# Jabruson/FDN-TIP2025

Hardware: AMD Instinct MI355X
Metric: images/sec, FDN (LPNet->FDN forward) 1280x720 bs=8 fp32 (higher is better)
Workload: dtype f32; 1 GPU; BASELINE.json configs[1]: FDN 1280x720 (padded 1280x736) batch=8 per GPU fp32; global_batch=8, parallelism=batch-shard x1, weights=synthetic (tamed 0.03) FDN + real LPNet, hip_streams=1, rccl_ranks=1, hip_graph=True, fdsa_full=False, fdsa_pair=False, no_tail_pin=False, tail_pin_l2=False, narrow_pipe=False, unfused_mlps=False, stats_launches=False, resample_upsample=False, aff_resized=False

## Files before the change

### fdn-tip2025_amd/basicsr/models/archs/FDN_arch.py

```python
import numbers

import numpy as np
import torch
import torch.nn as nn
import torch.nn.functional as F
from einops import rearrange

import fdn_hip
from fdn_hip import ACT_LEAKY, ACT_NONE, ACT_SIGMOID, ops


_Cache = ops.WeightCache


def _w(p):
    return p.detach()


class WithBias_LayerNorm(nn.Module):

    def __init__(self, dim):
        super().__init__()
        self.weight = nn.Parameter(torch.ones(dim))
        self.bias = nn.Parameter(torch.zeros(dim))
# ... 128 lines not shown
        self.dwconv = nn.Conv2d(hidden, hidden * 2, kernel_size=3, padding=1, groups=hidden, bias=bias)
        self._c = _Cache()

    def fused(self, xn, x_high, xp2, x_img, res=None, ln=None):
        _, _, h, w = xn.shape
        wp = ops.spec_pitch(w // 2 + 1)
        z = ops.rfft_rows_ln(xn, *ln, pitch=wp) if ln is not None else ops.rfft_rows(xn, pitch=wp)
        ops.fft_cols_fcaffn(z, x_high, xp2, _w(self.conv1_xa.weight), _w(self.conv1_xp.weight))
        xi = ops.irfft_rows(z, h, w, 2.0 / (h * w))
        gam, bet = self.norm.params()
        if xi.shape[1] in ops.FCAFFN_IN_C and w % 2 == 0:
            t = ops.fcaffn_in(xi, xn, x_img, _w(self.project_in.weight), gam, bet, _w(self.conv1_mul.weight),
                              _w(self.conv3_mul.weight), _w(self.conv1_add.weight), _w(self.conv3_add.weight), x1_ln=ln)
        elif xi.shape[1] >= ops.FCAFFN_PACKED_MIN_C and fdn_hip.matrix_pipe() == "bf16":
            srcs = [self.project_in.weight, self.conv1_mul.weight, self.conv3_mul.weight, self.conv1_add.weight, self.conv3_add.weight]
            wpk = self._c.get("fcpk", srcs, lambda: ops.fcaffn_in_pack(*[_w(p) for p in srcs]))
            t = ops.fcaffn_in_packed(xi, None if ops.GEMM_OWN_STATS else ops.chan_stats(xi), xn, x_img, wpk, gam, bet, x1_ln=ln)
        else:
            stats = ops.chan_stats(xi)
            mul, add = ops.img_mod_maps(x_img, _w(self.conv1_mul.weight), _w(self.conv3_mul.weight),
                                        _w(self.conv1_add.weight), _w(self.conv3_add.weight))
            t = ops.conv1x1(xi, _w(self.project_in.weight), ln_muladd=(stats, gam, bet, xn), muladd=(mul, add), cache=(self._c, "pi"))
        return ops.ffn_tail(t, _w(self.dwconv.weight), _w(self.project_out.weight), res=res, want_stats=res is not None,
                            cache=(self._c, "po"))

    def forward(self, x, x_high, xp2, x_img=None):
        return self.fused(x, x_high, xp2, x_img)


class TransformerBlock(nn.Module):

    def __init__(self, dim, ffn_expansion_factor=2.66, mode=1, bias=False, LayerNorm_type="WithBias", att=False,
                 use_light=True, use_img=True):
        super().__init__()
        self.use_light = use_light
        self.att = att
        if att:
            self.norm1 = LayerNorm(dim)
            self.attn = FDSA(dim, bias)
        self.norm2 = LayerNorm(dim)
        self.ffn = FDFFN(dim, bias, use_light=use_light, use_img=use_img)
        if use_light:
            self.norm3 = LayerNorm(dim)
            self.ffn2 = FCAFFN(dim, bias, use_light=use_light, use_img=use_img)

    def forward(self, xt):
        x, x_high, x_p, x_img = xt
        if self.att:
            x = self.attn.fused(x, ln=(ops.stats_of(x),) + self.norm1.params(), res=x, pin=(self.ffn, self.norm2.params()))
        x = self.ffn.fused(x, ln=(ops.stats_of(x),) + self.norm2.params(), res=x)
        if self.use_light:
            if (x.shape[1] in ops.FCAFFN_IN_C or (x.shape[1] >= ops.FCAFFN_PACKED_MIN_C and fdn_hip.matrix_pipe() == "bf16")) and ops.rows_ln_ok(x):
                x = self.ffn2.fused(x, x_high, x_p, x_img, res=x, ln=(ops.stats_of(x),) + self.norm3.params())
            else:
                x = self.ffn2.fused(self.norm3(x), x_high, x_p, x_img, res=x)
        return x, x_high, x_p, x_img


class Fuse(nn.Module):

    def __init__(self, n_feat):
        super().__init__()
        self.n_feat = n_feat
        self.att_channel = TransformerBlock(dim=n_feat * 2, use_light=False, use_img=False)
        self.conv = nn.Conv2d(n_feat * 2, n_feat * 2, 1, 1, 0)
        self.conv2 = nn.Conv2d(n_feat * 2, n_feat * 2, 1, 1, 0)
        self._c = _Cache()

    def forward(self, enc, dnc, x_high=None, x_high_p=None, x_img=None):
        n = self.n_feat
        x = ops.conv1x1([enc, dnc], _w(self.conv.weight), _w(self.conv.bias), want_stats=True, cache=(self._c, "c1"))
        x = self.att_channel((x, x_high, x_high_p, x_img))[0]
        wf = self._c.get("w", [self.conv2.weight], lambda: self.conv2.weight.detach()[:n] + self.conv2.weight.detach()[n:])
        bf = self._c.get("b", [self.conv2.bias], lambda: self.conv2.bias.detach()[:n] + self.conv2.bias.detach()[n:])
        return ops.conv1x1(x, wf, bf, cache=(self._c, "c2"), want_stats=True)


class OverlapPatchEmbed(nn.Module):
    def __init__(self, in_c=3, embed_dim=48, bias=False):
        super().__init__()
        self.proj = nn.Conv2d(in_c, embed_dim, kernel_size=3, stride=1, padding=1, bias=bias)

    def forward(self, x):
        return ops.conv2d(x, _w(self.proj.weight), pad=1)


class Downsample(nn.Module):

    def __init__(self, n_feat):
        super().__init__()
        self.body = nn.Sequential(nn.Identity(), nn.Conv2d(n_feat, n_feat * 2, 3, stride=1, padding=1, bias=False))

    def forward(self, x):
        return ops.conv2d(ops.resample(x, ops.RS_BILINEAR_HALF), _w(self.body[1].weight), pad=1)


class Upsample(nn.Module):

    def __init__(self, n_feat):
        super().__init__()
        self.body = nn.Sequential(nn.Identity(), nn.Conv2d(n_feat, n_feat // 2, 3, stride=1, padding=1, bias=False))
        self._c = _Cache()

    def forward(self, x):
        if ops.UPCONV_GATHER:
            return ops.upsample_conv3x3(x, _w(self.body[1].weight), cache=(self._c, "up"))
        return ops.conv2d(ops.resample(x, ops.RS_BILINEAR_X2), _w(self.body[1].weight), pad=1)


class FDformer(nn.Module):

    def __init__(self, inp_channels=3, out_channels=3, dim=48, num_blocks=[6, 6, 12, 8], num_refinement_blocks=4,
                 ffn_expansion_factor=3, bias=False):
        super().__init__()

        def stage(d, n, enc):
            return nn.Sequential(*[TransformerBlock(dim=d, ffn_expansion_factor=ffn_expansion_factor, bias=bias, att=True,
                                                    mode=1 if enc else 2, use_light=enc, use_img=enc) for _ in range(n)])

        self.patch_embed = OverlapPatchEmbed(inp_channels, dim)
        self.encoder_level1 = stage(dim, num_blocks[0], True)
        self.down1_2 = Downsample(dim)
        self.encoder_level2 = stage(dim * 2, num_blocks[1], True)
        self.down2_3 = Downsample(dim * 2)
        self.encoder_level3 = stage(dim * 4, num_blocks[2], True)
        self.decoder_level3 = stage(dim * 4, num_blocks[2], False)
        self.up3_2 = Upsample(dim * 4)
        self.reduce_chan_level2 = nn.Conv2d(dim * 4, dim * 2, kernel_size=1, bias=bias)
        self.decoder_level2 = stage(dim * 2, num_blocks[1], False)
        self.up2_1 = Upsample(dim * 2)
        self.decoder_level1 = stage(dim, num_blocks[0], False)
        self.refinement = stage(dim, num_refinement_blocks, False)
        self.fuse2 = Fuse(dim * 2)
        self.fuse1 = Fuse(dim)
        self.output = nn.Conv2d(dim, out_channels, kernel_size=3, stride=1, padding=1, bias=bias)
        self.norm = LayerNorm(3)

    def forward(self, inp_img, ori_img=None, x_high1=None, x_high2=None, x_high3=None, x_high12=None, x_high22=None,
                x_high32=None, x1=None, x2=None, x3=None):
        e1 = self.encoder_level1((self.patch_embed(inp_img), x_high1, x_high12, x1))[0]
        e2 = self.encoder_level2((self.down1_2(e1), x_high2, x_high22, x2))[0]
        e3 = self.encoder_level3((self.down2_3(e2), x_high3, x_high32, x3))[0]
        d3 = self.decoder_level3((e3, x_high3, x_high32, x3))[0]
        d2 = self.fuse2(self.up3_2(d3), e2, x_high2, x_high22, x2)
        d2 = self.decoder_level2((d2, x_high2, x_high22, x2))[0]
        d1 = self.fuse1(self.up2_1(d2), e1, x_high1, x_high12, x1)
        d1 = self.decoder_level1((d1, x_high1, x_high12, x1))[0]
        d1 = self.refinement((d1, x_high1, x_high12, x1))[0]
        res = inp_img if ori_img is None else ori_img
        return ops.conv2d(d1, _w(self.output.weight), pad=1, res=res)


class BasicConv(nn.Module):
    def __init__(self, in_channel, out_channel, kernel_size, stride, bias=True, relu=True, transpose=False):
        super().__init__()
        self.k, self.stride, self.relu, self.transpose = kernel_size, stride, relu, transpose
        if transpose:
            conv = nn.ConvTranspose2d(in_channel, out_channel, kernel_size, padding=kernel_size // 2 - 1, stride=stride, bias=bias)
        else:
            conv = nn.Conv2d(in_channel, out_channel, kernel_size, padding=kernel_size // 2, stride=stride, bias=bias)
        self.main = nn.Sequential(conv)

    def forward(self, x, res=None, res_before_act=False, act=None, post_add=0.0):
        c = self.main[0]
        a = (ACT_LEAKY if self.relu else ACT_NONE) if act is None else act
        if self.transpose:
            return ops.conv_transpose4x4s2(x, _w(c.weight), _w(c.bias), a)
        if self.k == 1 and self.stride == 1:
            return ops.conv1x1(x, _w(c.weight), _w(c.bias), act=a)
        return ops.conv2d(x, _w(c.weight), _w(c.bias), stride=self.stride, pad=self.k // 2, act=a, res=res,
                          res_before_act=res_before_act, post_add=post_add)


class FAM(nn.Module):
    def __init__(self, channel):
        super().__init__()
        self.merge1 = nn.Conv2d(channel * 2, channel, kernel_size=1)
        self.merge2 = nn.Conv2d(channel, channel, kernel_size=3, stride=1, padding=1)

    def forward(self, x1, x2):
        t = ops.conv1x1([x1, x2], _w(self.merge1.weight), _w(self.merge1.bias))
        return ops.conv2d(t, _w(self.merge2.weight), _w(self.merge2.bias), pad=1)


def _mlp2(seq, x):
    t = ops.conv1x1(x, _w(seq[0].weight), _w(seq[0].bias), act=ACT_LEAKY)
    return ops.conv1x1(t, _w(seq[2].weight), _w(seq[2].bias))


def _spectral_mlps(y, process1, process2, H, W):
    z = ops.rfft_rows(y)
    mag, pha = ops.fft_cols_fwd(z, True, True, rd_before=False, fix_real=True)
    if ops.SPECTRAL_MLP_FUSED and mag.shape[1] in ops.SPECTRAL_MLP_C:
        ops.spectral_mlp2(mag, pha, _w(process1[0].weight), _w(process1[0].bias), _w(process1[2].weight), _w(process1[2].bias),
                          _w(process2[0].weight), _w(process2[0].bias), _w(process2[2].weight), _w(process2[2].bias), slope=0.1)
    else:
        mag = _mlp2(process1, mag)
        pha = _mlp2(process2, pha)
    return ops.fft_cols_inv_polar(mag, pha, H, W // 2 + 1)


class FreBlock(nn.Module):
    def __init__(self, nc):
        super().__init__()
        self.fpre = nn.Conv2d(nc, nc, 1, 1, 0)
        self.process1 = nn.Sequential(nn.Conv2d(nc, nc, 1, 1, 0), nn.LeakyReLU(0.1), nn.Conv2d(nc, nc, 1, 1, 0))
        self.process2 = nn.Sequential(nn.Conv2d(nc, nc, 1, 1, 0), nn.LeakyReLU(0.1), nn.Conv2d(nc, nc, 1, 1, 0))

    def forward(self, x, skip_gain=1.0):
        _, _, H, W = x.shape
        y = ops.conv1x1(x, _w(self.fpre.weight), _w(self.fpre.bias))
        zz = _spectral_mlps(y, self.process1, self.process2, H, W)
        return ops.irfft_rows(zz, H, W, 2.0 / (H * W), res=x, alpha=skip_gain)


class ProcessBlock(nn.Module):
    def __init__(self, in_nc, spatial=False):
        super().__init__()
        self.frequency_process = FreBlock(in_nc)
        self.cat = nn.Conv2d(in_nc, in_nc, 1, 1, 0)

    def forward(self, x):
        return self.frequency_process(x, skip_gain=2.0)


class fourier_fuse(nn.Module):
    def __init__(self, in_nc, out_nc):
        super().__init__()
        self.fpre = nn.Sequential(nn.Conv2d(in_nc, out_nc, 1, 1), nn.Conv2d(out_nc, out_nc, 1, 1, 1, groups=out_nc))
        self.process1 = nn.Sequential(nn.Conv2d(out_nc, out_nc, 1, 1, 0), nn.LeakyReLU(0.1), nn.Conv2d(out_nc, out_nc, 1, 1, 0))
        self.process2 = nn.Sequential(nn.Conv2d(out_nc, out_nc, 1, 1, 0), nn.LeakyReLU(0.1), nn.Conv2d(out_nc, out_nc, 1, 1, 0))
        self.fourier_out = nn.Conv2d(out_nc, out_nc, 3, 1, 1)
        self._c = _Cache()

    def forward(self, x1, x2, x4):
        return self._rest(ops.conv1x1([x1, x2, x4], _w(self.fpre[0].weight), _w(self.fpre[0].bias)))

    def forward_multires(self, same, up1, up2):
        wfull, bias = _w(self.fpre[0].weight), _w(self.fpre[0].bias)
        n = wfull.shape[0]
        ks = sum(t.shape[1] for t in same)
        k1 = 0 if up1 is None else up1.shape[1]
        w2 = wfull.reshape(n, -1)
        parts = self._c.get("split", [self.fpre[0].weight], lambda: (w2[:, :ks].contiguous(), w2[:, ks:ks + k1].contiguous(), w2[:, ks + k1:].contiguous()))
        acc = ops.conv1x1(up2, parts[2])
        if up1 is not None:
            acc = ops.conv1x1(up1, parts[1], res=ops.resample(acc, ops.RS_NEAREST_X2))
        return self._rest(ops.conv1x1(same, parts[0], bias, res=ops.resample(acc, ops.RS_NEAREST_X2)))

    def _rest(self, y):
        H, W = y.shape[-2:]
        y = ops.dw1x1_pad1(y, _w(self.fpre[1].weight), _w(self.fpre[1].bias))
        zz = _spectral_mlps(y, self.process1, self.process2, H, W)
        xo = ops.irfft_rows(zz, H, W, 2.0 / (H * W))
        return ops.conv2d(xo, _w(self.fourier_out.weight), _w(self.fourier_out.bias), pad=1)


class MAR_archa(nn.Module):
    def __init__(self, use_ratio=True, block=None, apply_ratio=True):
        super().__init__()
        ProcessBlock_ = ProcessBlock if block is None else block
        self.use_ratio = use_ratio
        self.apply_ratio = apply_ratio
        c = 12
        self.Encoder = nn.ModuleList([ProcessBlock_(c), ProcessBlock_(c * 2), ProcessBlock_(c * 4)])
        self.Decoder = nn.ModuleList([ProcessBlock_(c * 4), ProcessBlock_(c * 2), ProcessBlock_(c)])
        self.Convs = nn.ModuleList([BasicConv(c * 4, c * 2, 1, 1, relu=True), BasicConv(c * 2, c, 1, 1, relu=True)])
        self.ConvsOut = nn.ModuleList([BasicConv(c * 4, 3, 3, 1, relu=False), BasicConv(c * 2, 3, 3, 1, relu=False)])
        self.AFFs = nn.ModuleList([fourier_fuse(c * 7, c), fourier_fuse(c * 7, c * 2)])
        self.FAM1 = FAM(c * 4)
        self.f1 = nn.Sequential(nn.Conv2d(3 * 16, c * 4, 1, 1, 0), ProcessBlock_(c * 4))
        self.f2 = nn.Sequential(nn.Conv2d(3 * 4, c * 2, 1, 1, 0), ProcessBlock_(c * 2))
        self.f3 = nn.Sequential(nn.Conv2d(3, c, 1, 1, 0), ProcessBlock_(c))
        self.f3_down = BasicConv(c, c * 2, 3, 2, relu=True)
        self.f2_down = BasicConv(c * 2, c * 4, 3, 2, relu=True)
        self.f2_up = BasicConv(c * 4, c * 2, 4, 2, relu=True, transpose=True)
        self.f3_up = BasicConv(c * 2, c, 4, 2, relu=True, transpose=True)
        self.out = BasicConv(c, 3, 3, 1, relu=False)
        self.FAM2 = FAM(c * 2)

    def _stem(self, seq, x, ratio):
        t = seq[1](ops.conv1x1(x, _w(seq[0].weight), _w(seq[0].bias)))
        return ops.scale_batch_(t, ratio) if self.apply_ratio else t

    def forward(self, x, ratio):
        x_2 = ops.resample(x, ops.RS_NEAREST_HALF)
        x_4 = ops.resample(x_2, ops.RS_NEAREST_HALF)
        z2 = self._stem(self.f2, ops.resample(x, ops.RS_PIXEL_UNSHUFFLE, 2), ratio)
        z4 = self._stem(self.f1, ops.resample(x, ops.RS_PIXEL_UNSHUFFLE, 4), ratio)
        x_ = self._stem(self.f3, x, ratio)
        res1 = self.Encoder[0](x_)
        res2 = self.Encoder[1](self.FAM2(self.f3_down(res1), z2))
        z = self.Encoder[2](self.FAM1(self.f2_down(res2), z4))
        z12 = ops.resample(res1, ops.RS_NEAREST_HALF)
        if ops.AFF_MULTIRES:
            res2n = self.AFFs[1].forward_multires([z12, res2], None, z)
            res1 = self.AFFs[0].forward_multires([res1], res2, z)
            res2 = res2n
        else:
            z21 = ops.resample(res2, ops.RS_NEAREST_X2)
            z42 = ops.resample(z, ops.RS_NEAREST_X2)
            z41 = ops.resample(z42, ops.RS_NEAREST_X2)
            res2 = self.AFFs[1](z12, res2, z42)
            res1 = self.AFFs[0](res1, z21, z41)
        z = self.Decoder[0](z)
        o4 = self.ConvsOut[0](z, res=x_4, res_before_act=True, act=ACT_SIGMOID, post_add=1e-8)
        z = self.f2_up(z)
        c0 = self.Convs[0].main[0]
        z = self.Decoder[1](ops.conv1x1([z, res2], _w(c0.weight), _w(c0.bias), act=ACT_LEAKY))
        o2 = self.ConvsOut[1](z, res=x_2, res_before_act=True, act=ACT_SIGMOID, post_add=1e-8)
        z = self.f3_up(z)
        c1 = self.Convs[1].main[0]
        z = self.Decoder[2](ops.conv1x1([z, res1], _w(c1.weight), _w(c1.bias), act=ACT_LEAKY))
        o1 = self.out(z, res=x, res_before_act=True, act=ACT_SIGMOID, post_add=1e-8)
        return [o4, o2, o1]


class MAR(nn.Module):
    def __init__(self, use_ratio=True):
        super().__init__()
        self.net = MAR_archa(use_ratio=True)
        self.scale = 40.0
        self.use_ratio = use_ratio

    def forward(self, x, ratio=None):
        ratio = ratio.reshape(-1).contiguous()
        x1 = x
        x2 = ops.resample(x1, ops.RS_BILINEAR_HALF)
        x3 = ops.resample(x2, ops.RS_BILINEAR_HALF)
        i3, i2, i1 = self.net(x, ratio)
        return ops.gamma_curve(x3, i3, self.scale), ops.gamma_curve(x2, i2, self.scale), ops.gamma_curve(x1, i1, self.scale)


class FDN(nn.Module):

    def __init__(self):
        super().__init__()
        self.net_a = MAR(use_ratio=True)
        self.net_p = FDformer(inp_channels=3, out_channels=3, dim=32, num_blocks=[6, 6, 10], num_refinement_blocks=4,
                              ffn_expansion_factor=3, bias=False)
        for p in self.net_a.parameters():
            p.requires_grad = False
        self.norm1 = LayerNorm(3)
        self.norm2 = LayerNorm(3)
        self.norm3 = LayerNorm(3)

    @staticmethod
    def _spectrum(x, want_abs, want_ang, rd):
        return ops.fft_cols_fwd(ops.rfft_rows(x), want_abs, want_ang, rd_before=rd, fix_real=True)

    def forward(self, inp_img, ori=None, device=None, ratio_i=None, mode=1):
        if ratio_i is None:
            raise ValueError("FDN.forward needs ratio_i of shape (B, 1) (reference FDN_arch.py:872)")
        inp_img = inp_img.contiguous()
        ratio = ratio_i.reshape(-1).to(torch.float32).contiguous()
        norms = (self.norm1, self.norm2, self.norm3)
        p1 = inp_img
        p2 = ops.resample(p1, ops.RS_BILINEAR_HALF)
        p3 = ops.resample(p2, ops.RS_BILINEAR_HALF)
        phas = [self._spectrum(n(p), False, True, True)[1] for n, p in zip(norms, (p1, p2, p3))]
        q3, q2, q1 = self.net_a(inp_img, ratio)
        amps = [self._spectrum(n(q), True, False, False)[0] for n, q in zip(norms, (q1, q2, q3))]
        out = self.net_p(inp_img, ori_img=inp_img, x_high1=amps[0], x_high2=amps[1], x_high3=amps[2],
                         x_high12=phas[0], x_high22=phas[1], x_high32=phas[2], x1=q1, x2=q2, x3=q3)
        return out, q1, q2, q3
```

### fdn-tip2025_amd/basicsr/models/archs/fdnlol24_arch.py

```python
import numbers

import numpy as np
import torch
import torch.nn as nn
import torch.nn.functional as F
from einops import rearrange

from fdn_hip import ops
from basicsr.models.archs.FDN_arch import (FDN, FDformer, FreBlock, LayerNorm, MAR_archa, _w)
from basicsr.models.archs import FDN_arch as _blur


class ProcessBlock(nn.Module):

    def __init__(self, in_nc, spatial=False):
        super().__init__()
        if spatial:
            raise NotImplementedError("spatial=True is never instantiated by FDN_lolv1 (fdnlol24_arch.py:104-137)")
        self.frequency_process = FreBlock(in_nc)
        self.cat = nn.Conv2d(in_nc, in_nc, 1, 1, 0)

    def forward(self, x):
        y = self.frequency_process(x, skip_gain=1.0)
        return ops.conv1x1(y, _w(self.cat.weight), _w(self.cat.bias), res=x)


class fourier_multi_scale_gamma2(MAR_archa):

    def __init__(self, use_ratio):
        super().__init__(use_ratio=use_ratio, block=ProcessBlock, apply_ratio=bool(use_ratio))


class MAR(_blur.MAR):

    def __init__(self, use_ratio=True):
        super().__init__(use_ratio=use_ratio)
        self.net = fourier_multi_scale_gamma2(use_ratio=use_ratio)


class FDN_lolv1(FDN):

    def __init__(self):
        nn.Module.__init__(self)
        self.net_a = MAR(use_ratio=True)
        self.net_p = FDformer(inp_channels=3, out_channels=3, dim=24, num_blocks=[6, 6, 10], num_refinement_blocks=4,
                              ffn_expansion_factor=3, bias=False)
        for p in self.net_a.parameters():
            p.requires_grad = False
        self.norm1 = LayerNorm(3)
        self.norm2 = LayerNorm(3)
        self.norm3 = LayerNorm(3)

    def forward(self, inp_img, ori=None, device=None, ratio_i=None, mode=1):
        out = super().forward(inp_img, ori=ori, device=device, ratio_i=ratio_i, mode=mode)[0]
        return out, out, out, out
```

### fdn-tip2025_amd/csrc/capi.hip

```cpp
#include "common.hpp"

#include <atomic>
extern "C" int fdn_abi_version(void) { return 20; }

static std::atomic<int> g_matrix_pipe_mode{0};
extern "C" int fdn_set_matrix_pipe(int mode) {
    if (mode < 0 || mode > 2) return FDN_ERR_ARG;
    g_matrix_pipe_mode.store(mode);
    return FDN_OK;
}
bool fdn_matrix_pipe_f32() { return g_matrix_pipe_mode.load() == 1; }
bool fdn_matrix_pipe_wide() { return g_matrix_pipe_mode.load() == 0; }

static std::atomic<long long> g_bf16_launches{0};
void fdn_note_bf16_launch() { g_bf16_launches.fetch_add(1, std::memory_order_relaxed); }
extern "C" long fdn_bf16_mfma_launches(void) { return g_bf16_launches.load(); }

extern "C" const char* fdn_error_string(int code) {
    switch (code) {
        case FDN_OK: return "ok";
        case FDN_ERR_ARG: return "invalid argument (null pointer, bad shape or unsupported size)";
        case FDN_ERR_LAUNCH: return "HIP kernel launch failed";
        case FDN_ERR_WORKSPACE: return "workspace too small";
        case FDN_ERR_UNSUPPORTED: return "configuration not supported by this build";
        default: return "unknown error";
    }
}

#include <mutex>
#include <map>
#include <utility>

namespace {
std::mutex g_mu;
int g_cus_by_dev[64];
int g_cu_budget_by_dev[64];
std::map<std::pair<const void*, int>, size_t> g_lds_limit;
struct OccKey {
    const void* k; int dev, threads; size_t lds;
    bool operator<(const OccKey& o) const {
        if (k != o.k) return k < o.k;
        if (dev != o.dev) return dev < o.dev;
        if (threads != o.threads) return threads < o.threads;
        return lds < o.lds;
    }
};
std::map<OccKey, int> g_occ;
}

bool fdn_occupancy(int* blocks_per_cu, const void* kernel, int threads, size_t lds) {
    int dev = 0;
    if (hipGetDevice(&dev) != hipSuccess) return false;
    std::lock_guard<std::mutex> lk(g_mu);
    const OccKey key{kernel, dev, threads, lds};
    auto it = g_occ.find(key);
    if (it == g_occ.end()) {
        int n = 0;
        if (hipOccupancyMaxActiveBlocksPerMultiprocessor(&n, kernel, threads, lds) != hipSuccess) return false;
        it = g_occ.emplace(key, n).first;
    }
    *blocks_per_cu = it->second;
    return true;
}

int fdn_persistent_grid(const void* kernel, int threads, size_t lds, int total_tiles, fdn_grid_cap cap) {
    const int cus = fdn_device_cus();
    if (cus <= 0) return -1;
    if (lds > 48 * 1024 && !fdn_allow_dynamic_lds(kernel, lds)) return -1;
    int per_cu = 1 << 20;
    if (cap.by_occupancy && !fdn_occupancy(&per_cu, kernel, threads, lds)) per_cu = 1;
    if (cap.max_wg > 0 && per_cu > cap.max_wg) per_cu = cap.max_wg;
    if (cap.max_waves > 0 && per_cu * (threads / 64) > cap.max_waves) per_cu = cap.max_waves / (threads / 64);
    if (cap.lds_budget > 0 && lds > 0 && (size_t)per_cu > cap.lds_budget / lds) per_cu = (int)(cap.lds_budget / lds);
    if (per_cu < 1) per_cu = 1;
    const long grid = (long)cus * per_cu;
    return grid > total_tiles ? total_tiles : (int)grid;
}

namespace {
int device_cus_locked(int dev) {
    if (g_cus_by_dev[dev] == 0) {
        int n = 0;
        if (hipDeviceGetAttribute(&n, hipDeviceAttributeMultiprocessorCount, dev) != hipSuccess || n <= 0) return -1;
        g_cus_by_dev[dev] = n;
    }
    return g_cus_by_dev[dev];
// ... 33 lines not shown
```

### fdn-tip2025_amd/csrc/convs.hip

```cpp
#include "common.hpp"

int fdn_conv3x3_mfma(const float* x, const float* w, const float* bias, const float* res, float* out, int B, int Cin, int H,
                     int W, int Cout, int act, int res_before_act, float post_add, hipStream_t s);

namespace {

constexpr int OCB = 8;

struct ConvArgs {
    const float* x; const float* w; const float* bias; const float* res; float* out;
    int B, Cin, H, W, Cout, OH, OW, KH, KW, stride, pad;
    int act; int res_before_act; float post_add;
};

__global__ __launch_bounds__(256) void conv2d_kernel(ConvArgs a) {
    unsigned bx, by, bz;
    fdn_xcd_block3(bx, by, bz);
    const long op = (long)bx * 256 + threadIdx.x;
    const int oc0 = by * OCB, b = bz;
    const long OP = (long)a.OH * a.OW;
    const bool live = op < OP;
    const int oy = live ? (int)(op / a.OW) : 0, ox = live ? (int)(op - (long)oy * a.OW) : 0;
    float acc[OCB];
#pragma unroll
// ... 13 lines not shown
                const float* wp = a.w + ((long)oc0 * a.Cin + ci) * kk + ky * a.KW + kx;
#pragma unroll
                for (int o = 0; o < OCB; ++o)
                    if (o < nvalid) acc[o] = fmaf(v, wp[(long)o * a.Cin * kk], acc[o]);
            }
        }
    }
    if (!live) return;
#pragma unroll
    for (int o = 0; o < OCB; ++o) {
        if (o >= nvalid) break;
        const int oc = oc0 + o;
        float v = acc[o] + (a.bias ? a.bias[oc] : 0.f);
        const long oi = ((long)b * a.Cout + oc) * OP + op;
        if (a.res && a.res_before_act) v += a.res[oi];
        v = apply_act(v, a.act);
        if (a.res && !a.res_before_act) v += a.res[oi];
        a.out[oi] = v + a.post_add;
    }
}

template <int S, int OCB_>
__global__ __launch_bounds__(256) void conv3x3_direct_kernel(ConvArgs a) {
    extern __shared__ __attribute__((aligned(16))) float wl[];
    unsigned bx, by, bz;
    fdn_xcd_block3(bx, by, bz);
    const int oc0 = by * OCB_, b = bz;
    const int nvalid = min(OCB_, a.Cout - oc0);
    for (int i = threadIdx.x; i < a.Cin * 9 * OCB_; i += 256) {
        const int o = i % OCB_, t = (i / OCB_) % 9, ci = i / (OCB_ * 9);
        wl[i] = o < nvalid ? a.w[((long)(oc0 + o) * a.Cin + ci) * 9 + t] : 0.f;
    }
    __syncthreads();
    const long op = (long)bx * 256 + threadIdx.x;
    const long OP = (long)a.OH * a.OW;
    const bool live = op < OP;
    const int oy = live ? (int)(op / a.OW) : 0, ox = live ? (int)(op - (long)oy * a.OW) : 0;
    int off[9];
    unsigned ok = 0;
#pragma unroll
    for (int t = 0; t < 9; ++t) {
        const int iy = oy * S - 1 + t / 3, ix = ox * S - 1 + t % 3;
        const bool v = live && iy >= 0 && iy < a.H && ix >= 0 && ix < a.W;
        off[t] = v ? iy * a.W + ix : 0;
        ok |= (v ? 1u : 0u) << t;
    }
    float acc[OCB_];
#pragma unroll
    for (int o = 0; o < OCB_; ++o) acc[o] = 0.f;
    const long hw = (long)a.H * a.W;
    const float* xc = a.x + (long)b * a.Cin * hw;
    for (int ci = 0; ci < a.Cin; ++ci, xc += hw) {
        float v[9];
#pragma unroll
        for (int t = 0; t < 9; ++t) v[t] = xc[off[t]];
#pragma unroll
        for (int t = 0; t < 9; ++t) {
            const float vv = ((ok >> t) & 1u) ? v[t] : 0.f;
            const float* wp = wl + (ci * 9 + t) * OCB_;
#pragma unroll
            for (int o = 0; o < OCB_; ++o) acc[o] = fmaf(vv, wp[o], acc[o]);
        }
    }
    if (!live) return;
#pragma unroll
    for (int o = 0; o < OCB_; ++o) {
        if (o >= nvalid) break;
        const int oc = oc0 + o;
        float v = acc[o] + (a.bias ? a.bias[oc] : 0.f);
        const long oi = ((long)b * a.Cout + oc) * OP + op;
        if (a.res && a.res_before_act) v += a.res[oi];
        v = apply_act(v, a.act);
        if (a.res && !a.res_before_act) v += a.res[oi];
        a.out[oi] = v + a.post_add;
    }
}

template <int S, int OCB_>
int launch_conv3x3_direct(const ConvArgs& a, hipStream_t s) {
    const size_t lds = (size_t)a.Cin * 9 * OCB_ * sizeof(float);
    if (lds > 64 * 1024) return FDN_ERR_UNSUPPORTED;
    hipLaunchKernelGGL((conv3x3_direct_kernel<S, OCB_>), dim3(cdiv((long)a.OH * a.OW, 256), cdiv(a.Cout, OCB_), a.B), dim3(256),
                       lds, s, a);
    return fdn_launch_status();
}

template <int OCB_>
__global__ __launch_bounds__(256) void convT_kernel(const float* __restrict__ x, const float* __restrict__ w,
                                                    const float* __restrict__ bias, float* __restrict__ out, int Cin, int H,
                                                    int W, int Cout, int act) {
    extern __shared__ __attribute__((aligned(16))) float wl[];
    unsigned bx, by, bz;
    fdn_xcd_block3(bx, by, bz);
    const int oc0 = by * OCB_, b = bz;
    const int nvalid = min(OCB_, Cout - oc0);
    for (int i = threadIdx.x; i < Cin * 16 * OCB_; i += 256) {
        const int o = i % OCB_, t = (i / OCB_) % 16, ci = i / (OCB_ * 16);
        wl[i] = o < nvalid ? w[((long)ci * Cout + oc0 + o) * 16 + t] : 0.f;
    }
    __syncthreads();
    const int OH = 2 * H, OW = 2 * W;
    const long op = (long)bx * 256 + threadIdx.x;
    const long OP = (long)OH * OW;
    const bool live = op < OP;
    const int oy = live ? (int)(op / OW) : 0, ox = live ? (int)(op - (long)oy * OW) : 0;
    const int ky0 = (oy + 1) & 1, kx0 = (ox + 1) & 1;
    int off[4], tap[4];
    unsigned ok = 0;
#pragma unroll
    for (int j = 0; j < 4; ++j) {
        const int ky = ky0 + 2 * (j >> 1), kx = kx0 + 2 * (j & 1);
        const int ny = oy + 1 - ky, nx = ox + 1 - kx;
        const int iy = ny >> 1, ix = nx >> 1;
        const bool v = live && ny >= 0 && iy < H && nx >= 0 && ix < W;
        off[j] = v ? iy * W + ix : 0;
        tap[j] = (ky * 4 + kx) * OCB_;
        ok |= (v ? 1u : 0u) << j;
    }
    float acc[OCB_];
#pragma unroll
    for (int o = 0; o < OCB_; ++o) acc[o] = 0.f;
    const long hw = (long)H * W;
    const float* xc = x + (long)b * Cin * hw;
    for (int ci = 0; ci < Cin; ++ci, xc += hw) {
        float v[4];
#pragma unroll
        for (int j = 0; j < 4; ++j) v[j] = xc[off[j]];
#pragma unroll
        for (int j = 0; j < 4; ++j) {
            const float vv = ((ok >> j) & 1u) ? v[j] : 0.f;
            const float* wp = wl + ci * 16 * OCB_ + tap[j];
#pragma unroll
            for (int o = 0; o < OCB_; ++o) acc[o] = fmaf(vv, wp[o], acc[o]);
        }
    }
    if (!live) return;
#pragma unroll
    for (int o = 0; o < OCB_; ++o) {
        if (o >= nvalid) break;
        out[((long)b * Cout + oc0 + o) * OP + op] = apply_act(acc[o] + (bias ? bias[oc0 + o] : 0.f), act);
    }
}

template <int OCB_>
__global__ __launch_bounds__(256) void convT_quad_kernel(const float* __restrict__ x, const float* __restrict__ w, const float* __restrict__ bias,
                                                         float* __restrict__ out, int Cin, int H, int W, int Cout, int act) {
    static_assert(OCB_ % 4 == 0, "weight rows are read as 16-byte words");
    extern __shared__ __attribute__((aligned(16))) float wl[];
    unsigned bx, by, bz;
    fdn_xcd_block3(bx, by, bz);
    const int oc0 = by * OCB_, b = bz;
    const int nvalid = min(OCB_, Cout - oc0);
    for (int i = threadIdx.x; i < Cin * 16 * OCB_; i += 256) {
        const int o = i % OCB_, t = (i / OCB_) % 16, ci = i / (OCB_ * 16);
        wl[i] = o < nvalid ? w[((long)ci * Cout + oc0 + o) * 16 + t] : 0.f;
    }
    __syncthreads();
    const long hw = (long)H * W;
    const int W2 = W >> 1;
    const long ip = (long)bx * 256 + threadIdx.x;
    const bool live = ip < (long)H * W2;
    const int iy = live ? (int)(ip / W2) : 0, ix0 = live ? 2 * (int)(ip - (long)iy * W2) : 0;
    int off[12];
    unsigned ok = 0;
#pragma unroll
    for (int d = 0; d < 12; ++d) {
// ... 262 lines not shown
        const float* w1 = ws, *w2t = ws + C * C, *b1 = ws + 2 * C * C, *b2 = b1 + C;
        float v[C], o[C];
#pragma unroll
        for (int i = 0; i < C; ++i) v[i] = t[base + (long)i * P];
#pragma unroll
        for (int k = 0; k < C; ++k) o[k] = b2[k];
#pragma unroll 1
        for (int j = 0; j < C; ++j) {
            float s = b1[j];
#pragma unroll
            for (int i = 0; i < C; ++i) s = fmaf(w1[j * C + i], v[i], s);
            const float h = s > 0.f ? s : s * slope;
#pragma unroll
            for (int k = 0; k < C; ++k) o[k] = fmaf(w2t[j * C + k], h, o[k]);
        }
#pragma unroll
        for (int k = 0; k < C; ++k) t[base + (long)k * P] = o[k];
    };
    mlp(mag, wsh);
    mlp(pha, wsh + WS);
}

__global__ __launch_bounds__(256) void gamma_curve_kernel(const float* __restrict__ x, const float* __restrict__ im,
                                                          float* __restrict__ out, float scale, long total) {
    const long idx = (long)blockIdx.x * 256 + threadIdx.x;
    if (idx < total) out[idx] = 1.0f - powf(1.0f - x[idx], im[idx] * scale);
}

template <int CIN, int COUT>
__global__ __launch_bounds__(256) void conv7x7s2_kernel(ConvArgs a) {
    constexpr int TR = 8, TCW = 32;
    constexpr int IR = 2 * TR + 5, IC = 2 * TCW + 5;
    constexpr int HC = (IC + 1) / 2;
    __shared__ float tile[CIN][IR][2][HC + 1];
    __shared__ __attribute__((aligned(16))) float wl[CIN * 49 * COUT];
    unsigned bx, by, bz;
    fdn_xcd_block3(bx, by, bz);
    const int tid = threadIdx.x, b = bz;
    const int oy0 = by * TR, ox0 = bx * TCW;
    for (int i = tid; i < CIN * 49 * COUT; i += 256) {
        const int o = i % COUT, t = i / COUT;
        wl[i] = a.w[(long)o * CIN * 49 + t];
    }
    const long hw = (long)a.H * a.W;
    const float* xb = a.x + (long)b * CIN * hw;
    const int iy0 = oy0 * 2 - 3, ix0 = ox0 * 2 - 3;
    for (int i = tid; i < CIN * IR * IC; i += 256) {
        const int c = i % IC, r = (i / IC) % IR, ci = i / (IC * IR);
        const int iy = iy0 + r, ix = ix0 + c;
        tile[ci][r][c & 1][c >> 1] = (iy >= 0 && iy < a.H && ix >= 0 && ix < a.W) ? xb[(long)ci * hw + (long)iy * a.W + ix] : 0.f;
    }
    __syncthreads();
    const int ty = tid >> 5, tx = tid & 31;
    float acc[COUT];
#pragma unroll
    for (int o = 0; o < COUT; ++o) acc[o] = 0.f;
#pragma unroll 1
    for (int ci = 0; ci < CIN; ++ci)
#pragma unroll
        for (int ky = 0; ky < 7; ++ky)
#pragma unroll
            for (int kx = 0; kx < 7; ++kx) {
                const float v = tile[ci][2 * ty + ky][kx & 1][tx + (kx >> 1)];
                const float* wp = wl + ((ci * 7 + ky) * 7 + kx) * COUT;
#pragma unroll
                for (int o = 0; o < COUT; ++o) acc[o] = fmaf(v, wp[o], acc[o]);
            }
    const int oy = oy0 + ty, ox = ox0 + tx;
    if (oy >= a.OH || ox >= a.OW) return;
    const long OP = (long)a.OH * a.OW, op = (long)oy * a.OW + ox;
#pragma unroll
    for (int oc = 0; oc < COUT; ++oc) {
        float v = acc[oc] + (a.bias ? a.bias[oc] : 0.f);
        const long oi = ((long)b * COUT + oc) * OP + op;
        if (a.res && a.res_before_act) v += a.res[oi];
        v = apply_act(v, a.act);
        if (a.res && !a.res_before_act) v += a.res[oi];
        a.out[oi] = v + a.post_add;
    }
}

}

extern "C" int fdn_conv2d(const float* x, const float* w, const float* bias, const float* res, float* out, int B, int Cin,
                          int H, int W, int Cout, int KH, int KW, int stride, int pad, int act, int res_before_act,
                          float post_add, fdn_stream_t stream) {
    FDN_CHECK_ARG(x && w && out && B > 0 && Cin > 0 && Cout > 0 && H > 0 && W > 0 && KH > 0 && KW > 0 && stride > 0 && pad >= 0);
    ConvArgs a;
    a.x = x; a.w = w; a.bias = bias; a.res = res; a.out = out;
    a.B = B; a.Cin = Cin; a.H = H; a.W = W; a.Cout = Cout; a.KH = KH; a.KW = KW; a.stride = stride; a.pad = pad;
    a.OH = (H + 2 * pad - KH) / stride + 1;
    a.OW = (W + 2 * pad - KW) / stride + 1;
    FDN_CHECK_ARG(a.OH > 0 && a.OW > 0);
    a.act = act; a.res_before_act = res_before_act; a.post_add = post_add;
    hipStream_t s = static_cast<hipStream_t>(stream);
    if (KH == 3 && KW == 3 && pad == 1 && (stride == 1 || stride == 2)) {
        int rc = FDN_ERR_UNSUPPORTED;
        if (stride == 1 && Cin % 8 == 0 && Cin >= 16 && Cout >= 16 && !fdn_matrix_pipe_f32()) {
            rc = fdn_conv3x3_mfma(x, w, bias, res, out, B, Cin, H, W, Cout, act, res_before_act, post_add, s);
            if (rc != FDN_ERR_UNSUPPORTED) return rc;
        }
        if (stride == 2) rc = Cout <= 8 ? launch_conv3x3_direct<2, 8>(a, s) : launch_conv3x3_direct<2, 16>(a, s);
        else if (Cout <= 4) rc = launch_conv3x3_direct<1, 4>(a, s);
        else if (Cout <= 8) rc = launch_conv3x3_direct<1, 8>(a, s);
        else if (Cout <= 64) rc = launch_conv3x3_direct<1, 16>(a, s);
        if (rc != FDN_ERR_UNSUPPORTED) return rc;
        if (stride == 1) {
            rc = fdn_conv3x3_mfma(x, w, bias, res, out, B, Cin, H, W, Cout, act, res_before_act, post_add, s);
            if (rc != FDN_ERR_UNSUPPORTED) return rc;
        }
    }
    if (KH == 7 && KW == 7 && stride == 2 && pad == 3 && Cin == 3 && Cout == 16) {
        hipLaunchKernelGGL((conv7x7s2_kernel<3, 16>), dim3(cdiv(a.OW, 32), cdiv(a.OH, 8), B), dim3(256), 0, s, a);
        return fdn_launch_status();
    }
    hipLaunchKernelGGL(conv2d_kernel, dim3(cdiv((long)a.OH * a.OW, 256), cdiv(Cout, OCB), B), dim3(256), 0, s, a);
    return fdn_launch_status();
}

extern "C" int fdn_conv_transpose4x4s2(const float* x, const float* w, const float* bias, float* out, int B, int Cin, int H,
                                       int W, int Cout, int act, fdn_stream_t stream) {
    FDN_CHECK_ARG(x && w && out && B > 0 && Cin > 0 && Cout > 0 && H > 0 && W > 0);
    hipStream_t s = static_cast<hipStream_t>(stream);
    if (Cout >= 12 && W % 2 == 0 && (size_t)Cin * 16 * 12 * sizeof(float) <= 48 * 1024 && (reinterpret_cast<uintptr_t>(out) & 15) == 0) {
        hipLaunchKernelGGL(convT_quad_kernel<12>, dim3(cdiv((long)H * (W / 2), 256), cdiv(Cout, 12), B), dim3(256), (size_t)Cin * 16 * 12 * sizeof(float), s,
                           x, w, bias, out, Cin, H, W, Cout, act);
        return fdn_launch_status();
    }
    if (Cout > 8 && (size_t)Cin * 16 * 16 * sizeof(float) <= 64 * 1024) {
        hipLaunchKernelGGL(convT_kernel<16>, dim3(cdiv(4L * H * W, 256), cdiv(Cout, 16), B), dim3(256), (size_t)Cin * 16 * 16 * sizeof(float),
                           s, x, w, bias, out, Cin, H, W, Cout, act);
    } else {
        FDN_CHECK_ARG((size_t)Cin * 16 * 8 * sizeof(float) <= 64 * 1024);
        hipLaunchKernelGGL(convT_kernel<8>, dim3(cdiv(4L * H * W, 256), cdiv(Cout, 8), B), dim3(256), (size_t)Cin * 16 * 8 * sizeof(float), s,
                           x, w, bias, out, Cin, H, W, Cout, act);
    }
    return fdn_launch_status();
}

extern "C" int fdn_resample(const float* x, float* out, long planes, int H, int W, int mode, int r, fdn_stream_t stream) {
    FDN_CHECK_ARG(x && out && planes > 0 && H > 0 && W > 0);
    int OH, OW;
    long oplanes = planes;
    switch (mode) {
        case FDN_RS_BILINEAR_HALF:
        case FDN_RS_NEAREST_HALF: FDN_CHECK_ARG(H % 2 == 0 && W % 2 == 0); OH = H / 2; OW = W / 2; break;
        case FDN_RS_BILINEAR_X2:
        case FDN_RS_NEAREST_X2: OH = 2 * H; OW = 2 * W; break;
        case FDN_RS_PIXEL_UNSHUFFLE: FDN_CHECK_ARG(r > 0 && H % r == 0 && W % r == 0); OH = H / r; OW = W / r; oplanes = planes * r * r; break;
        default: return FDN_ERR_ARG;
    }
    FDN_CHECK_ARG(OH <= 65535);
    const long rr = mode == FDN_RS_PIXEL_UNSHUFFLE ? (long)r * r : 1;
    FDN_CHECK_ARG(rr <= 65535);
    const long chunk = 65535 / rr * rr;
    for (long p0 = 0; p0 < oplanes; p0 += chunk) {
        const long np = oplanes - p0 < chunk ? oplanes - p0 : chunk;
        const long in_pl = p0 / rr;
        const bool quad = OW % 4 == 0 && ((reinterpret_cast<uintptr_t>(x) | reinterpret_cast<uintptr_t>(out)) & 15) == 0 &&
                          (mode != FDN_RS_BILINEAR_HALF || W % 8 == 0);
        const dim3 qgrid((unsigned)cdiv((long)OH * (OW / 4), 256), (unsigned)np);
        if (quad && mode == FDN_RS_BILINEAR_X2)
            hipLaunchKernelGGL(resample4_kernel<FDN_RS_BILINEAR_X2>, qgrid, dim3(256), 0, static_cast<hipStream_t>(stream),
                               x + in_pl * H * W, out + p0 * OH * OW, H, W, OH, OW);
        else if (quad && mode == FDN_RS_BILINEAR_HALF)
            hipLaunchKernelGGL(resample4_kernel<FDN_RS_BILINEAR_HALF>, qgrid, dim3(256), 0, static_cast<hipStream_t>(stream),
                               x + in_pl * H * W, out + p0 * OH * OW, H, W, OH, OW);
        else if (quad && mode == FDN_RS_NEAREST_X2 && W % 2 == 0)
            hipLaunchKernelGGL(resample4_kernel<FDN_RS_NEAREST_X2>, qgrid, dim3(256), 0, static_cast<hipStream_t>(stream),
                               x + in_pl * H * W, out + p0 * OH * OW, H, W, OH, OW);
        else
        hipLaunchKernelGGL(resample_kernel, dim3(cdiv(OW, 256), OH, (unsigned)np), dim3(256), 0, static_cast<hipStream_t>(stream),
                           x + in_pl * H * W, out + p0 * OH * OW, np, H, W, OH, OW, mode, r);
    }
    return fdn_launch_status();
}

extern "C" int fdn_upconv_gather(const float* z, float* out, int B, int Cout, int h, int w, fdn_stream_t stream) {
    FDN_CHECK_ARG(z && out && B > 0 && Cout > 0 && h > 0 && w > 0 && B < 65536);
    FDN_CHECK_ARG((reinterpret_cast<uintptr_t>(out) & 7) == 0);
    if ((long)h * w > 0x7FFFFFFFL / 4) return FDN_ERR_UNSUPPORTED;
    constexpr int COB = 8;
    hipLaunchKernelGGL(upconv_gather_kernel<COB>, dim3((unsigned)cdiv((long)h * w, 256), (unsigned)cdiv(Cout, COB), (unsigned)B), dim3(256), 0,
                       static_cast<hipStream_t>(stream), z, out, Cout, h, w);
    return fdn_launch_status();
}

extern "C" int fdn_dw1x1_pad1(const float* x, const float* w, const float* bias, float* out, int B, int C, int H, int W,
                              fdn_stream_t stream) {
    FDN_CHECK_ARG(x && w && bias && out && B > 0 && C > 0 && H > 0 && W > 0);
    FDN_CHECK_ARG(H + 2 <= 65535 && (long)B * C <= 65535);
    hipLaunchKernelGGL(dw1x1_pad1_kernel, dim3(cdiv(W + 2, 256), H + 2, (unsigned)(B * C)), dim3(256), 0, static_cast<hipStream_t>(stream),
                       x, w, bias, out, C, H, W);
    return fdn_launch_status();
}

extern "C" int fdn_avgpool3s2(const float* x, float* out, long planes, int H, int W, fdn_stream_t stream) {
    FDN_CHECK_ARG(x && out && planes > 0 && H > 0 && W > 0);
    const int OH = (H + 2 - 3) / 2 + 1, OW = (W + 2 - 3) / 2 + 1;
    hipLaunchKernelGGL(avgpool3s2_kernel, dim3(cdiv(planes * OH * OW, 256)), dim3(256), 0, static_cast<hipStream_t>(stream), x,
// ... 47 lines not shown
```

### fdn-tip2025_amd/csrc/fft2d.hip

```cpp
#include <math.h>

#include <map>
#include <mutex>
#include <vector>

#include "common.hpp"
#include "fft_regs.hpp"

namespace {

constexpr int MAX_STAGES = FDN_FFT_MAX_STAGES;
constexpr int NT = 256;

struct Plan {
    int N;
    int nst;
    int radix[MAX_STAGES];
    const float2* tw;
    int tab_mul;
};

std::mutex g_mu;
std::map<std::pair<int, int>, const float2*> g_tables;

// ... 300 lines not shown
    __syncthreads();
    return src;
}

constexpr int EMAX = 36;

template <bool INV, int R>
__device__ void fft_pass_inplace(float2* buf, int N, int Ns, int nseq, const float2* __restrict__ tw) {
    constexpr int JMAX = EMAX / R;
    const int T = N / R;
    const int L = Ns * R;
    const int tws = N / L, twr = N / R;
    const int jobs = T * nseq;
    const float r_nseq = 1.0f / (float)nseq, r_Ns = 1.0f / (float)Ns;
    float2 u[JMAX][R];
#pragma unroll
    for (int j = 0; j < JMAX; ++j) {
        const int job = threadIdx.x + NT * j;
        if (job < jobs) {
            const int i = fdiv(job, r_nseq), s = job - i * nseq;
            const int k = i - fdiv(i, r_Ns) * Ns;
#pragma unroll
            for (int r = 0; r < R; ++r) u[j][r] = buf[s + (i + r * T) * nseq];
            if (k) {
#pragma unroll
                for (int r = 1; r < R; ++r) u[j][r] = cmul(u[j][r], twd<INV>(tw, r * k * tws));
            }
        }
    }
    __syncthreads();
#pragma unroll
    for (int j = 0; j < JMAX; ++j) {
        const int job = threadIdx.x + NT * j;
        if (job < jobs) {
            const int i = fdiv(job, r_nseq), s = job - i * nseq;
            const int k = i - fdiv(i, r_Ns) * Ns;
            float2* dp = buf + s + ((i - k) * R + k) * nseq;
            if (R == 2) {
                dp[0] = make_float2(u[j][0].x + u[j][1].x, u[j][0].y + u[j][1].y);
                dp[Ns * nseq] = make_float2(u[j][0].x - u[j][1].x, u[j][0].y - u[j][1].y);
            } else if (R == 4) {
                const float2 a = make_float2(u[j][0].x + u[j][2].x, u[j][0].y + u[j][2].y);
                const float2 b = make_float2(u[j][0].x - u[j][2].x, u[j][0].y - u[j][2].y);
                const float2 c = make_float2(u[j][1].x + u[j][3].x, u[j][1].y + u[j][3].y);
                const float2 d = make_float2(u[j][1].x - u[j][3].x, u[j][1].y - u[j][3].y);
                const float2 jd = INV ? make_float2(-d.y, d.x) : make_float2(d.y, -d.x);
                dp[0] = make_float2(a.x + c.x, a.y + c.y);
                dp[Ns * nseq] = make_float2(b.x + jd.x, b.y + jd.y);
                dp[2 * Ns * nseq] = make_float2(a.x - c.x, a.y - c.y);
                dp[3 * Ns * nseq] = make_float2(b.x - jd.x, b.y - jd.y);
            } else if constexpr (R % 2 == 1) {
                float2 wR[(R - 1) / 2];
#pragma unroll
                for (int t = 1; t <= (R - 1) / 2; ++t) wR[t - 1] = twd<INV>(tw, t * twr);
                dft_odd<R>(u[j], wR);
#pragma unroll
                for (int o = 0; o < R; ++o) dp[o * Ns * nseq] = u[j][o];
            }
        }
    }
    __syncthreads();
}

template <bool INV, int BIG>
__device__ void fft_run_inplace(float2* buf, const Plan& p, const float2* tw, int nseq) {
    int Ns = 1;
    __syncthreads();
    for (int st = 0; st < p.nst; ++st) {
        const int R = p.radix[st];
        switch (R) {
            case 2: fft_pass_inplace<INV, 2>(buf, p.N, Ns, nseq, tw); break;
            case 3: fft_pass_inplace<INV, 3>(buf, p.N, Ns, nseq, tw); break;
            case 4: fft_pass_inplace<INV, 4>(buf, p.N, Ns, nseq, tw); break;
            case 5: fft_pass_inplace<INV, 5>(buf, p.N, Ns, nseq, tw); break;
            case 7: fft_pass_inplace<INV, 7>(buf, p.N, Ns, nseq, tw); break;
            case 17: if (BIG) fft_pass_inplace<INV, 17>(buf, p.N, Ns, nseq, tw); break;
            case 23: if (BIG) fft_pass_inplace<INV, 23>(buf, p.N, Ns, nseq, tw); break;
            default: break;
        }
        Ns *= R;
    }
}

template <bool BIG>
__global__ __launch_bounds__(NT) void rfft_rows_kernel(const float* __restrict__ in, float2* __restrict__ out, int W, long R,
                                                       int rpb, const Plan p, const Rader rd, int pitch) {
    extern __shared__ __attribute__((aligned(16))) unsigned char smem[];
    const int M = W / 2, Wf = M + 1;
    float2* A = reinterpret_cast<float2*>(smem);
    float2* Bf = A + (long)rpb * M;
    float2* twl = Bf + (long)rpb * M;
    float2* tws = twl + W;
    for (int i = threadIdx.x; i < W; i += NT) twl[i] = p.tw[i];
    if (rd.p)
        for (int i = threadIdx.x; i < M - 1; i += NT) tws[i] = rd.sub.tw[i];
    const long row0 = (long)blockIdx.x * rpb;
    const int nrow = (int)min((long)rpb, R - row0);
    {
        constexpr int U = 8;
        const float2* in2 = reinterpret_cast<const float2*>(in + row0 * W);
        const int tot = rpb * M, live = nrow * M;
        if (M % 2 == 0 && (reinterpret_cast<uintptr_t>(in) & 15) == 0) {
            const float4* in4 = reinterpret_cast<const float4*>(in2);
            float4* A4 = reinterpret_cast<float4*>(A);
            const int tot4 = tot / 2, live4 = live / 2;
            for (int base = threadIdx.x; base < tot4; base += NT * 4) {
                float4 v[4];
#pragma unroll
                for (int u = 0; u < 4; ++u) {
                    const int idx = base + NT * u;
                    v[u] = in4[idx < live4 ? idx : 0];
                }
#pragma unroll
                for (int u = 0; u < 4; ++u) {
                    const int idx = base + NT * u;
                    if (idx < tot4) A4[idx] = idx < live4 ? v[u] : make_float4(0.f, 0.f, 0.f, 0.f);
                }
            }
        } else
        for (int base = threadIdx.x; base < tot; base += NT * U) {
            float2 v[U];
#pragma unroll
            for (int u = 0; u < U; ++u) {
                const int idx = base + NT * u;
                v[u] = in2[idx < live ? idx : 0];
            }
#pragma unroll
            for (int u = 0; u < U; ++u) {
                const int idx = base + NT * u;
                if (idx < tot) A[idx] = idx < live ? v[u] : make_float2(0.f, 0.f);
            }
        }
    }
    float2* Z;
    if (rd.p) {
        const int n = M - 1;
        float2* z0 = tws + n;
        __syncthreads();
        for (int idx = threadIdx.x; idx < rpb * n; idx += NT) {
            const int s = idx / n, q = idx - s * n;
            Bf[s * M + q] = A[s * M + rd.perm_in[q]];
        }
        if (threadIdx.x < rpb) z0[threadIdx.x] = A[threadIdx.x * M];
        float2* Y = fft_run<false, BIG>(Bf, A, rd.sub, tws, rpb, M, 1, false);
        float2* other = (Y == Bf) ? A : Bf;
        __syncthreads();
        for (int idx = threadIdx.x; idx < rpb * n; idx += NT) {
            const int s = idx / n, k = idx - s * n;
            const float2 y = Y[s * M + k];
            if (k == 0) other[s * M + n] = make_float2(z0[s].x + y.x, z0[s].y + y.y);
            Y[s * M + k] = cmul(y, rd.bhat[k]);
        }
        __syncthreads();
        float2 x0 = make_float2(0.f, 0.f);
        const bool keeper = threadIdx.x < rpb;
        if (keeper) x0 = other[threadIdx.x * M + n];
        float2* Cv = fft_run<true, BIG>(Y, other, rd.sub, tws, rpb, M, 1, false);
        float2* dst = (Cv == Y) ? other : Y;
        __syncthreads();
        for (int idx = threadIdx.x; idx < rpb * n; idx += NT) {
            const int s = idx / n, q = idx - s * n;
            const float2 c = Cv[s * M + q];
            dst[s * M + rd.perm_out[q]] = make_float2(z0[s].x + c.x, z0[s].y + c.y);
        }
        if (keeper) dst[threadIdx.x * M] = x0;
        __syncthreads();
        Z = dst;
    } else {
        Z = fft_run<false, BIG>(A, Bf, p, twl, rpb, M, 1, false);
    }
    const int tw1 = p.tab_mul / 2;
    const float r_Wf = 1.0f / (float)Wf;
#pragma unroll 4
    for (int idx = threadIdx.x; idx < nrow * Wf; idx += NT) {
        const int s = fdiv(idx, r_Wf), k = idx - s * Wf;
        const float2 zk = Z[s * M + (k == M ? 0 : k)];
        const float2 zc = Z[s * M + (k == 0 ? 0 : M - k)];
        const float2 e = make_float2(0.5f * (zk.x + zc.x), 0.5f * (zk.y - zc.y));
        const float2 d = make_float2(0.5f * (zk.x - zc.x), 0.5f * (zk.y + zc.y));
        const float2 o = make_float2(d.y, -d.x);
        float2 x;
        if (k == 0) x = make_float2(e.x + o.x, 0.0f);
        else if (k == M) x = make_float2(e.x - o.x, 0.0f);
        else {
            const float2 w = twl[k * tw1];
            x = make_float2(e.x + (o.x * w.x - o.y * w.y), e.y + (o.x * w.y + o.y * w.x));
        }
        out[(row0 + s) * pitch + k] = x;
    }
    for (int idx = threadIdx.x; idx < nrow * (pitch - Wf); idx += NT) {
        const int s = idx / (pitch - Wf), k = Wf + idx - s * (pitch - Wf);
        out[(row0 + s) * pitch + k] = make_float2(0.f, 0.f);
    }
}

template <bool BIG>
__global__ __launch_bounds__(NT) void irfft_rows_kernel(const float2* __restrict__ in, long in_ws, long in_plane_rows,
                                                        long in_plane_stride, float* __restrict__ out, int W, int H, long R,
                                                        int rpb, float scale, const float* __restrict__ res, float alpha,
                                                        const Plan p) {
    extern __shared__ __attribute__((aligned(16))) unsigned char smem[];
    const int M = W / 2;
    float2* A = reinterpret_cast<float2*>(smem);
    float2* Bf = A + (long)rpb * M;
    float2* twl = Bf + (long)rpb * M;
    for (int i = threadIdx.x; i < W; i += NT) twl[i] = p.tw[i];
    __syncthreads();
    const long row0 = (long)blockIdx.x * rpb;
    const int nrow = (int)min((long)rpb, R - row0);
    const int tw1 = p.tab_mul / 2;
    constexpr int UL = 4;
    const float r_M = 1.0f / (float)M, r_H = 1.0f / (float)H;
    for (int base = threadIdx.x; base < rpb * M; base += NT * UL) {
      float2 xks[UL], xcs[UL];
#pragma unroll
      for (int u = 0; u < UL; ++u) {
        const int idx = base + NT * u;
        const int s0 = fdiv(idx, r_M), k = idx - s0 * M;
        const int s = min(s0, nrow - 1);
        const long row = row0 + s;
        const long plane = row < (1L << 22) ? (long)fdiv((int)row, r_H) : row / H, h = row - plane * H;
        const float2* src = in + plane * in_plane_stride + h * in_ws;
        xks[u] = src[k];
        xcs[u] = src[M - k];
      }
#pragma unroll
      for (int u = 0; u < UL; ++u) {
        const int idx = base + NT * u;
        if (idx >= rpb * M) continue;
        const int s = fdiv(idx, r_M), k = idx - s * M;
        float2 z = make_float2(0.f, 0.f);
        if (s < nrow) {
            float2 xk = xks[u], xc = xcs[u];
            if (k == 0) { xk.y = 0.f; xc.y = 0.f; }
            const float2 e = make_float2(0.5f * (xk.x + xc.x), 0.5f * (xk.y - xc.y));
            const float2 d = make_float2(0.5f * (xk.x - xc.x), 0.5f * (xk.y + xc.y));
            const float2 w = twl[k * tw1];
            const float2 o = make_float2(d.x * w.x + d.y * w.y, d.y * w.x - d.x * w.y);
            z = make_float2(e.x - o.y, e.y + o.x);
        }
        A[idx] = z;
      }
    }
    float2* Z = fft_run<true, BIG>(A, Bf, p, twl, rpb, M, 1, false);
    {
        constexpr int US = 8;
        const float2* res2 = res ? reinterpret_cast<const float2*>(res + row0 * W) : nullptr;
        float2* out2 = reinterpret_cast<float2*>(out + row0 * W);
        const int live = nrow * M;
        if (M % 2 == 0 && ((reinterpret_cast<uintptr_t>(out) | reinterpret_cast<uintptr_t>(res)) & 15) == 0) {
            const float4* res4 = reinterpret_cast<const float4*>(res2);
            float4* out4 = reinterpret_cast<float4*>(out2);
            const float4* Z4 = reinterpret_cast<const float4*>(Z);
            const int live4 = live / 2;
            for (int base = threadIdx.x; base < live4; base += NT * 4) {
                float4 r[4];
                if (res4) {
#pragma unroll
                    for (int u = 0; u < 4; ++u) r[u] = res4[min(base + NT * u, live4 - 1)];
                }
#pragma unroll
                for (int u = 0; u < 4; ++u) {
                    const int idx = base + NT * u;
                    if (idx >= live4) continue;
                    float4 v = Z4[idx];
                    v.x *= scale; v.y *= scale; v.z *= scale; v.w *= scale;
                    if (res4) {
                        v.x = fmaf(alpha, r[u].x, v.x); v.y = fmaf(alpha, r[u].y, v.y);
                        v.z = fmaf(alpha, r[u].z, v.z); v.w = fmaf(alpha, r[u].w, v.w);
                    }
                    out4[idx] = v;
                }
            }
        } else
        for (int base = threadIdx.x; base < live; base += NT * US) {
            float2 r[US];
            if (res2) {
#pragma unroll
                for (int u = 0; u < US; ++u) r[u] = res2[min(base + NT * u, live - 1)];
            }
#pragma unroll
            for (int u = 0; u < US; ++u) {
                const int idx = base + NT * u;
                if (idx >= live) continue;
                float2 v = Z[idx];
                v.x *= scale;
                v.y *= scale;
                if (res2) {
                    v.x = fmaf(alpha, r[u].x, v.x);
                    v.y = fmaf(alpha, r[u].y, v.y);
                }
                out2[idx] = v;
            }
        }
    }
}

struct ColArgs {
    float2* z;
    int H, Wf, C;
    int tc, tcs;
    long planes;
    const float4* guide;
    const float* wxa;
    const float* wxp;
    float* out_abs;
    float* out_ang;
    int rd_before;
    int fix_real;
    const float* in_mag;
    const float* in_pha;
    int Hin, Wfin;
};

enum { COL_FCAFFN = 0, COL_FWD = 1, COL_INV_POLAR = 2 };

template <int MODE, int BIG, bool INPL>
__global__ __launch_bounds__(NT, (INPL ? 2 : 1)) void fft_cols_kernel(ColArgs a, const Plan p) {
    extern __shared__ __attribute__((aligned(16))) unsigned char smem[];
    const int H = a.H, Wf = a.Wf, tc = a.tc;
    float2* A = reinterpret_cast<float2*>(smem);
    float2* Bf = A + (long)H * tc;
    float2* twl = INPL ? Bf : Bf + (long)H * tc;
    for (int i = threadIdx.x; i < H; i += NT) twl[i] = p.tw[i];
    int plane, col0;
    {
        const int ntile = (Wf + tc - 1) / tc;
        const long total = (long)ntile * a.planes, per_xcd = (total + 7) / 8;
        const long w = (long)(blockIdx.x & 7) * per_xcd + (blockIdx.x >> 3);
        if (w >= total) return;
        const int C = a.C;
        const long grp = w / C;
        const int ch = (int)(w - grp * C);
        plane = (int)(grp / ntile) * C + ch;
        col0 = (int)(grp % ntile) * tc;
    }
    const int ncol = min(tc, Wf - col0);
    float2* zp = a.z + (long)plane * H * Wf;

    const int per = H * tc, tcs = a.tcs, tcm = tc - 1;
    if (MODE == COL_INV_POLAR) {
        constexpr int U = 4;
        for (int base = threadIdx.x; base < per; base += NT * U) {
            float mg[U], ph[U];
#pragma unroll
            for (int u = 0; u < U; ++u) {
                const int idx = base + NT * u, h = idx >> tcs, c = idx & tcm;
                mg[u] = 0.f; ph[u] = 0.f;
                if (idx < per && c < ncol) {
                    const long o = ((long)plane * a.Hin + h) * a.Wfin + col0 + c;
                    mg[u] = a.in_mag[o];
                    ph[u] = a.in_pha[o];
                }
            }
#pragma unroll
            for (int u = 0; u < U; ++u) {
                const int idx = base + NT * u;
                if (idx < per) {
                    float sn, cs;
                    fdn_sincos(ph[u], &sn, &cs);
                    A[idx] = make_float2(mg[u] * cs, mg[u] * sn);
                }
            }
        }
    } else {
        constexpr int U = 12;
        for (int base = threadIdx.x; base < per; base += NT * U) {
            float2 v[U];
#pragma unroll
            for (int u = 0; u < U; ++u) {
                const int idx = base + NT * u, h = idx >> tcs, c = idx & tcm;
                v[u] = make_float2(0.f, 0.f);
                if (idx < per && c < ncol) v[u] = zp[(long)h * Wf + col0 + c];
// ... 524 lines not shown
    const long row0 = (long)blockIdx.x * RW;
    const int nrow = (int)min((long)RW, R - row0);
    {
        const int n2 = tid & (P - 1), rw = tid / P < RW ? tid / P : RW - 1;
        const int rwc = rw < nrow ? rw : nrow - 1;
        const __amdgpu_buffer_rsrc_t rin = cols_rsrc(in + row0 * W, (long)nrow * W * 4);
        const unsigned voff = (unsigned)(rwc * W + 2 * n2) * 4u;
        f2 u[R1];
        sfor<0, R1>([&](auto n1) { u[decltype(n1)::value] = bload2(rin, voff, (unsigned)(decltype(n1)::value * P * 8)); });
        if constexpr (LN) {
            const long row = row0 + rwc, plane = row / lnp.H;
            const int h = (int)(row - plane * lnp.H), c = (int)(plane % lnp.C);
            const long b = plane / lnp.C, HW = (long)lnp.H * W;
            const __amdgpu_buffer_rsrc_t rs_ = cols_rsrc(lnp.stats, (R / ((long)lnp.C * lnp.H)) * 2 * HW * 4);
            const unsigned so = (unsigned)(b * 2 * HW + h * W + 2 * n2) * 4u;
            const float ga = lnp.gamma[c], be = lnp.beta[c];
            f2 mu[R1], rs[R1];
            sfor<0, R1>([&](auto n1) {
                constexpr int N1 = decltype(n1)::value;
                mu[N1] = bload2(rs_, so, (unsigned)(N1 * P * 8));
                rs[N1] = bload2(rs_, so + (unsigned)HW * 4u, (unsigned)(N1 * P * 8));
            });
            sfor<0, R1>([&](auto n1) {
                constexpr int N1 = decltype(n1)::value;
                u[N1] = (u[N1] - mu[N1]) * rs[N1] * ga + be;
            });
        }
        fftr::dft_nat<R1, false>(u);
        sfor<0, R1>([&](auto k1) { Y[rw * RS + decltype(k1)::value * PS + n2] = u[decltype(k1)::value]; });
    }
    __syncthreads();
    const int jt = (tid + 64 * (int)(blockIdx.x & 3)) & 255;
    const bool worker = jt < NJ;
    const int rg = jt / R1, k1 = jt - rg * R1;
    f2 v[32];
    if (worker) {
        const f2* yb = Y + rg * CJ * RS + k1 * PS;
        sfor<0, P>([&](auto n) {
            constexpr int N2 = decltype(n)::value;
#pragma unroll
            for (int cc = 0; cc < CJ; ++cc) v[cc * P + N2] = yb[cc * RS + N2];
            if constexpr (N2 > 0) {
                const f2 w = tw2[(N2 - 1) * R1 + k1];
#pragma unroll
                for (int cc = 0; cc < CJ; ++cc) v[cc * P + N2] = fftr::cmul(v[cc * P + N2], w);
            }
        });
#pragma unroll
        for (int cc = 0; cc < CJ; ++cc) fftr::dft_nat<P, false>(v + cc * P);
    }
    __syncthreads();
    if (worker) {
        f2* zb = Y + rg * CJ * RS + k1;
        sfor<0, P>([&](auto k2) {
#pragma unroll
            for (int cc = 0; cc < CJ; ++cc) zb[cc * RS + R1 * decltype(k2)::value] = v[cc * P + decltype(k2)::value];
        });
    }
    __syncthreads();
    f2* out2 = reinterpret_cast<f2*>(out) + row0 * pitch;
    const int live = nrow * pitch;
    const float r_Wf = 1.0f / (float)pitch;
#pragma unroll 4
    for (int idx = tid; idx < live; idx += 256) {
        const int s = fdiv(idx, r_Wf), k = idx - s * pitch;
        if (k >= Wf) { out2[idx] = f2{0.f, 0.f}; continue; }
        const f2 zk = Y[s * RS + (k == M ? 0 : k)];
        const f2 zc = Y[s * RS + (k == 0 ? 0 : M - k)];
        const f2 e = 0.5f * f2{zk.x + zc.x, zk.y - zc.y};
        const f2 d = 0.5f * f2{zk.x - zc.x, zk.y + zc.y};
        const f2 o = fftr::mul_ni(d);
        f2 x;
        if (k == 0) x = f2{e.x + o.x, 0.0f};
        else if (k == M) x = f2{e.x - o.x, 0.0f};
        else x = e + fftr::cmul(o, tws[k]);
        out2[idx] = x;
    }
}

template <int R1, int P>
__global__ __launch_bounds__(256, 2) void irfft_rows_rp_kernel(const float2* __restrict__ in, long in_ws, long in_plane_stride,
                                                               float* __restrict__ out, int H, long R, float scale,
                                                               const float* __restrict__ res, float alpha,
                                                               const float2* __restrict__ tab) {
    typedef RowPlan<R1, P> L;
    constexpr int M = L::M, W = L::W, RW = L::RW, CJ = L::CJ, PS = L::PS, RS = L::RS, NJ = L::NJ;
    extern __shared__ __attribute__((aligned(16))) unsigned char smem[];
    f2* Y = reinterpret_cast<f2*>(smem);
    f2* tw2 = Y + RW * RS;
    f2* tws = tw2 + (P - 1) * R1;
    __shared__ long rowoff[RW];
    const int tid = threadIdx.x;
    for (int i = tid; i < L::NTW; i += 256) tw2[i] = f2{tab[i].x, tab[i].y};
    const long row0 = (long)blockIdx.x * RW;
    const int nrow = (int)min((long)RW, R - row0);
    if (tid < RW) {
        const long row = row0 + min(tid, nrow - 1);
        const long plane = row / H, h = row - plane * H;
        rowoff[tid] = plane * in_plane_stride + h * in_ws;
    }
    __syncthreads();
    {
        constexpr int UL = 4, NP = M / 2 + 1, TOT = RW * NP;
        const f2* in2 = reinterpret_cast<const f2*>(in);
        const float r_NP = 1.0f / (float)NP;
        for (int base = tid; base < TOT; base += 256 * UL) {
            f2 xks[UL], xcs[UL];
#pragma unroll
            for (int u = 0; u < UL; ++u) {
                const int idx = min(base + 256 * u, TOT - 1), s = fdiv(idx, r_NP), k = idx - s * NP;
                const f2* src = in2 + rowoff[s];
                xks[u] = src[k];
                xcs[u] = src[M - k];
            }
#pragma unroll
            for (int u = 0; u < UL; ++u) {
                const int idx = base + 256 * u;
                if (idx >= TOT) continue;
                const int s = fdiv(idx, r_NP), k = idx - s * NP;
                f2 xk = xks[u], xc = xcs[u];
                if (k == 0) { xk.y = 0.f; xc.y = 0.f; }
                const f2 e = 0.5f * f2{xk.x + xc.x, xk.y - xc.y};
                const f2 d = 0.5f * f2{xk.x - xc.x, xk.y + xc.y};
                const f2 io = fftr::mul_pi(fftr::cmulc(d, tws[k]));
                f2* row = Y + s * RS;
                row[k] = e + io;
                if (k != 0) {
                    const f2 c = e - io;
                    row[M - k] = f2{c.x, -c.y};
                }
            }
        }
    }
    __syncthreads();
    const int jt = (tid + 64 * (int)(blockIdx.x & 3)) & 255;
    const bool worker = jt < NJ;
    const int rg = jt / R1, k1 = jt - rg * R1;
    f2 v[32];
    if (worker) {
        const f2* zb = Y + rg * CJ * RS + k1;
        sfor<0, P>([&](auto k2) {
#pragma unroll
            for (int cc = 0; cc < CJ; ++cc) v[cc * P + decltype(k2)::value] = zb[cc * RS + R1 * decltype(k2)::value];
        });
#pragma unroll
        for (int cc = 0; cc < CJ; ++cc) fftr::dft_nat<P, true>(v + cc * P);
    }
    __syncthreads();
    if (worker) {
        f2* yb = Y + rg * CJ * RS + k1 * PS;
        sfor<0, P>([&](auto n) {
            constexpr int N2 = decltype(n)::value;
            if constexpr (N2 > 0) {
                const f2 w = tw2[(N2 - 1) * R1 + k1];
#pragma unroll
                for (int cc = 0; cc < CJ; ++cc) v[cc * P + N2] = fftr::cmulc(v[cc * P + N2], w);
            }
#pragma unroll
            for (int cc = 0; cc < CJ; ++cc) yb[cc * RS + N2] = v[cc * P + N2];
        });
    }
    __syncthreads();
    {
        const int n2 = tid & (P - 1), rw = tid / P;
        const int rwl = rw < RW ? rw : RW - 1;
        f2 u[R1];
        sfor<0, R1>([&](auto k) { u[decltype(k)::value] = Y[rwl * RS + decltype(k)::value * PS + n2]; });
        fftr::dft_nat<R1, true>(u);
        if (rw < nrow) {
            const __amdgpu_buffer_rsrc_t ro = cols_rsrc(out + row0 * W, (long)nrow * W * 4);
            const __amdgpu_buffer_rsrc_t rr = cols_rsrc(res ? res + row0 * W : out, res ? (long)nrow * W * 4 : 0);
            const unsigned voff = (unsigned)(rw * W + 2 * n2) * 4u;
            f2 r[R1];
            if (res) sfor<0, R1>([&](auto n1) { r[decltype(n1)::value] = bload2(rr, voff, (unsigned)(decltype(n1)::value * P * 8)); });
            sfor<0, R1>([&](auto n1) {
                constexpr int N1 = decltype(n1)::value;
                f2 x = u[N1] * scale;
                if (res) x += alpha * r[N1];
                bstore2(x, ro, voff, (unsigned)(N1 * P * 8));
            });
        }
    }
}

const float2* get_table_rows_rp(int R1, int P) {
    int devid = 0;
    if (hipGetDevice(&devid) != hipSuccess) return nullptr;
    std::lock_guard<std::mutex> lk(g_mu);
    const int key = -(1 << 24) - (R1 * 1024 + P);
    auto it = g_tables.find({devid, key});
    if (it != g_tables.end()) return it->second;
    const int M = R1 * P, W = 2 * M;
    auto root = [](long t, long N) {
        t %= N;
        double c, s;
        if ((4 * t) % N == 0) {
            const int q = (int)((4 * t) / N);
            c = (q == 0) ? 1.0 : (q == 2 ? -1.0 : 0.0);
            s = (q == 1) ? 1.0 : (q == 3 ? -1.0 : 0.0);
        } else {
            const double ang = 2.0 * M_PI * (double)t / (double)N;
            c = cos(ang); s = sin(ang);
        }
        float2 w = make_float2((float)c, (float)(-s) + 0.0f);
        if (w.y == 0.0f) w.y = 0.0f;
        if (w.x == 0.0f) w.x = 0.0f;
        return w;
    };
    std::vector<float2> h;
    for (int n2 = 1; n2 < P; ++n2)
        for (int k1 = 0; k1 < R1; ++k1) h.push_back(root((long)n2 * k1, M));
    for (int k = 0; k <= M; ++k) h.push_back(root(k, W));
    float2* d = nullptr;
    if (hipMalloc(&d, sizeof(float2) * h.size()) != hipSuccess) return nullptr;
    if (hipMemcpy(d, h.data(), sizeof(float2) * h.size(), hipMemcpyHostToDevice) != hipSuccess) return nullptr;
    g_tables[{devid, key}] = d;
    return d;
}

template <int R1, int P>
int launch_rfft_rp(const float* in, float* out_c, long rows, fdn_stream_t stream, int pitch, const RowLN* ln = nullptr) {
    typedef RowPlan<R1, P> L;
    const float2* tab = get_table_rows_rp(R1, P);
    if (!tab) return FDN_ERR_LAUNCH;
    if (ln) {
        if (int e = set_lds(rfft_rows_rp_kernel<R1, P, true>, L::lds)) return e;
        hipLaunchKernelGGL((rfft_rows_rp_kernel<R1, P, true>), dim3(cdiv(rows, L::RW)), dim3(256), L::lds, static_cast<hipStream_t>(stream),
                           in, reinterpret_cast<float2*>(out_c), rows, tab, *ln, pitch);
        return fdn_launch_status();
    }
    if (int e = set_lds(rfft_rows_rp_kernel<R1, P, false>, L::lds)) return e;
    hipLaunchKernelGGL((rfft_rows_rp_kernel<R1, P, false>), dim3(cdiv(rows, L::RW)), dim3(256), L::lds, static_cast<hipStream_t>(stream), in,
                       reinterpret_cast<float2*>(out_c), rows, tab, RowLN{}, pitch);
    return fdn_launch_status();
}

template <int R1, int P>
int launch_irfft_rp(const float* in_c, long in_row_bins, long in_plane_bins, float* out, long planes, int H, float scale,
                    const float* res, float alpha, fdn_stream_t stream) {
    typedef RowPlan<R1, P> L;
    const float2* tab = get_table_rows_rp(R1, P);
    if (!tab) return FDN_ERR_LAUNCH;
    if (int e = set_lds(irfft_rows_rp_kernel<R1, P>, L::lds)) return e;
    const long rows = planes * H;
    hipLaunchKernelGGL((irfft_rows_rp_kernel<R1, P>), dim3(cdiv(rows, L::RW)), dim3(256), L::lds, static_cast<hipStream_t>(stream),
                       reinterpret_cast<const float2*>(in_c), in_row_bins, in_plane_bins, out, H, rows, scale, res, alpha, tab);
    return fdn_launch_status();
}

bool rows_plan(int W, int* R1, int* P) {
    for (int r : {20, 30})
        for (int p : {32, 16, 8})
            if (W == 2 * r * p) { *R1 = r; *P = p; return true; }
    for (int p : {16, 8})
        if (W == 2 * 19 * p) { *R1 = 19; *P = p; return true; }
    for (int p : {16, 8, 4})
        if (W == 2 * 35 * p) { *R1 = 35; *P = p; return true; }
    return false;
}
#define FDN_ROWS_DISPATCH(CALL)                                        \
    switch (R1 * 64 + P) {                                             \
        case 20 * 64 + 32: return CALL(20, 32);                        \
        case 20 * 64 + 16: return CALL(20, 16);                        \
        case 20 * 64 + 8: return CALL(20, 8);                          \
        case 30 * 64 + 32: return CALL(30, 32);                        \
        case 30 * 64 + 16: return CALL(30, 16);                        \
        case 30 * 64 + 8: return CALL(30, 8);                          \
        case 19 * 64 + 16: return CALL(19, 16);                        \
        case 19 * 64 + 8: return CALL(19, 8);                          \
        case 35 * 64 + 16: return CALL(35, 16);                        \
        case 35 * 64 + 8: return CALL(35, 8);                          \
        case 35 * 64 + 4: return CALL(35, 4);                          \
        default: break;                                                \
    }

}

extern "C" int fdn_fft_prepare(int n) {
    FDN_CHECK_ARG(n > 0);
    {
        int R = 0, P = 0;
        if (cols_plan(n, &R, &P) && !get_table_rp(R, P)) return FDN_ERR_LAUNCH;
    }
    {
        int R1 = 0, P = 0;
        if (rows_plan(n, &R1, &P) && !get_table_rows_rp(R1, P)) return FDN_ERR_LAUNCH;
    }
    return get_table(n) ? FDN_OK : FDN_ERR_LAUNCH;
}

extern "C" int fdn_fft_route(int kind, int n, int* desc, int ndesc) {
    FDN_CHECK_ARG(kind >= 0 && kind <= 2 && n >= 1 && desc && ndesc >= FDN_FFT_ROUTE_DESC);
    FDN_CHECK_ARG(kind == 2 || n % 2 == 0);
    for (int i = 0; i < FDN_FFT_ROUTE_DESC; ++i) desc[i] = 0;
    int R = 0, P = 0;
    if (kind == 2 ? cols_plan(n, &R, &P) : rows_plan(n, &R, &P)) {
        desc[0] = FDN_FFT_PLANNED;
        desc[2] = kind == 2 ? 256 / P : row_plan_groups(R, P) * (32 / P);
        desc[4] = 2;
        desc[5] = R;
        desc[6] = P;
        return FDN_OK;
    }
    Route r;
    if (kind == 2) cols_route(n, &r);
    else rows_route(n, kind == 0, &r);
    desc[0] = r.kind;
    if (r.kind == FDN_FFT_REFUSED) return FDN_OK;
    desc[1] = r.big;
    desc[2] = r.width;
    const Plan& q = r.kind == FDN_FFT_RADER ? r.sub : r.p;
    desc[3] = r.kind == FDN_FFT_RADER ? n / 2 : 0;
    desc[4] = q.nst;
    for (int i = 0; i < q.nst; ++i) {
        const int x = q.radix[i];
        const bool reg = x == 2 || x == 4 || x == 3 || x == 5 || x == 7 || (r.big >= 1 && (x == 17 || x == 23)) ||
                         (r.big == 2 && (x == 13 || x == 37 || x == 41));
        desc[5 + i] = x;
        desc[5 + MAX_STAGES + i] = (r.kind != FDN_FFT_INPLACE && !reg) ? 1 : 0;
    }
    return FDN_OK;
}

namespace {
__global__ __launch_bounds__(256) void sincos_kernel(const float* __restrict__ x, float* __restrict__ sn, float* __restrict__ cs, long n) {
    const long i = (long)blockIdx.x * 256 + threadIdx.x;
    if (i < n) {
        float s, c;
        fdn_sincos(x[i], &s, &c);
        sn[i] = s;
        cs[i] = c;
    }
}
}

extern "C" int fdn_sincos_f32(const float* x, float* sn, float* cs, long n, fdn_stream_t stream) {
    FDN_CHECK_ARG(x && sn && cs && n > 0 && n < (1L << 39));
    hipLaunchKernelGGL(sincos_kernel, dim3((unsigned)cdiv(n, 256)), dim3(256), 0, static_cast<hipStream_t>(stream), x, sn, cs, n);
    return fdn_launch_status();
}

extern "C" int fdn_rfft_rows(const float* in, float* out_c, long rows, int W, long out_row_bins, fdn_stream_t stream) {
    FDN_CHECK_ARG(in && out_c && rows > 0 && W >= 2 && W % 2 == 0 && (out_row_bins == 0 || (out_row_bins >= W / 2 + 1 && out_row_bins < (1L << 20))));
    const int pitch = out_row_bins ? (int)out_row_bins : W / 2 + 1;
    {
        int R1 = 0, P = 0;
        if (rows_plan(W, &R1, &P) && (reinterpret_cast<uintptr_t>(in) & 7) == 0) {
#define FDN_CALL(a, b) launch_rfft_rp<a, b>(in, out_c, rows, stream, pitch)
            FDN_ROWS_DISPATCH(FDN_CALL)
#undef FDN_CALL
        }
    }
    Route r;
    rows_route(W, true, &r);
    if (r.kind == FDN_FFT_REFUSED) return FDN_ERR_UNSUPPORTED;
    Plan p;
    if (!make_plan(W / 2, W, &p)) return FDN_ERR_UNSUPPORTED;
    Rader rd = {};
    if (r.kind == FDN_FFT_RADER && !get_rader(W / 2, &rd)) return FDN_ERR_LAUNCH;
    const int rpb = r.width;
    const size_t lds = r.lds;
    if (r.big) {
        if (int e = set_lds(rfft_rows_kernel<true>, lds)) return e;
        hipLaunchKernelGGL(rfft_rows_kernel<true>, dim3(cdiv(rows, rpb)), dim3(NT), lds, static_cast<hipStream_t>(stream), in,
                           reinterpret_cast<float2*>(out_c), W, rows, rpb, p, rd, pitch);
    } else {
        if (int e = set_lds(rfft_rows_kernel<false>, lds)) return e;
        hipLaunchKernelGGL(rfft_rows_kernel<false>, dim3(cdiv(rows, rpb)), dim3(NT), lds, static_cast<hipStream_t>(stream), in,
                           reinterpret_cast<float2*>(out_c), W, rows, rpb, p, rd, pitch);
    }
    return fdn_launch_status();
}

extern "C" int fdn_rfft_rows_ln(const float* x, const float* stats, const float* gamma, const float* beta, float* out_c, int B, int C,
                                int H, int W, long out_row_bins, fdn_stream_t stream) {
    FDN_CHECK_ARG(x && stats && gamma && beta && out_c && B > 0 && C > 0 && H > 0 && W >= 2 && W % 2 == 0);
    FDN_CHECK_ARG(out_row_bins == 0 || (out_row_bins >= W / 2 + 1 && out_row_bins < (1L << 20)));
    const int pitch = out_row_bins ? (int)out_row_bins : W / 2 + 1;
    FDN_CHECK_ARG((long)H * W < (1L << 28));
    int R1 = 0, P = 0;
    if (!rows_plan(W, &R1, &P) || (reinterpret_cast<uintptr_t>(x) & 7) != 0 || (reinterpret_cast<uintptr_t>(stats) & 7) != 0)
        return FDN_ERR_UNSUPPORTED;
    if ((long)B * 2 * H * W * 4 > 0x7FFFFFFFL) return FDN_ERR_UNSUPPORTED;
    const RowLN ln = {stats, gamma, beta, C, H};
    const long rows = (long)B * C * H;
#define FDN_CALL(a, b) launch_rfft_rp<a, b>(x, out_c, rows, stream, pitch, &ln)
    FDN_ROWS_DISPATCH(FDN_CALL)
#undef FDN_CALL
    return FDN_ERR_UNSUPPORTED;
}

extern "C" int fdn_irfft_rows(const float* in_c, long in_row_bins, long in_plane_bins, float* out, long planes, int H, int W,
                              float scale, const float* res, float alpha, fdn_stream_t stream) {
    FDN_CHECK_ARG(in_c && out && planes > 0 && H > 0 && W >= 2 && W % 2 == 0 && in_row_bins >= W / 2 + 1);
    {
        int R1 = 0, P = 0;
        if (rows_plan(W, &R1, &P) && ((reinterpret_cast<uintptr_t>(out) | reinterpret_cast<uintptr_t>(res)) & 7) == 0) {
#define FDN_CALL(a, b) launch_irfft_rp<a, b>(in_c, in_row_bins, in_plane_bins, out, planes, H, scale, res, alpha, stream)
            FDN_ROWS_DISPATCH(FDN_CALL)
#undef FDN_CALL
        }
    }
    Route r;
    rows_route(W, false, &r);
    if (r.kind == FDN_FFT_REFUSED) return FDN_ERR_UNSUPPORTED;
    Plan p;
    if (!make_plan(W / 2, W, &p)) return FDN_ERR_UNSUPPORTED;
    const int rpb = r.width;
    const size_t lds = r.lds;
    const long rows = planes * H;
    if (r.big) {
        if (int e = set_lds(irfft_rows_kernel<true>, lds)) return e;
        hipLaunchKernelGGL(irfft_rows_kernel<true>, dim3(cdiv(rows, rpb)), dim3(NT), lds, static_cast<hipStream_t>(stream),
                           reinterpret_cast<const float2*>(in_c), in_row_bins, (long)H, in_plane_bins, out, W, H, rows, rpb,
                           scale, res, alpha, p);
    } else {
        if (int e = set_lds(irfft_rows_kernel<false>, lds)) return e;
        hipLaunchKernelGGL(irfft_rows_kernel<false>, dim3(cdiv(rows, rpb)), dim3(NT), lds, static_cast<hipStream_t>(stream),
                           reinterpret_cast<const float2*>(in_c), in_row_bins, (long)H, in_plane_bins, out, W, H, rows, rpb,
                           scale, res, alpha, p);
    }
    return fdn_launch_status();
}

__global__ __launch_bounds__(256) void pack_guidance_kernel(const float* __restrict__ amp, const float* __restrict__ pha,
                                                            float4* __restrict__ out, int H, int Wf, int pitch, long total) {
    const long i = (long)blockIdx.x * 256 + threadIdx.x;
    if (i >= total) return;
    const long row = i / pitch;
    const int w = (int)(i - row * pitch);
    if (w >= Wf) {
        out[2 * i] = make_float4(0.f, 0.f, 0.f, 0.f);
        out[2 * i + 1] = make_float4(0.f, 0.f, 0.f, 0.f);
        return;
    }
    const long b = row / H, bins = (long)H * Wf, o = (row - b * H) * Wf + w;
    const float* ap = amp + b * 3 * bins + o;
    const float* pp = pha + b * 3 * bins + o;
    out[2 * i] = make_float4(ap[0], ap[bins], ap[2 * bins], pp[0]);
    out[2 * i + 1] = make_float4(pp[bins], pp[2 * bins], 0.f, 0.f);
}

extern "C" int fdn_pack_guidance(const float* amp, const float* pha, float* packed, int B, int H, int Wf, long row_bins,
                                 fdn_stream_t stream) {
    FDN_CHECK_ARG(amp && pha && packed && B > 0 && H > 0 && Wf > 0 && (row_bins == 0 || (row_bins >= Wf && row_bins < (1L << 20))));
    FDN_CHECK_ARG((reinterpret_cast<uintptr_t>(packed) & 15) == 0);
    const int pitch = row_bins ? (int)row_bins : Wf;
    const long total = (long)B * H * pitch;
    hipLaunchKernelGGL(pack_guidance_kernel, dim3((unsigned)cdiv(total, 256)), dim3(256), 0, static_cast<hipStream_t>(stream), amp,
                       pha, reinterpret_cast<float4*>(packed), H, Wf, pitch, total);
    return fdn_launch_status();
}

extern "C" int fdn_fft_cols_fcaffn(float* z, const float* guide, const float* wxa, const float* wxp, int B, int C, int H,
                                   int Wf, fdn_stream_t stream) {
    FDN_CHECK_ARG(z && guide && wxa && wxp && B > 0 && C > 0 && H > 0 && Wf > 0);
    FDN_CHECK_ARG((reinterpret_cast<uintptr_t>(guide) & 15) == 0);
    ColArgs a = {};
    a.z = reinterpret_cast<float2*>(z);
    a.H = H; a.Wf = Wf; a.C = C;
    a.guide = reinterpret_cast<const float4*>(guide); a.wxa = wxa; a.wxp = wxp;
    return launch_cols<COL_FCAFFN>(a, (long)B * C, stream);
}

extern "C" int fdn_fft_cols_fwd(const float* z, float* out_abs, float* out_ang, long planes, int H, int Wf, int rd_before,
                                int fix_real, fdn_stream_t stream) {
    FDN_CHECK_ARG(z && (out_abs || out_ang) && planes > 0 && H > 0 && Wf > 0);
    ColArgs a = {};
    a.z = reinterpret_cast<float2*>(const_cast<float*>(z));
    a.H = H; a.Wf = Wf; a.C = 1;
    a.out_abs = out_abs; a.out_ang = out_ang; a.rd_before = rd_before; a.fix_real = fix_real;
    return launch_cols<COL_FWD>(a, planes, stream);
}

extern "C" int fdn_fft_cols_inv_polar(const float* mag, const float* pha, int Hin, int Wfin, float* z_out, long planes, int H,
                                      int Wf, fdn_stream_t stream) {
    FDN_CHECK_ARG(mag && pha && z_out && planes > 0 && H > 0 && Wf > 0 && Hin >= H && Wfin >= Wf);
    ColArgs a = {};
    a.z = reinterpret_cast<float2*>(z_out);
    a.H = H; a.Wf = Wf; a.C = 1;
    a.in_mag = mag; a.in_pha = pha; a.Hin = Hin; a.Wfin = Wfin;
    return launch_cols<COL_INV_POLAR>(a, planes, stream);
}
```

### fdn-tip2025_amd/fdn_hip/__init__.py

```python
import ctypes
import os

import torch

_HERE = os.path.dirname(os.path.abspath(__file__))
_LIB_PATH = os.path.join(_HERE, "libfdn_hip.so")
_lib = None

ACT_NONE, ACT_LEAKY, ACT_RELU, ACT_SIGMOID, ACT_GELU = 0, 1, 2, 3, 4
PRO_NONE, PRO_LN, PRO_LN3_GATE, PRO_LN_MULADD = 0, 1, 2, 3
EPI_NONE, EPI_RES, EPI_MULADD = 0, 1, 2

c_fp = ctypes.c_void_p


class Conv1x1Desc(ctypes.Structure):
    _fields_ = [
        ("x", c_fp * 3), ("xbs", ctypes.c_long * 3), ("kseg", ctypes.c_int * 3),
        ("w", c_fp), ("bias", c_fp), ("out", c_fp), ("obs", ctypes.c_long),
        ("B", ctypes.c_int), ("K", ctypes.c_int), ("N", ctypes.c_int), ("P", ctypes.c_int),
        ("pro", ctypes.c_int), ("ln_group", ctypes.c_int),
        ("stats", c_fp), ("gamma", c_fp), ("beta", c_fp), ("xb", c_fp), ("xbbs", ctypes.c_long),
        ("act", ctypes.c_int), ("epi", ctypes.c_int),
        ("res", c_fp), ("rbs", ctypes.c_long), ("mul", c_fp), ("add", c_fp), ("mbs", ctypes.c_long),
        ("vec4", ctypes.c_int), ("stats_out", c_fp), ("x_bf16", ctypes.c_int), ("out_bf16", ctypes.c_int), ("wpk", c_fp),
    ]


class FdnHipError(RuntimeError):
    pass


ABI_VERSION = 20


def lib_path():
    return _LIB_PATH


def lib():
    global _lib
    if _lib is None:
        if not os.path.isfile(_LIB_PATH):
            raise ImportError(
                f"{_LIB_PATH} not found: build it with fdn-tip2025_amd/build.sh (hipcc --offload-arch=gfx950). "
                "The FDN path has no CPU fallback.")
        _lib = ctypes.CDLL(_LIB_PATH)
        _declare(_lib)
        if _lib.fdn_abi_version() != ABI_VERSION:
            v = _lib.fdn_abi_version()
            _lib = None
            raise ImportError(f"{_LIB_PATH} has ABI version {v}, this binding needs {ABI_VERSION}: rebuild with build.sh")
    return _lib


def _declare(l):
    from ._abi import PROTOTYPES
    kinds = {"P": ctypes.c_void_p, "I": ctypes.c_int, "L": ctypes.c_long, "F": ctypes.c_float, "DESC": ctypes.POINTER(Conv1x1Desc)}
    for name, (ret, sig) in PROTOTYPES.items():
        f = getattr(l, name)
        f.restype = ctypes.c_char_p if ret == "S" else ctypes.c_long if ret == "L" else ctypes.c_int
        f.argtypes = [kinds[k] for k in sig]


def check(code, what):
    if code != 0:
        raise FdnHipError(f"{what}: {lib().fdn_error_string(code).decode()} (code {code})")


def stream():
    return ctypes.c_void_p(torch.cuda.current_stream().cuda_stream)


_storage = "f32"


def set_storage_dtype(name):
    global _storage
    if name not in ("f32", "bf16"):
        raise ValueError(f"storage dtype must be 'f32' or 'bf16', got {name!r}")
    _storage = name


def storage_dtype():
    return _storage


_matrix_pipe = "bf16"


def set_matrix_pipe(name):
    global _matrix_pipe
    if name not in ("bf16", "f32", "bf16-narrow"):
        raise ValueError(f"matrix pipe must be 'bf16', 'f32' or 'bf16-narrow', got {name!r}")
    check(lib().fdn_set_matrix_pipe({"bf16": 0, "f32": 1, "bf16-narrow": 2}[name]), "fdn_set_matrix_pipe")
    _matrix_pipe = name


def matrix_pipe():
    return "bf16" if _matrix_pipe == "bf16-narrow" else _matrix_pipe


def matrix_pipe_mode():
    return _matrix_pipe


_cu_budgets = {}


def set_cu_budget(n):
    n = int(n)
    check(lib().fdn_set_cu_budget(n), "fdn_set_cu_budget")
    d = torch.cuda.current_device()
    if n:
        _cu_budgets[d] = n
    else:
# ... 25 lines not shown
```

### fdn-tip2025_amd/fdn_hip/_abi.py

```python

PROTOTYPES = {
    "fdn_abi_version": ("I", []),
    "fdn_error_string": ("S", ['I']),
    "fdn_set_matrix_pipe": ("I", ['I']),
    "fdn_bf16_mfma_launches": ("L", []),
    "fdn_set_cu_budget": ("I", ['I']),
    "fdn_conv1x1": ("I", ['DESC', 'P']),
    "fdn_conv1x1_pack_bytes": ("L", ['I', 'I', 'I']),
    "fdn_conv1x1_pack": ("I", ['P', 'I', 'I', 'I', 'P', 'P']),
    "fdn_chan_stats": ("I", ['P', 'L', 'P', 'I', 'I', 'I', 'I', 'P']),
    "fdn_layernorm_chan": ("I", ['P', 'P', 'P', 'P', 'I', 'I', 'I', 'P']),
    "fdn_fdsa_core": ("I", ['P', 'P', 'P', 'P', 'I', 'I', 'I', 'I', 'P']),
    "fdn_fdsa_pack": ("I", ['P', 'P', 'P', 'P', 'I', 'I', 'P']),
    "fdn_fdsa_fused": ("I", ['P', 'L', 'P', 'P', 'P', 'P', 'P', 'I', 'I', 'I', 'I', 'I', 'I', 'P']),
    "fdn_fdsa_full_pack_bytes": ("L", ['I', 'I']),
    "fdn_fdsa_full_pack": ("I", ['P', 'P', 'P', 'P', 'P', 'P', 'P', 'I', 'I', 'P']),
    "fdn_fdsa_full": ("I", ['P', 'L', 'P', 'P', 'P', 'P', 'P', 'P', 'P', 'I', 'I', 'I', 'I', 'I', 'P']),
    "fdn_fdsa_tail_pack_floats": ("L", ['I', 'I', 'I', 'I']),
    "fdn_fdsa_scratch_floats": ("L", ['I', 'I', 'I', 'I']),
    "fdn_fdsa_tail_pack": ("I", ['P', 'P', 'P', 'P', 'P', 'P', 'I', 'I', 'I', 'I', 'P']),
    "fdn_fdsa_fused_tail": ("I", ['P', 'L', 'P', 'P', 'P', 'P', 'P', 'P', 'P', 'P', 'P', 'P', 'I', 'I', 'I', 'I', 'I', 'I', 'I', 'P']),
    "fdn_fdsa_out": ("I", ['P', 'P', 'P', 'P', 'P', 'P', 'P', 'I', 'I', 'I', 'I', 'I', 'P']),
    "fdn_fdffn_mid": ("I", ['P', 'P', 'P', 'P', 'P', 'P', 'I', 'I', 'I', 'I', 'I', 'I', 'P']),
    "fdn_dwconv_gate": ("I", ['P', 'P', 'P', 'I', 'I', 'I', 'I', 'I', 'I', 'P']),
    "fdn_ffn_tail": ("I", ['P', 'P', 'P', 'P', 'P', 'P', 'I', 'I', 'I', 'I', 'I', 'I', 'I', 'P']),
    "fdn_dwconv3x3": ("I", ['P', 'P', 'P', 'I', 'I', 'I', 'I', 'I', 'P']),
    "fdn_fcaffn_in": ("I", ['P', 'P', 'P', 'P', 'P', 'P', 'P', 'P', 'P', 'P', 'P', 'P', 'P', 'P', 'I', 'I', 'I', 'I', 'P']),
    "fdn_fcaffn_in_pack_bytes": ("L", ['I']),
    "fdn_fcaffn_in_pack": ("I", ['P', 'P', 'P', 'P', 'P', 'I', 'P', 'P']),
    "fdn_fcaffn_in_packed": ("I", ['P', 'P', 'P', 'P', 'P', 'P', 'P', 'P', 'P', 'P', 'P', 'I', 'I', 'I', 'I', 'P']),
    "fdn_img_mod_maps": ("I", ['P', 'P', 'P', 'P', 'P', 'P', 'P', 'I', 'I', 'I', 'I', 'P']),
    "fdn_fft_prepare": ("I", ['I']),
    "fdn_sincos_f32": ("I", ['P', 'P', 'P', 'L', 'P']),
    "fdn_rfft_rows": ("I", ['P', 'P', 'L', 'I', 'L', 'P']),
    "fdn_rfft_rows_ln": ("I", ['P', 'P', 'P', 'P', 'P', 'I', 'I', 'I', 'I', 'L', 'P']),
    "fdn_irfft_rows": ("I", ['P', 'L', 'L', 'P', 'L', 'I', 'I', 'F', 'P', 'F', 'P']),
    "fdn_pack_guidance": ("I", ['P', 'P', 'P', 'I', 'I', 'I', 'L', 'P']),
    "fdn_fft_cols_fcaffn": ("I", ['P', 'P', 'P', 'P', 'I', 'I', 'I', 'I', 'P']),
    "fdn_fft_cols_fwd": ("I", ['P', 'P', 'P', 'L', 'I', 'I', 'I', 'I', 'P']),
    "fdn_fft_route": ("I", ['I', 'I', 'P', 'I']),
    "fdn_fft_cols_inv_polar": ("I", ['P', 'P', 'I', 'I', 'P', 'L', 'I', 'I', 'P']),
    "fdn_conv2d": ("I", ['P', 'P', 'P', 'P', 'P', 'I', 'I', 'I', 'I', 'I', 'I', 'I', 'I', 'I', 'I', 'I', 'F', 'P']),
    "fdn_upconv_gather": ("I", ['P', 'P', 'I', 'I', 'I', 'I', 'P']),
    "fdn_conv_transpose4x4s2": ("I", ['P', 'P', 'P', 'P', 'I', 'I', 'I', 'I', 'I', 'I', 'P']),
    "fdn_resample": ("I", ['P', 'P', 'L', 'I', 'I', 'I', 'I', 'P']),
    "fdn_dw1x1_pad1": ("I", ['P', 'P', 'P', 'P', 'I', 'I', 'I', 'I', 'P']),
    "fdn_avgpool3s2": ("I", ['P', 'P', 'L', 'I', 'I', 'P']),
    "fdn_global_avgpool": ("I", ['P', 'P', 'L', 'L', 'P']),
    "fdn_se_apply": ("I", ['P', 'P', 'P', 'P', 'L', 'L', 'P']),
    "fdn_spectral_mlp2": ("I", ['P', 'P', 'P', 'P', 'P', 'P', 'P', 'P', 'P', 'P', 'I', 'I', 'L', 'F', 'P']),
    "fdn_scale_batch": ("I", ['P', 'P', 'I', 'L', 'P']),
    "fdn_gamma_curve": ("I", ['P', 'P', 'P', 'F', 'L', 'P']),
    "fdn_pre_u8": ("I", ['P', 'P', 'I', 'I', 'I', 'I', 'I', 'I', 'P']),
    "fdn_post_u8": ("I", ['P', 'P', 'I', 'I', 'I', 'I', 'I', 'I', 'P']),
    "fdn_tiles_gather": ("I", ['P', 'P', 'P', 'I', 'I', 'I', 'I', 'I', 'I', 'P']),
    "fdn_tiles_merge": ("I", ['P', 'P', 'P', 'I', 'I', 'I', 'I', 'I', 'I', 'P']),
    "fdn_sse_max": ("I", ['P', 'P', 'L', 'P', 'P']),
    "fdn_ssim3d": ("I", ['P', 'P', 'I', 'I', 'I', 'F', 'P', 'P', 'P']),
    "fdn_y_channel": ("I", ['P', 'P', 'I', 'I', 'P']),
    "fdn_ssim2d": ("I", ['P', 'P', 'I', 'I', 'I', 'F', 'I', 'P', 'P', 'P']),
    "fdn_niqe_luma": ("I", ['P', 'P', 'I', 'I', 'I', 'I', 'I', 'I', 'I', 'I', 'I', 'P']),
    "fdn_niqe_mscn": ("I", ['P', 'P', 'I', 'I', 'I', 'I', 'P', 'P']),
    "fdn_niqe_features": ("I", ['P', 'P', 'I', 'I', 'I', 'I', 'P', 'I', 'P']),
    "fdn_lpips_prep_u8": ("I", ['P', 'P', 'I', 'I', 'I', 'I', 'P']),
    "fdn_lpips_prep_f32": ("I", ['P', 'P', 'I', 'I', 'I', 'I', 'P']),
    "fdn_maxpool2d": ("I", ['P', 'P', 'L', 'I', 'I', 'I', 'I', 'P']),
    "fdn_lpips_layer": ("I", ['P', 'P', 'P', 'I', 'I', 'I', 'I', 'I', 'P', 'P']),
    "fdn_pair_ssim3d_ws": ("L", ['I', 'I', 'I', 'I']),
    "fdn_pair_sse_u8": ("I", ['P', 'P', 'I', 'I', 'I', 'I', 'P', 'P']),
    "fdn_pair_ssim3d_u8": ("I", ['P', 'P', 'I', 'I', 'I', 'I', 'P', 'P', 'P', 'P', 'P', 'P']),
}

ARG_NAMES = {
    "fdn_abi_version": [],
    "fdn_error_string": ['code'],
    "fdn_set_matrix_pipe": ['mode'],
    "fdn_bf16_mfma_launches": [],
    "fdn_set_cu_budget": ['cus'],
    "fdn_conv1x1": ['d', 'stream'],
    "fdn_conv1x1_pack_bytes": ['N', 'K', 'ln3_E'],
    "fdn_conv1x1_pack": ['w', 'N', 'K', 'ln3_E', 'wpk', 'stream'],
    "fdn_chan_stats": ['x', 'xbs', 'stats', 'B', 'G', 'E', 'P', 'stream'],
    "fdn_layernorm_chan": ['x', 'gamma', 'beta', 'out', 'B', 'C', 'P', 'stream'],
    "fdn_fdsa_core": ['hidden', 'dw_w', 'fft_w', 'out', 'B', 'E', 'H', 'W', 'stream'],
    "fdn_fdsa_pack": ['w', 'gamma', 'beta', 'wpk', 'C', 'E', 'stream'],
    "fdn_fdsa_fused": ['x', 'xbs', 'stats', 'wpk', 'dw_w', 'fft_w', 'out', 'B', 'C', 'E', 'H', 'W', 'out_bf16', 'stream'],
    "fdn_fdsa_full_pack_bytes": ['C', 'E'],
    "fdn_fdsa_full_pack": ['w_hidden', 'gamma', 'beta', 'w_out', 'gamma3', 'beta3', 'wpk', 'C', 'E', 'stream'],
    "fdn_fdsa_full": ['x', 'xbs', 'stats', 'wpk', 'dw_w', 'fft_w', 'res', 'out', 'stats_out', 'B', 'C', 'E', 'H', 'W', 'stream'],
    "fdn_fdsa_tail_pack_floats": ['C', 'E', 'N', 'Hd'],
    "fdn_fdsa_scratch_floats": ['B', 'E', 'H', 'W'],
    "fdn_fdsa_tail_pack": ['w_out', 'gamma3', 'beta3', 'pin_w', 'pin_b', 'img', 'C', 'E', 'N', 'Hd', 'stream'],
    "fdn_fdsa_fused_tail": ['x', 'xbs', 'stats', 'wpk', 'dw_w', 'fft_w', 'tail_img', 'res', 'out', 'stats_out', 'scratch', 'h_out', 'B', 'C', 'E', 'H', 'W', 'Hd', 'h_bf16', 'stream'],
    "fdn_fdsa_out": ['o', 'w', 'gamma3', 'beta3', 'res', 'out', 'stats_out', 'B', 'E', 'N', 'P', 'o_bf16', 'stream'],
    "fdn_fdffn_mid": ['x', 'w0', 'w2', 'ffta', 'fftp', 'out', 'B', 'Hd', 'H', 'W', 'x_bf16', 'out_bf16', 'stream'],
    "fdn_dwconv_gate": ['x', 'w', 'out', 'B', 'C', 'H', 'W', 'x_bf16', 'out_bf16', 'stream'],
    "fdn_ffn_tail": ['y', 'dw_w', 'w', 'res', 'out', 'stats_out', 'B', 'C', 'N', 'H', 'W', 'y_bf16', 'form', 'stream'],
    "fdn_dwconv3x3": ['x', 'w', 'out', 'B', 'C', 'H', 'W', 'act', 'stream'],
    "fdn_fcaffn_in": ['xi', 'x1', 'stats1', 'gamma1', 'beta1', 'img', 'w', 'gamma', 'beta', 'w1_mul', 'w3_mul', 'w1_add', 'w3_add', 'out', 'B', 'C', 'H', 'W', 'stream'],
    "fdn_fcaffn_in_pack_bytes": ['C'],
    "fdn_fcaffn_in_pack": ['w', 'w1_mul', 'w3_mul', 'w1_add', 'w3_add', 'C', 'wpk', 'stream'],
    "fdn_fcaffn_in_packed": ['xi', 'stats_xi', 'x1', 'stats1', 'gamma1', 'beta1', 'img', 'wpk', 'gamma', 'beta', 'out', 'B', 'C', 'H', 'W', 'stream'],
    "fdn_img_mod_maps": ['img', 'w1_mul', 'w3_mul', 'w1_add', 'w3_add', 'mul', 'add', 'B', 'C', 'H', 'W', 'stream'],
    "fdn_fft_prepare": ['n'],
    "fdn_sincos_f32": ['x', 'sn', 'cs', 'n', 'stream'],
    "fdn_rfft_rows": ['in', 'out_c', 'rows', 'W', 'out_row_bins', 'stream'],
    "fdn_rfft_rows_ln": ['x', 'stats', 'gamma', 'beta', 'out_c', 'B', 'C', 'H', 'W', 'out_row_bins', 'stream'],
    "fdn_irfft_rows": ['in_c', 'in_row_bins', 'in_plane_bins', 'out', 'planes', 'H', 'W', 'scale', 'res', 'alpha', 'stream'],
    "fdn_pack_guidance": ['amp', 'pha', 'packed', 'B', 'H', 'Wf', 'row_bins', 'stream'],
    "fdn_fft_cols_fcaffn": ['z', 'guide', 'wxa', 'wxp', 'B', 'C', 'H', 'Wf', 'stream'],
    "fdn_fft_cols_fwd": ['z', 'out_abs', 'out_ang', 'planes', 'H', 'Wf', 'rd_before', 'fix_real', 'stream'],
    "fdn_fft_route": ['kind', 'n', 'desc', 'ndesc'],
    "fdn_fft_cols_inv_polar": ['mag', 'pha', 'Hin', 'Wfin', 'z_out', 'planes', 'H', 'Wf', 'stream'],
    "fdn_conv2d": ['x', 'w', 'bias', 'res', 'out', 'B', 'Cin', 'H', 'W', 'Cout', 'KH', 'KW', 'stride', 'pad', 'act', 'res_before_act', 'post_add', 'stream'],
    "fdn_upconv_gather": ['z', 'out', 'B', 'Cout', 'h', 'w', 'stream'],
    "fdn_conv_transpose4x4s2": ['x', 'w', 'bias', 'out', 'B', 'Cin', 'H', 'W', 'Cout', 'act', 'stream'],
    "fdn_resample": ['x', 'out', 'planes', 'H', 'W', 'mode', 'r', 'stream'],
    "fdn_dw1x1_pad1": ['x', 'w', 'bias', 'out', 'B', 'C', 'H', 'W', 'stream'],
    "fdn_avgpool3s2": ['x', 'out', 'planes', 'H', 'W', 'stream'],
    "fdn_global_avgpool": ['x', 'out', 'planes', 'P', 'stream'],
    "fdn_se_apply": ['y', 'gate', 'shortcut', 'out', 'planes', 'P', 'stream'],
    "fdn_spectral_mlp2": ['mag', 'pha', 'w1m', 'b1m', 'w2m', 'b2m', 'w1p', 'b1p', 'w2p', 'b2p', 'B', 'C', 'P', 'slope', 'stream'],
    "fdn_scale_batch": ['x', 'ratio', 'B', 'per_batch', 'stream'],
    "fdn_gamma_curve": ['x', 'i_map', 'out', 'scale', 'total', 'stream'],
    "fdn_pre_u8": ['img', 'out', 'B', 'h', 'w', 'H', 'W', 'swap_rb', 'stream'],
    "fdn_post_u8": ['res', 'out', 'B', 'h', 'w', 'H', 'W', 'swap_rb', 'stream'],
    "fdn_tiles_gather": ['x', 'tiles', 'ij', 'T', 'C', 'H', 'W', 'ch', 'cw', 'stream'],
    "fdn_tiles_merge": ['tiles', 'out', 'ij', 'T', 'C', 'H', 'W', 'ch', 'cw', 'stream'],
    "fdn_sse_max": ['a', 'b', 'n', 'out2', 'stream'],
    "fdn_ssim3d": ['a', 'b', 'C', 'H', 'W', 'max_value', 'ws', 'out_sum', 'stream'],
    "fdn_y_channel": ['img_bgr', 'out', 'H', 'W', 'stream'],
    "fdn_ssim2d": ['a', 'b', 'C', 'H', 'W', 'max_value', 'replicate_no_crop', 'ws', 'out_sum', 'stream'],
    "fdn_niqe_luma": ['src', 'out', 'B', 'C', 'Hs', 'Ws', 'top', 'left', 'H', 'W', 'mode', 'stream'],
    "fdn_niqe_mscn": ['src', 'mscn', 'B', 'H', 'W', 'half', 'window49', 'stream'],
    "fdn_niqe_features": ['mscn', 'feats', 'B', 'H', 'W', 'block', 'tables', 'ntab', 'stream'],
    "fdn_lpips_prep_u8": ['src', 'out', 'B', 'H', 'W', 'bgr', 'stream'],
    "fdn_lpips_prep_f32": ['x', 'out', 'B', 'H', 'W', 'from01', 'stream'],
    "fdn_maxpool2d": ['x', 'out', 'planes', 'H', 'W', 'k', 's', 'stream'],
    "fdn_lpips_layer": ['f', 'w', 'out', 'B', 'C', 'H', 'W', 'accumulate', 'ws', 'stream'],
    "fdn_pair_ssim3d_ws": ['B', 'h', 'w', 'crop'],
    "fdn_pair_sse_u8": ['a', 'b', 'B', 'h', 'w', 'crop', 'stats', 'stream'],
    "fdn_pair_ssim3d_u8": ['a', 'b', 'B', 'h', 'w', 'crop', 'stats', 'taps11', 'chmix9', 'ws', 'out3', 'stream'],
}
```

### fdn-tip2025_amd/fdn_hip/ops.py

```python
import ctypes

import torch

from . import (ACT_NONE, EPI_MULADD, EPI_NONE, EPI_RES, PRO_LN, PRO_LN3_GATE, PRO_LN_MULADD, PRO_NONE,
               Conv1x1Desc, FdnHipError, check, lib, storage_dtype, stream)

BF16 = torch.bfloat16
ERR_UNSUPPORTED = 4


def _planes(t, what, bf16_ok=False):
    if not t.is_cuda:
        raise FdnHipError(f"{what} must live on a ROCm device (got {t.device}); the FDN path has no CPU fallback")
    if t.dtype != torch.float32 and not (bf16_ok and t.dtype == BF16):
        raise FdnHipError(f"{what} must be float32{' or bfloat16 storage' if bf16_ok else ''} (got {t.dtype})")
    assert t.dim() == 4, what
    _, C, H, W = t.shape
    st = t.stride()
    if not (st[3] == 1 and st[2] == W and st[1] == H * W) and t.numel() > 0:
        raise FdnHipError(f"{what}: channel/row/column dims must be dense (strides {st})")
    return ctypes.c_void_p(t.data_ptr()), (st[0] if t.shape[0] > 1 else C * H * W)


def _flat(t, what, bf16_ok=False):
# ... 335 lines not shown

def dwconv3x3(x, w, act=ACT_NONE):
    B, C, H, W = x.shape
    out = torch.empty_like(x)
    check(lib().fdn_dwconv3x3(_flat(x, "x"), _flat(w, "w"), _flat(out, "out"), B, C, H, W, act, stream()), "fdn_dwconv3x3")
    return out


def img_mod_maps(img, w1_mul, w3_mul, w1_add, w3_add):
    B, _, H, W = img.shape
    C = w1_mul.shape[0]
    mul = torch.empty((B, C, H, W), device=img.device, dtype=torch.float32)
    add = torch.empty_like(mul)
    check(lib().fdn_img_mod_maps(_flat(img, "img"), _flat(w1_mul, "w1_mul"), _flat(w3_mul, "w3_mul"),
                                 _flat(w1_add, "w1_add"), _flat(w3_add, "w3_add"), _flat(mul, "mul"), _flat(add, "add"),
                                 B, C, H, W, stream()), "fdn_img_mod_maps")
    return mul, add


FCAFFN_IN_C = (32, 64)


def fcaffn_in(xi, x1, img, w, gamma, beta, w1_mul, w3_mul, w1_add, w3_add, x1_ln=None):
    B, C, H, W = xi.shape
    out = torch.empty_like(xi)
    st1, g1, b1 = x1_ln if x1_ln is not None else (None, None, None)
    check(lib().fdn_fcaffn_in(_flat(xi, "xi"), _flat(x1, "x1"), _flat(st1, "stats1"), _flat(g1, "gamma1"), _flat(b1, "beta1"),
                              _flat(img, "img"), _flat(w, "w"), _flat(gamma, "gamma"),
                              _flat(beta, "beta"), _flat(w1_mul, "w1_mul"), _flat(w3_mul, "w3_mul"), _flat(w1_add, "w1_add"),
                              _flat(w3_add, "w3_add"), _flat(out, "out"), B, C, H, W, stream()), "fdn_fcaffn_in")
    return out


FCAFFN_PACKED_MIN_C = 96


def fcaffn_in_pack(w, w1_mul, w3_mul, w1_add, w3_add):
    C = w.shape[0]
    wpk = torch.empty(lib().fdn_fcaffn_in_pack_bytes(C), device=w.device, dtype=torch.uint8)
    check(lib().fdn_fcaffn_in_pack(_flat(w.reshape(C, C), "w"), _flat(w1_mul, "w1_mul"), _flat(w3_mul, "w3_mul"), _flat(w1_add, "w1_add"),
                                   _flat(w3_add, "w3_add"), C, ctypes.c_void_p(wpk.data_ptr()), stream()), "fdn_fcaffn_in_pack")
    return wpk


def fcaffn_in_packed(xi, stats_xi, x1, img, wpk, gamma, beta, x1_ln=None):
    B, C, H, W = xi.shape
    out = torch.empty_like(xi)
    st1, g1, b1 = x1_ln if x1_ln is not None else (None, None, None)
    check(lib().fdn_fcaffn_in_packed(_flat(xi, "xi"), _flat(stats_xi, "stats_xi"), _flat(x1, "x1"), _flat(st1, "stats1"), _flat(g1, "gamma1"),
                                     _flat(b1, "beta1"), _flat(img, "img"), ctypes.c_void_p(wpk.data_ptr()), _flat(gamma, "gamma"),
                                     _flat(beta, "beta"), _flat(out, "out"), B, C, H, W, stream()), "fdn_fcaffn_in_packed")
    return out


RS_BILINEAR_HALF, RS_BILINEAR_X2, RS_NEAREST_HALF, RS_NEAREST_X2, RS_PIXEL_UNSHUFFLE = 0, 1, 2, 3, 4


def spec_pitch(Wf):
    return (Wf + 15) // 16 * 16


FFT_ROUTES = ("refused", "planned", "inplace", "pingpong", "rader")
FFT_MAX_STAGES = 16
FFT_ROWS, FFT_IROWS, FFT_COLS = 0, 1, 2


def fft_route(kind, n):
    desc = (ctypes.c_int * (5 + 2 * FFT_MAX_STAGES))()
    check(lib().fdn_fft_route(int(kind), int(n), desc, len(desc)), "fdn_fft_route")
    nst = desc[4]
    radices = tuple(desc[5 + i] for i in range(nst))
    return {"route": FFT_ROUTES[desc[0]], "big": desc[1], "width": desc[2], "rader": desc[3], "radices": radices,
            "gather": tuple(r for i, r in enumerate(radices) if desc[5 + FFT_MAX_STAGES + i])}


def rfft_rows(x, pitch=None):
    W = x.shape[-1]
    rows = x.numel() // W
    out = torch.empty(x.shape[:-1] + (pitch or W // 2 + 1, 2), device=x.device, dtype=torch.float32)
    check(lib().fdn_rfft_rows(_flat(x, "x"), _flat(out, "out"), ctypes.c_long(rows), W, ctypes.c_long(pitch or 0), stream()), "fdn_rfft_rows")
    return out


ROWS_PLANNED_W = tuple(2 * r * p for r in (20, 30) for p in (32, 16, 8)) + (608, 304) + (1120, 560, 280)


def rows_ln_ok(x):
    B, _, H, W = x.shape
    return W in ROWS_PLANNED_W and B * 2 * H * W * 4 <= 0x7FFFFFFF


def rfft_rows_ln(x, stats, gamma, beta, pitch=None):
    B, C, H, W = x.shape
    out = torch.empty((B, C, H, pitch or W // 2 + 1, 2), device=x.device, dtype=torch.float32)
    check(lib().fdn_rfft_rows_ln(_flat(x, "x"), _flat(stats, "stats"), _flat(gamma, "gamma"), _flat(beta, "beta"), _flat(out, "out"),
                                 B, C, H, W, ctypes.c_long(pitch or 0), stream()), "fdn_rfft_rows_ln")
    return out


def irfft_rows(z, H, W, scale, res=None, alpha=0.0, out=None):
    B, C, Hin, Wfin, _ = z.shape
    if out is None:
        out = torch.empty((B, C, H, W), device=z.device, dtype=torch.float32)
    check(lib().fdn_irfft_rows(_flat(z, "z"), ctypes.c_long(Wfin), ctypes.c_long(Hin * Wfin), _flat(out, "out"),
                               ctypes.c_long(B * C), H, W, ctypes.c_float(scale), _flat(res, "res"),
                               ctypes.c_float(alpha), stream()), "fdn_irfft_rows")
    return out


def sincos(x):
    sn, cs = torch.empty_like(x), torch.empty_like(x)
    check(lib().fdn_sincos_f32(_flat(x, "x"), _flat(sn, "sn"), _flat(cs, "cs"), ctypes.c_long(x.numel()), stream()), "fdn_sincos_f32")
    return sn, cs


def pack_guidance(amp, pha, pitch=None):
    B, _, H, Wf = amp.shape
    pitch = pitch or Wf
    cached = getattr(amp, "_fdn_packed", None)
    if cached is not None and cached[0] is pha and cached[1].shape[2] == pitch:
        return cached[1]
    out = torch.empty((B, H, pitch, 8), device=amp.device, dtype=torch.float32)
    check(lib().fdn_pack_guidance(_flat(amp, "amp"), _flat(pha, "pha"), _flat(out, "packed"), B, H, Wf, ctypes.c_long(pitch), stream()),
          "fdn_pack_guidance")
    amp._fdn_packed = (pha, out)
    return out


def fft_cols_fcaffn(z, amp, pha, wxa, wxp):
    B, C, H, Wf, _ = z.shape
    guide = pack_guidance(amp, pha, pitch=Wf)
    check(lib().fdn_fft_cols_fcaffn(_flat(z, "z"), _flat(guide, "guide"), _flat(wxa, "wxa"), _flat(wxp, "wxp"), B, C, H, Wf,
                                    stream()), "fdn_fft_cols_fcaffn")
    return z


def fft_cols_fwd(z, want_abs, want_ang, rd_before=False, fix_real=True):
    B, C, H, Wf, _ = z.shape
    oa = torch.empty((B, C, H, Wf), device=z.device, dtype=torch.float32) if want_abs else None
    og = torch.empty((B, C, H, Wf), device=z.device, dtype=torch.float32) if want_ang else None
    check(lib().fdn_fft_cols_fwd(_flat(z, "z"), _flat(oa, "abs"), _flat(og, "ang"), ctypes.c_long(B * C), H, Wf,
                                 int(rd_before), int(fix_real), stream()), "fdn_fft_cols_fwd")
    return oa, og


def fft_cols_inv_polar(mag, pha, H, Wf):
    B, C, Hin, Wfin = mag.shape
    z = torch.empty((B, C, H, Wf, 2), device=mag.device, dtype=torch.float32)
    check(lib().fdn_fft_cols_inv_polar(_flat(mag, "mag"), _flat(pha, "pha"), Hin, Wfin, _flat(z, "z"),
                                       ctypes.c_long(B * C), H, Wf, stream()), "fdn_fft_cols_inv_polar")
    return z


def conv2d(x, w, bias=None, stride=1, pad=0, act=ACT_NONE, res=None, res_before_act=False, post_add=0.0):
    B, Cin, H, W = x.shape
    Cout, _, KH, KW = w.shape
    OH, OW = (H + 2 * pad - KH) // stride + 1, (W + 2 * pad - KW) // stride + 1
    out = torch.empty((B, Cout, OH, OW), device=x.device, dtype=torch.float32)
    check(lib().fdn_conv2d(_flat(x, "x"), _flat(w, "w"), _flat(bias, "bias"), _flat(res, "res"), _flat(out, "out"),
                           B, Cin, H, W, Cout, KH, KW, stride, pad, act, int(res_before_act), ctypes.c_float(post_add),
                           stream()), "fdn_conv2d")
    return out


def maxpool2d(x, k, s):
    B, C, H, W = x.shape
    if H < k or W < k:
        raise FdnHipError(f"maxpool2d: {H}x{W} is smaller than the {k}x{k} window")
    out = torch.empty((B, C, (H - k) // s + 1, (W - k) // s + 1), device=x.device, dtype=torch.float32)
    check(lib().fdn_maxpool2d(_flat(x, "x"), _flat(out, "out"), ctypes.c_long(B * C), H, W, k, s, stream()), "fdn_maxpool2d")
    return out


def conv_transpose4x4s2(x, w, bias, act):
    B, Cin, H, W = x.shape
    Cout = w.shape[1]
    out = torch.empty((B, Cout, 2 * H, 2 * W), device=x.device, dtype=torch.float32)
    check(lib().fdn_conv_transpose4x4s2(_flat(x, "x"), _flat(w, "w"), _flat(bias, "bias"), _flat(out, "out"),
                                        B, Cin, H, W, Cout, act, stream()), "fdn_conv_transpose4x4s2")
    return out


AFF_MULTIRES = True
UPCONV_GATHER = True


def upsample_conv3x3(x, w, cache=None):
    B, C, h, w_ = x.shape
    Cout = w.shape[0]
    build = lambda: w.detach().permute(2, 3, 0, 1).reshape(9 * Cout, C).contiguous()
    wr = cache[0].get(cache[1] + ":taps", [w], build) if cache is not None else build()
    z = conv1x1(x, wr, cache=None if cache is None else (cache[0], cache[1] + ":z"))
    out = torch.empty((B, Cout, 2 * h, 2 * w_), device=x.device, dtype=torch.float32)
    check(lib().fdn_upconv_gather(_flat(z, "z"), _flat(out, "out"), B, Cout, h, w_, stream()), "fdn_upconv_gather")
    return out


def resample(x, mode, r=1):
    B, C, H, W = x.shape
    if mode in (RS_BILINEAR_HALF, RS_NEAREST_HALF):
        shp = (B, C, H // 2, W // 2)
    elif mode in (RS_BILINEAR_X2, RS_NEAREST_X2):
        shp = (B, C, 2 * H, 2 * W)
    else:
        shp = (B, C * r * r, H // r, W // r)
    out = torch.empty(shp, device=x.device, dtype=torch.float32)
    check(lib().fdn_resample(_flat(x, "x"), _flat(out, "out"), ctypes.c_long(B * C), H, W, mode, r, stream()),
          "fdn_resample")
    return out


def dw1x1_pad1(x, w, bias):
    B, C, H, W = x.shape
    out = torch.empty((B, C, H + 2, W + 2), device=x.device, dtype=torch.float32)
    check(lib().fdn_dw1x1_pad1(_flat(x, "x"), _flat(w, "w"), _flat(bias, "bias"), _flat(out, "out"), B, C, H, W,
                               stream()), "fdn_dw1x1_pad1")
    return out


def avgpool3s2(x):
    B, C, H, W = x.shape
    out = torch.empty((B, C, (H - 1) // 2 + 1, (W - 1) // 2 + 1), device=x.device, dtype=torch.float32)
    check(lib().fdn_avgpool3s2(_flat(x, "x"), _flat(out, "out"), ctypes.c_long(B * C), H, W, stream()), "fdn_avgpool3s2")
    return out


def global_avgpool(x):
    B, C, H, W = x.shape
    out = torch.empty((B, C, 1, 1), device=x.device, dtype=torch.float32)
    check(lib().fdn_global_avgpool(_flat(x, "x"), _flat(out, "out"), ctypes.c_long(B * C), ctypes.c_long(H * W),
                                   stream()), "fdn_global_avgpool")
    return out


def se_apply(y, gate, shortcut):
    B, C, H, W = y.shape
    out = torch.empty_like(y)
    check(lib().fdn_se_apply(_flat(y, "y"), _flat(gate, "gate"), _flat(shortcut, "shortcut"), _flat(out, "out"),
                             ctypes.c_long(B * C), ctypes.c_long(H * W), stream()), "fdn_se_apply")
    return out


def scale_batch_(x, ratio):
    B = x.shape[0]
# ... 24 lines not shown
```

### fdn-tip2025_amd/fdn_hip/pipeline.py

```python
import collections
import contextlib
import gc
import os

import torch

from . import storage_dtype

_streams = {}
CAPTURE_MODE = "thread_local"
MULTISTREAM_ENV = "FDN_HIP_ALLOW_MULTISTREAM"


@contextlib.contextmanager
def _capturing(graph):
    was = gc.isenabled()
    gc.disable()
    try:
        with torch.cuda.graph(graph, capture_error_mode=CAPTURE_MODE):
            yield
    finally:
        if was:
            gc.enable()


def _check_streams(n_streams):
    if n_streams > 1 and os.environ.get(MULTISTREAM_ENV) != "1":
        raise RuntimeError(
            f"fdn_hip: n_streams={n_streams} refused - kernels of different HIP streams that share the GPU with a bf16-MFMA "
            f"kernel return wrong rows on MI355X / ROCm 7.2 (DESIGN.md 4.7).  Use one stream per GPU, or set {MULTISTREAM_ENV}=1 "
            "for experiments (to bisect, call fdn_hip.set_matrix_pipe('f32') first: the fp32-MFMA forms of every matrix product).")


def _get_streams(device, n):
    key = (device.index if device.index is not None else torch.cuda.current_device(), n)
    if key not in _streams:
        _streams[key] = [torch.cuda.Stream(device=device) for _ in range(n)]
    return _streams[key]


def forward_streams(net, lpnet, x, n_streams=1, keep=None):
    _check_streams(n_streams)
    B = x.shape[0]
    if n_streams <= 1 or B < n_streams:
        with torch.no_grad():
            ratio = lpnet(x)
            if keep is not None:
                keep["ratio"] = ratio
            return net(x, ratio_i=ratio, device=x.device)[0]
    cur = torch.cuda.current_stream(x.device)
    streams = _get_streams(x.device, n_streams)
    bounds = [round(i * B / n_streams) for i in range(n_streams + 1)]
    outs = []
    for i, s in enumerate(streams):
        s.wait_stream(cur)
        with torch.cuda.stream(s), torch.no_grad():
            xi = x[bounds[i]:bounds[i + 1]].contiguous()
            xi.record_stream(s)
            outs.append(net(xi, ratio_i=lpnet(xi), device=x.device)[0])
    for s, o in zip(streams, outs):
        cur.wait_stream(s)
        o.record_stream(cur)
    return torch.cat(outs)


def weights_signature(*modules):
    from . import _cu_budgets, matrix_pipe_mode, ops
    ps = [p for m in modules for p in list(m.parameters()) + list(m.buffers())]
    return (storage_dtype(), matrix_pipe_mode(), tuple(sorted(_cu_budgets.items())), bool(ops.FDSA_FULL), int(ops.FDSA_FULL_MAX_C), bool(ops.FDSA_TAIL), bool(ops.FDSA_TAIL_PIN), int(ops.FDSA_TAIL_PIN_MAX_C), str(ops.FFN_TAIL_MODE), bool(ops.SPECTRAL_MLP_FUSED), bool(ops.GEMM_OWN_STATS), bool(ops.UPCONV_GATHER), bool(ops.AFF_MULTIRES),
            len(ps), sum(p._version for p in ps), sum(p.data_ptr() & 0xFFFFFFFF for p in ps))


class GraphedForward:

    MAX_GRAPHS = 4

    def __init__(self, net, lpnet, warmup=2):
        self.net, self.lpnet, self.warmup = net, lpnet, warmup
        self._graphs = collections.OrderedDict()
        self._seen = collections.OrderedDict()

    def __deepcopy__(self, memo):
        return None

    def __getstate__(self):
        return {"warmup": self.warmup}

    def __setstate__(self, st):
        self.net = self.lpnet = None
        self.warmup = st.get("warmup", 2)
        self._graphs = collections.OrderedDict()
        self._seen = collections.OrderedDict()

    def _weights_signature(self):
        return weights_signature(self.net, self.lpnet)

    def _eager(self, x):
        with torch.no_grad():
            return self.net(x, ratio_i=self.lpnet(x), device=x.device)[0]

    def _capture(self, x):
        static_x = x.clone()
        s = torch.cuda.Stream(device=x.device)
        s.wait_stream(torch.cuda.current_stream(x.device))
        with torch.cuda.stream(s), torch.no_grad():
            for _ in range(self.warmup):
                self.net(static_x, ratio_i=self.lpnet(static_x), device=x.device)
        torch.cuda.current_stream(x.device).wait_stream(s)
        g = torch.cuda.CUDAGraph()
        with _capturing(g), torch.no_grad():
            static_out = self.net(static_x, ratio_i=self.lpnet(static_x), device=x.device)[0]
        return g, static_x, static_out, self._weights_signature()

    def __call__(self, x):
        key = (tuple(x.shape), x.device.index)
        hit = self._graphs.get(key)
        if hit is not None and hit[3] != self._weights_signature():
            del self._graphs[key]
            hit = None
        if hit is None:
            if key not in self._seen:
                self._seen[key] = True
                while len(self._seen) > 64:
                    self._seen.popitem(last=False)
                return self._eager(x)
            hit = self._capture(x)
            self._graphs[key] = hit
            while len(self._graphs) > self.MAX_GRAPHS:
                self._graphs.popitem(last=False)
        self._graphs.move_to_end(key)
        g, static_x, static_out, _ = hit
        static_x.copy_(x)
        g.replay()
        return static_out


class GraphedStep:

    def __init__(self, net, lpnet, n_streams=1):
        _check_streams(n_streams)
        self.net, self.lpnet, self.n = net, lpnet, n_streams
        self._g = None
        self._key = None
        self.captures = 0

    def __call__(self, x):
        key = (tuple(x.shape), x.device.index, weights_signature(self.net, self.lpnet))
        if self._g is None or self._key != key:
            self._key = key
            self.captures += 1
            self._x = x.clone()
            for _ in range(2):
# ... 27 lines not shown
```

### include/fdn_hip.h

```cpp
#ifndef FDN_HIP_H
#define FDN_HIP_H

#ifdef __cplusplus
extern "C" {
#endif

typedef void* fdn_stream_t;

enum { FDN_OK = 0, FDN_ERR_ARG = 1, FDN_ERR_LAUNCH = 2, FDN_ERR_WORKSPACE = 3, FDN_ERR_UNSUPPORTED = 4 };
enum { FDN_ACT_NONE = 0, FDN_ACT_LEAKY = 1, FDN_ACT_RELU = 2, FDN_ACT_SIGMOID = 3, FDN_ACT_GELU = 4 };
enum { FDN_PRO_NONE = 0, FDN_PRO_LN = 1, FDN_PRO_LN3_GATE = 2, FDN_PRO_LN_MULADD = 3 };
enum { FDN_EPI_NONE = 0, FDN_EPI_RES = 1, FDN_EPI_MULADD = 2 };
enum { FDN_RS_BILINEAR_HALF = 0, FDN_RS_BILINEAR_X2 = 1, FDN_RS_NEAREST_HALF = 2, FDN_RS_NEAREST_X2 = 3, FDN_RS_PIXEL_UNSHUFFLE = 4 };

int fdn_abi_version(void);
const char* fdn_error_string(int code);
int fdn_set_matrix_pipe(int mode);
long fdn_bf16_mfma_launches(void);
int fdn_set_cu_budget(int cus);

typedef struct fdn_conv1x1_desc {
    const float* x[3];
    long xbs[3];
    int kseg[3];
// ... 1 lines not shown
    const float* bias;
    float* out;
    long obs;
    int B, K, N, P;
    int pro, ln_group;
    const float* stats;
    const float* gamma;
    const float* beta;
    const float* xb;
    long xbbs;
    int act, epi;
    const float* res;
    long rbs;
    const float* mul;
    const float* add;
    long mbs;
    int vec4;
    float* stats_out;
    int x_bf16;
    int out_bf16;
    const void* wpk;
} fdn_conv1x1_desc;
int fdn_conv1x1(const fdn_conv1x1_desc* d, fdn_stream_t stream);

long fdn_conv1x1_pack_bytes(int N, int K, int ln3_E);
int fdn_conv1x1_pack(const float* w, int N, int K, int ln3_E, void* wpk, fdn_stream_t stream);

int fdn_chan_stats(const float* x, long xbs, float* stats, int B, int G, int E, int P, fdn_stream_t stream);
int fdn_layernorm_chan(const float* x, const float* gamma, const float* beta, float* out, int B, int C, int P,
                       fdn_stream_t stream);

int fdn_fdsa_core(const float* hidden, const float* dw_w, const float* fft_w, float* out, int B, int E, int H, int W,
                  fdn_stream_t stream);

int fdn_fdsa_pack(const float* w, const float* gamma, const float* beta, float* wpk, int C, int E, fdn_stream_t stream);
int fdn_fdsa_fused(const float* x, long xbs, const float* stats, const float* wpk, const float* dw_w, const float* fft_w,
                   void* out, int B, int C, int E, int H, int W, int out_bf16, fdn_stream_t stream);

long fdn_fdsa_full_pack_bytes(int C, int E);
int fdn_fdsa_full_pack(const float* w_hidden, const float* gamma, const float* beta, const float* w_out, const float* gamma3,
                       const float* beta3, void* wpk, int C, int E, fdn_stream_t stream);
int fdn_fdsa_full(const float* x, long xbs, const float* stats, const void* wpk, const float* dw_w, const float* fft_w,
                  const float* res, float* out, float* stats_out, int B, int C, int E, int H, int W, fdn_stream_t stream);

long fdn_fdsa_tail_pack_floats(int C, int E, int N, int Hd);
long fdn_fdsa_scratch_floats(int B, int E, int H, int W);
int fdn_fdsa_tail_pack(const float* w_out, const float* gamma3, const float* beta3, const float* pin_w, const float* pin_b, float* img, int C, int E,
                       int N, int Hd, fdn_stream_t stream);
int fdn_fdsa_fused_tail(const float* x, long xbs, const float* stats, const float* wpk, const float* dw_w, const float* fft_w,
                        const float* tail_img, const float* res, float* out, float* stats_out, float* scratch, void* h_out, int B, int C,
                        int E, int H, int W, int Hd, int h_bf16, fdn_stream_t stream);

int fdn_fdsa_out(const void* o, const float* w, const float* gamma3, const float* beta3, const float* res, float* out,
                 float* stats_out, int B, int E, int N, int P, int o_bf16, fdn_stream_t stream);

int fdn_fdffn_mid(const void* x, const float* w0, const float* w2, const float* ffta, const float* fftp, void* out,
                  int B, int Hd, int H, int W, int x_bf16, int out_bf16, fdn_stream_t stream);

int fdn_dwconv_gate(const void* x, const float* w, void* out, int B, int C, int H, int W, int x_bf16, int out_bf16,
                    fdn_stream_t stream);

int fdn_ffn_tail(const void* y, const float* dw_w, const float* w, const float* res, float* out, float* stats_out, int B,
                 int C, int N, int H, int W, int y_bf16, int form, fdn_stream_t stream);

int fdn_dwconv3x3(const float* x, const float* w, float* out, int B, int C, int H, int W, int act, fdn_stream_t stream);

int fdn_fcaffn_in(const float* xi, const float* x1, const float* stats1, const float* gamma1, const float* beta1, const float* img,
                  const float* w, const float* gamma, const float* beta, const float* w1_mul, const float* w3_mul,
                  const float* w1_add, const float* w3_add, float* out, int B, int C, int H, int W, fdn_stream_t stream);

long fdn_fcaffn_in_pack_bytes(int C);
int fdn_fcaffn_in_pack(const float* w, const float* w1_mul, const float* w3_mul, const float* w1_add, const float* w3_add, int C,
                       void* wpk, fdn_stream_t stream);
int fdn_fcaffn_in_packed(const float* xi, const float* stats_xi, const float* x1, const float* stats1, const float* gamma1,
                         const float* beta1, const float* img, const void* wpk, const float* gamma, const float* beta, float* out,
                         int B, int C, int H, int W, fdn_stream_t stream);

int fdn_img_mod_maps(const float* img, const float* w1_mul, const float* w3_mul, const float* w1_add,
                     const float* w3_add, float* mul, float* add, int B, int C, int H, int W, fdn_stream_t stream);

int fdn_fft_prepare(int n);
int fdn_sincos_f32(const float* x, float* sn, float* cs, long n, fdn_stream_t stream);
int fdn_rfft_rows(const float* in, float* out_c, long rows, int W, long out_row_bins, fdn_stream_t stream);
int fdn_rfft_rows_ln(const float* x, const float* stats, const float* gamma, const float* beta, float* out_c, int B, int C, int H,
                     int W, long out_row_bins, fdn_stream_t stream);
int fdn_irfft_rows(const float* in_c, long in_row_bins, long in_plane_bins, float* out, long planes, int H, int W,
                   float scale, const float* res, float alpha, fdn_stream_t stream);
int fdn_pack_guidance(const float* amp, const float* pha, float* packed, int B, int H, int Wf, long row_bins, fdn_stream_t stream);
int fdn_fft_cols_fcaffn(float* z, const float* guide, const float* wxa, const float* wxp, int B, int C, int H, int Wf,
                        fdn_stream_t stream);
int fdn_fft_cols_fwd(const float* z, float* out_abs, float* out_ang, long planes, int H, int Wf, int rd_before,
                     int fix_real, fdn_stream_t stream);
enum { FDN_FFT_REFUSED = 0, FDN_FFT_PLANNED = 1, FDN_FFT_INPLACE = 2, FDN_FFT_PINGPONG = 3, FDN_FFT_RADER = 4 };
enum { FDN_FFT_MAX_STAGES = 16, FDN_FFT_ROUTE_DESC = 5 + 2 * FDN_FFT_MAX_STAGES };
int fdn_fft_route(int kind, int n, int* desc, int ndesc);
int fdn_fft_cols_inv_polar(const float* mag, const float* pha, int Hin, int Wfin, float* z_out, long planes, int H, int Wf,
                           fdn_stream_t stream);

int fdn_conv2d(const float* x, const float* w, const float* bias, const float* res, float* out, int B, int Cin, int H,
               int W, int Cout, int KH, int KW, int stride, int pad, int act, int res_before_act, float post_add,
               fdn_stream_t stream);
int fdn_upconv_gather(const float* z, float* out, int B, int Cout, int h, int w, fdn_stream_t stream);
int fdn_conv_transpose4x4s2(const float* x, const float* w, const float* bias, float* out, int B, int Cin, int H, int W,
                            int Cout, int act, fdn_stream_t stream);
int fdn_resample(const float* x, float* out, long planes, int H, int W, int mode, int r, fdn_stream_t stream);
int fdn_dw1x1_pad1(const float* x, const float* w, const float* bias, float* out, int B, int C, int H, int W,
                   fdn_stream_t stream);
int fdn_avgpool3s2(const float* x, float* out, long planes, int H, int W, fdn_stream_t stream);
int fdn_global_avgpool(const float* x, float* out, long planes, long P, fdn_stream_t stream);
int fdn_se_apply(const float* y, const float* gate, const float* shortcut, float* out, long planes, long P,
                 fdn_stream_t stream);
int fdn_spectral_mlp2(float* mag, float* pha, const float* w1m, const float* b1m, const float* w2m, const float* b2m, const float* w1p,
                      const float* b1p, const float* w2p, const float* b2p, int B, int C, long P, float slope, fdn_stream_t stream);
int fdn_scale_batch(float* x, const float* ratio, int B, long per_batch, fdn_stream_t stream);
int fdn_gamma_curve(const float* x, const float* i_map, float* out, float scale, long total, fdn_stream_t stream);

int fdn_pre_u8(const unsigned char* img, float* out, int B, int h, int w, int H, int W, int swap_rb, fdn_stream_t stream);
int fdn_post_u8(const float* res, unsigned char* out, int B, int h, int w, int H, int W, int swap_rb, fdn_stream_t stream);

int fdn_tiles_gather(const float* x, float* tiles, const int* ij, int T, int C, int H, int W, int ch, int cw, fdn_stream_t stream);
int fdn_tiles_merge(const float* tiles, float* out, const int* ij, int T, int C, int H, int W, int ch, int cw, fdn_stream_t stream);

int fdn_sse_max(const float* a, const float* b, long n, double* out2, fdn_stream_t stream);
int fdn_ssim3d(const float* a, const float* b, int C, int H, int W, float max_value, float* ws, double* out_sum,
               fdn_stream_t stream);
int fdn_y_channel(const float* img_bgr, float* out, int H, int W, fdn_stream_t stream);
int fdn_ssim2d(const float* a, const float* b, int C, int H, int W, float max_value, int replicate_no_crop, double* ws,
               double* out_sum, fdn_stream_t stream);
int fdn_niqe_luma(const float* src, float* out, int B, int C, int Hs, int Ws, int top, int left, int H, int W, int mode,
                  fdn_stream_t stream);
int fdn_niqe_mscn(const float* src, float* mscn, int B, int H, int W, int half, const double* window49, fdn_stream_t stream);
int fdn_niqe_features(const float* mscn, double* feats, int B, int H, int W, int block, const double* tables, int ntab,
                      fdn_stream_t stream);
enum { FDN_LPIPS_PARTS = 1024 };
int fdn_lpips_prep_u8(const unsigned char* src, float* out, int B, int H, int W, int bgr, fdn_stream_t stream);
int fdn_lpips_prep_f32(const float* x, float* out, int B, int H, int W, int from01, fdn_stream_t stream);
int fdn_maxpool2d(const float* x, float* out, long planes, int H, int W, int k, int s, fdn_stream_t stream);
int fdn_lpips_layer(const float* f, const float* w, double* out, int B, int C, int H, int W, int accumulate, double* ws,
                    fdn_stream_t stream);
enum { FDN_PAIR_PARTS = 256 };
long fdn_pair_ssim3d_ws(int B, int h, int w, int crop);
int fdn_pair_sse_u8(const unsigned char* a, const unsigned char* b, int B, int h, int w, int crop, long* stats, fdn_stream_t stream);
int fdn_pair_ssim3d_u8(const unsigned char* a, const unsigned char* b, int B, int h, int w, int crop, const long* stats,
                       const double* taps11, const double* chmix9, double* ws, double* out3, fdn_stream_t stream);

#ifdef __cplusplus
}
#endif
#endif
```

Measured before the change: 27.93 images/s.

## Fuse ratio scaling, pad1 depthwise, and LN stats into FFT and conv kernels

Adds a register-blocked 3x3 conv kernel where each thread computes a run of 4 (or 2) output pixels. The patch-embed conv gets an optional variant that emits per-pixel LayerNorm statistics in the same pass. The per-batch ratio scaling is folded into the inverse row FFT, and the depthwise pad-1 1x1 conv is folded into the forward row FFT. Each fusion removes a separate full-tensor read/write pass and a kernel launch, at the cost of more specialised kernels and extra conditional dispatch paths.

```diff
diff --git a/fdn-tip2025_amd/basicsr/models/archs/FDN_arch.py b/fdn-tip2025_amd/basicsr/models/archs/FDN_arch.py
--- a/fdn-tip2025_amd/basicsr/models/archs/FDN_arch.py
+++ b/fdn-tip2025_amd/basicsr/models/archs/FDN_arch.py
@@ -234,7 +234,7 @@
         self.proj = nn.Conv2d(in_c, embed_dim, kernel_size=3, stride=1, padding=1, bias=bias)
 
     def forward(self, x):
-        return ops.conv2d(x, _w(self.proj.weight), pad=1)
+        return ops.conv2d(x, _w(self.proj.weight), pad=1, want_stats=True)
 
 
 class Downsample(nn.Module):
@@ -340,8 +340,9 @@
     return ops.conv1x1(t, _w(seq[2].weight), _w(seq[2].bias))
 
 
-def _spectral_mlps(y, process1, process2, H, W):
-    z = ops.rfft_rows(y)
+def _spectral_mlps(y, process1, process2, H, W, z=None):
+    if z is None:
+        z = ops.rfft_rows(y)
     mag, pha = ops.fft_cols_fwd(z, True, True, rd_before=False, fix_real=True)
     if ops.SPECTRAL_MLP_FUSED and mag.shape[1] in ops.SPECTRAL_MLP_C:
         ops.spectral_mlp2(mag, pha, _w(process1[0].weight), _w(process1[0].bias), _w(process1[2].weight), _w(process1[2].bias),
@@ -359,11 +360,11 @@
         self.process1 = nn.Sequential(nn.Conv2d(nc, nc, 1, 1, 0), nn.LeakyReLU(0.1), nn.Conv2d(nc, nc, 1, 1, 0))
         self.process2 = nn.Sequential(nn.Conv2d(nc, nc, 1, 1, 0), nn.LeakyReLU(0.1), nn.Conv2d(nc, nc, 1, 1, 0))
 
-    def forward(self, x, skip_gain=1.0):
+    def forward(self, x, skip_gain=1.0, ratio=None):
         _, _, H, W = x.shape
         y = ops.conv1x1(x, _w(self.fpre.weight), _w(self.fpre.bias))
         zz = _spectral_mlps(y, self.process1, self.process2, H, W)
-        return ops.irfft_rows(zz, H, W, 2.0 / (H * W), res=x, alpha=skip_gain)
+        return ops.irfft_rows(zz, H, W, 2.0 / (H * W), res=x, alpha=skip_gain, ratio=ratio)
 
 
 class ProcessBlock(nn.Module):
@@ -372,8 +373,8 @@
         self.frequency_process = FreBlock(in_nc)
         self.cat = nn.Conv2d(in_nc, in_nc, 1, 1, 0)
 
-    def forward(self, x):
-        return self.frequency_process(x, skip_gain=2.0)
+    def forward(self, x, ratio=None):
+        return self.frequency_process(x, skip_gain=2.0, ratio=ratio)
 
 
 class fourier_fuse(nn.Module):
@@ -402,8 +403,10 @@
 
     def _rest(self, y):
         H, W = y.shape[-2:]
-        y = ops.dw1x1_pad1(y, _w(self.fpre[1].weight), _w(self.fpre[1].bias))
-        zz = _spectral_mlps(y, self.process1, self.process2, H, W)
+        z = ops.rfft_rows_pad1(y, _w(self.fpre[1].weight), _w(self.fpre[1].bias))
+        if z is None:
+            y = ops.dw1x1_pad1(y, _w(self.fpre[1].weight), _w(self.fpre[1].bias))
+        zz = _spectral_mlps(y, self.process1, self.process2, H, W, z=z)
         xo = ops.irfft_rows(zz, H, W, 2.0 / (H * W))
         return ops.conv2d(xo, _w(self.fourier_out.weight), _w(self.fourier_out.bias), pad=1)
 
@@ -432,8 +435,7 @@
         self.FAM2 = FAM(c * 2)
 
     def _stem(self, seq, x, ratio):
-        t = seq[1](ops.conv1x1(x, _w(seq[0].weight), _w(seq[0].bias)))
-        return ops.scale_batch_(t, ratio) if self.apply_ratio else t
+        return seq[1](ops.conv1x1(x, _w(seq[0].weight), _w(seq[0].bias)), ratio=ratio if self.apply_ratio else None)
 
     def forward(self, x, ratio):
         x_2 = ops.resample(x, ops.RS_NEAREST_HALF)
diff --git a/fdn-tip2025_amd/basicsr/models/archs/fdnlol24_arch.py b/fdn-tip2025_amd/basicsr/models/archs/fdnlol24_arch.py
--- a/fdn-tip2025_amd/basicsr/models/archs/fdnlol24_arch.py
+++ b/fdn-tip2025_amd/basicsr/models/archs/fdnlol24_arch.py
@@ -20,9 +20,10 @@
         self.frequency_process = FreBlock(in_nc)
         self.cat = nn.Conv2d(in_nc, in_nc, 1, 1, 0)
 
-    def forward(self, x):
+    def forward(self, x, ratio=None):
         y = self.frequency_process(x, skip_gain=1.0)
-        return ops.conv1x1(y, _w(self.cat.weight), _w(self.cat.bias), res=x)
+        y = ops.conv1x1(y, _w(self.cat.weight), _w(self.cat.bias), res=x)
+        return y if ratio is None else ops.scale_batch_(y, ratio)
 
 
 class fourier_multi_scale_gamma2(MAR_archa):
diff --git a/fdn-tip2025_amd/csrc/capi.hip b/fdn-tip2025_amd/csrc/capi.hip
--- a/fdn-tip2025_amd/csrc/capi.hip
+++ b/fdn-tip2025_amd/csrc/capi.hip
@@ -1,7 +1,7 @@
 #include "common.hpp"
 
 #include <atomic>
-extern "C" int fdn_abi_version(void) { return 20; }
+extern "C" int fdn_abi_version(void) { return 21; }
 
 static std::atomic<int> g_matrix_pipe_mode{0};
 extern "C" int fdn_set_matrix_pipe(int mode) {
diff --git a/fdn-tip2025_amd/csrc/convs.hip b/fdn-tip2025_amd/csrc/convs.hip
--- a/fdn-tip2025_amd/csrc/convs.hip
+++ b/fdn-tip2025_amd/csrc/convs.hip
@@ -119,6 +119,153 @@
     if (lds > 64 * 1024) return FDN_ERR_UNSUPPORTED;
     hipLaunchKernelGGL((conv3x3_direct_kernel<S, OCB_>), dim3(cdiv((long)a.OH * a.OW, 256), cdiv(a.Cout, OCB_), a.B), dim3(256),
                        lds, s, a);
+    return fdn_launch_status();
+}
+
+template <int S, int OCB_, int NG, bool STATS>
+__global__ __launch_bounds__(256, ((S == 1 ? 4 : 2) * OCB_ >= 64 ? 2 : (S == 1 ? 4 : 2) * OCB_ >= 48 ? 3 : 4)) void conv3x3_run_kernel(ConvArgs a, float* __restrict__ stats) {
+    static_assert(OCB_ % 4 == 0, "weight rows are read as 16-byte words");
+    constexpr int RUN = S == 1 ? 4 : 2;
+    constexpr int WC = S * RUN + 2;
+    extern __shared__ __attribute__((aligned(16))) float wl[];
+    unsigned bx, by, bz;
+    fdn_xcd_block3(bx, by, bz);
+    const int oc0 = by * (OCB_ * NG), b = bz;
+    for (int i = threadIdx.x; i < NG * a.Cin * 9 * OCB_; i += 256) {
+        const int o = i % OCB_, t = (i / OCB_) % 9, ci = (i / (OCB_ * 9)) % a.Cin, g = i / (OCB_ * 9 * a.Cin);
+        const int oc = oc0 + g * OCB_ + o;
+        wl[i] = oc < a.Cout ? a.w[((long)oc * a.Cin + ci) * 9 + t] : 0.f;
+    }
+    __syncthreads();
+    const int OWq = a.OW / RUN;
+    const unsigned idx = bx * 256u + threadIdx.x;
+    const bool live = idx < (unsigned)(a.OH * OWq);
+    const int oy = live ? (int)(idx / (unsigned)OWq) : 0, ox0 = live ? ((int)idx - oy * OWq) * RUN : 0;
+    const int iy0 = oy * S - 1, ix0 = ox0 * S;
+    int roff[3];
+    bool rok[3];
+#pragma unroll
+    for (int r = 0; r < 3; ++r) {
+        const int iy = iy0 + r;
+        rok[r] = live && iy >= 0 && iy < a.H;
+        roff[r] = min(max(iy, 0), a.H - 1) * a.W;
+    }
+    const bool lok = ix0 > 0, rgt = ix0 + 4 < a.W;
+    const int cl = max(ix0 - 1, 0), cr = min(ix0 + 4, a.W - 1);
+    const long hw = (long)a.H * a.W;
+    const float* xc = a.x + (long)b * a.Cin * hw;
+    const long OP = (long)a.OH * a.OW, op = (long)oy * a.OW + ox0;
+    auto fetch = [&](const float* pl, float (&v)[3][WC]) __attribute__((always_inline)) {
+#pragma unroll
+        for (int r = 0; r < 3; ++r) {
+            const float4 m = *reinterpret_cast<const float4*>(pl + roff[r] + ix0);
+            v[r][0] = pl[roff[r] + cl];
+            v[r][1] = m.x; v[r][2] = m.y; v[r][3] = m.z; v[r][4] = m.w;
+            v[r][5] = S == 1 ? pl[roff[r] + cr] : 0.f;
+        }
+    };
+    float x0[RUN] = {}, s1[RUN] = {}, s2[RUN] = {};
+#pragma unroll 1
+    for (int g = 0; g < NG; ++g) {
+        const int ocg = oc0 + g * OCB_;
+        const int nvalid = min(OCB_, a.Cout - ocg);
+        if (nvalid <= 0) break;
+        float win[3][WC], nxt[3][WC];
+        float acc[RUN][OCB_];
+#pragma unroll
+        for (int j = 0; j < RUN; ++j)
+#pragma unroll
+            for (int o = 0; o < OCB_; ++o) acc[j][o] = 0.f;
+        fetch(xc, nxt);
+        for (int ci = 0; ci < a.Cin; ++ci) {
+#pragma unroll
+            for (int r = 0; r < 3; ++r) {
+                win[r][0] = (rok[r] && lok) ? nxt[r][0] : 0.f;
+#pragma unroll
+                for (int c = 1; c < 5; ++c) win[r][c] = rok[r] ? nxt[r][c] : 0.f;
+                win[r][5] = (rok[r] && rgt) ? nxt[r][5] : 0.f;
+            }
+            fetch(xc + (long)min(ci + 1, a.Cin - 1) * hw, nxt);
+            const float* wc = wl + (g * a.Cin + ci) * 9 * OCB_;
+#pragma unroll
+            for (int t = 0; t < 9; ++t) {
+                const float* wp = wc + t * OCB_;
+#pragma unroll
+                for (int o = 0; o < OCB_; ++o) {
+                    const float ww = wp[o];
+#pragma unroll
+                    for (int j = 0; j < RUN; ++j) acc[j][o] = fmaf(win[t / 3][j * S + t % 3], ww, acc[j][o]);
+                }
+            }
+        }
+        if (live) {
+#pragma unroll
+            for (int o = 0; o < OCB_; ++o) {
+                if (o < nvalid) {
+                    const int oc = ocg + o;
+                    const long oi = ((long)b * a.Cout + oc) * OP + op;
+                    float v[RUN], rv[RUN];
+#pragma unroll
+                    for (int j = 0; j < RUN; ++j) rv[j] = a.res ? a.res[oi + j] : 0.f;
+#pragma unroll
+                    for (int j = 0; j < RUN; ++j) {
+                        v[j] = acc[j][o] + (a.bias ? a.bias[oc] : 0.f);
+                        if (a.res && a.res_before_act) v[j] += rv[j];
+                        v[j] = apply_act(v[j], a.act);
+                        if (a.res && !a.res_before_act) v[j] += rv[j];
+                        v[j] = v[j] + a.post_add;
+                    }
+                    if (RUN == 4) *reinterpret_cast<float4*>(a.out + oi) = make_float4(v[0], v[1], v[2], v[3]);
+                    else *reinterpret_cast<float2*>(a.out + oi) = make_float2(v[0], v[1]);
+                    if (STATS) {
+#pragma unroll
+                        for (int j = 0; j < RUN; ++j) {
+                            if (o == 0 && g == 0) x0[j] = v[j];
+                            else {
+                                const float dlt = v[j] - x0[j];
+                                s1[j] += dlt;
+                                s2[j] += dlt * dlt;
+                            }
+                        }
+                    }
+                }
+            }
+        }
+    }
+    if (STATS && live) {
+        const float inv = 1.0f / (float)a.Cout;
+        float mu[RUN], rs[RUN];
+#pragma unroll
+        for (int j = 0; j < RUN; ++j) {
+            const float md = s1[j] * inv;
+            const float var = fmaxf(s2[j] * inv - md * md, 0.f);
+            mu[j] = x0[j] + md;
+            rs[j] = 1.0f / sqrtf(var + 1e-5f);
+        }
+        float* dst = stats + (long)b * 2 * OP + op;
+        if (RUN == 4) {
+            *reinterpret_cast<float4*>(dst) = make_float4(mu[0], mu[1], mu[2], mu[3]);
+            *reinterpret_cast<float4*>(dst + OP) = make_float4(rs[0], rs[1], rs[2], rs[3]);
+        } else {
+            *reinterpret_cast<float2*>(dst) = make_float2(mu[0], mu[1]);
+            *reinterpret_cast<float2*>(dst + OP) = make_float2(rs[0], rs[1]);
+        }
+    }
+}
+
+inline bool conv3x3_run_ok(const ConvArgs& a, const float* stats) {
+    const uintptr_t al = reinterpret_cast<uintptr_t>(a.x) | reinterpret_cast<uintptr_t>(a.out) | reinterpret_cast<uintptr_t>(a.res) |
+                         reinterpret_cast<uintptr_t>(stats);
+    return a.W % 4 == 0 && (al & 15) == 0 && (long)a.H * a.W < (1L << 31);
+}
+
+template <int S, int OCB_, int NG = 1, bool STATS = false>
+int launch_conv3x3_run(const ConvArgs& a, float* stats, hipStream_t s) {
+    constexpr int RUN = S == 1 ? 4 : 2;
+    const size_t lds = (size_t)NG * a.Cin * 9 * OCB_ * sizeof(float);
+    if (lds > 64 * 1024) return FDN_ERR_UNSUPPORTED;
+    hipLaunchKernelGGL((conv3x3_run_kernel<S, OCB_, NG, STATS>), dim3(cdiv((long)a.OH * (a.OW / RUN), 256), cdiv(a.Cout, OCB_ * NG), a.B), dim3(256),
+                       lds, s, a, stats);
     return fdn_launch_status();
 }
 
@@ -547,9 +694,10 @@
 
 }
 
-extern "C" int fdn_conv2d(const float* x, const float* w, const float* bias, const float* res, float* out, int B, int Cin,
-                          int H, int W, int Cout, int KH, int KW, int stride, int pad, int act, int res_before_act,
-                          float post_add, fdn_stream_t stream) {
+namespace {
+int conv2d_impl(const float* x, const float* w, const float* bias, const float* res, float* out, int B, int Cin, int H, int W, int Cout,
+                int KH, int KW, int stride, int pad, int act, int res_before_act, float post_add, float* stats, int one_pixel,
+                fdn_stream_t stream) {
     FDN_CHECK_ARG(x && w && out && B > 0 && Cin > 0 && Cout > 0 && H > 0 && W > 0 && KH > 0 && KW > 0 && stride > 0 && pad >= 0);
     ConvArgs a;
     a.x = x; a.w = w; a.bias = bias; a.res = res; a.out = out;
@@ -561,8 +709,20 @@
     hipStream_t s = static_cast<hipStream_t>(stream);
     if (KH == 3 && KW == 3 && pad == 1 && (stride == 1 || stride == 2)) {
         int rc = FDN_ERR_UNSUPPORTED;
+        if (stats) {
+            if (stride == 1 && Cout == 32 && !one_pixel && conv3x3_run_ok(a, stats) && B < 65536) return launch_conv3x3_run<1, 16, 2, true>(a, stats, s);
+            return FDN_ERR_UNSUPPORTED;
+        }
         if (stride == 1 && Cin % 8 == 0 && Cin >= 16 && Cout >= 16 && !fdn_matrix_pipe_f32()) {
             rc = fdn_conv3x3_mfma(x, w, bias, res, out, B, Cin, H, W, Cout, act, res_before_act, post_add, s);
+            if (rc != FDN_ERR_UNSUPPORTED) return rc;
+        }
+        if (!one_pixel && conv3x3_run_ok(a, nullptr) && Cout <= 48) {
+            rc = FDN_ERR_UNSUPPORTED;
+            if (stride == 2) rc = Cout % 24 == 0 ? launch_conv3x3_run<2, 24>(a, nullptr, s) : Cout <= 8 ? launch_conv3x3_run<2, 8>(a, nullptr, s) : launch_conv3x3_run<2, 16>(a, nullptr, s);
+            else if (Cout <= 4) { if ((long)B * a.OH * a.OW >= (4L << 20)) rc = launch_conv3x3_run<1, 4>(a, nullptr, s); }
+            else if (Cout <= 8) rc = launch_conv3x3_run<1, 8>(a, nullptr, s);
+            else if (Cout <= 12) rc = launch_conv3x3_run<1, 12>(a, nullptr, s);
             if (rc != FDN_ERR_UNSUPPORTED) return rc;
         }
         if (stride == 2) rc = Cout <= 8 ? launch_conv3x3_direct<2, 8>(a, s) : launch_conv3x3_direct<2, 16>(a, s);
@@ -575,12 +735,26 @@
             if (rc != FDN_ERR_UNSUPPORTED) return rc;
         }
     }
-    if (KH == 7 && KW == 7 && stride == 2 && pad == 3 && Cin == 3 && Cout == 16) {
+    if (KH == 7 && KW == 7 && stride == 2 && pad == 3 && Cin == 3 && Cout == 16 && !stats) {
         hipLaunchKernelGGL((conv7x7s2_kernel<3, 16>), dim3(cdiv(a.OW, 32), cdiv(a.OH, 8), B), dim3(256), 0, s, a);
         return fdn_launch_status();
     }
+    if (stats) return FDN_ERR_UNSUPPORTED;
     hipLaunchKernelGGL(conv2d_kernel, dim3(cdiv((long)a.OH * a.OW, 256), cdiv(Cout, OCB), B), dim3(256), 0, s, a);
     return fdn_launch_status();
+}
+}
+
+extern "C" int fdn_conv2d(const float* x, const float* w, const float* bias, const float* res, float* out, int B, int Cin,
+                          int H, int W, int Cout, int KH, int KW, int stride, int pad, int act, int res_before_act,
+                          float post_add, fdn_stream_t stream) {
+    return conv2d_impl(x, w, bias, res, out, B, Cin, H, W, Cout, KH, KW, stride, pad, act, res_before_act, post_add, nullptr, 0, stream);
+}
+
+extern "C" int fdn_conv2d_ex(const float* x, const float* w, const float* bias, const float* res, float* out, int B, int Cin,
+                             int H, int W, int Cout, int KH, int KW, int stride, int pad, int act, int res_before_act,
+                             float post_add, float* stats_out, int one_pixel, fdn_stream_t stream) {
+    return conv2d_impl(x, w, bias, res, out, B, Cin, H, W, Cout, KH, KW, stride, pad, act, res_before_act, post_add, stats_out, one_pixel, stream);
 }
 
 extern "C" int fdn_conv_transpose4x4s2(const float* x, const float* w, const float* bias, float* out, int B, int Cin, int H,
diff --git a/fdn-tip2025_amd/csrc/fft2d.hip b/fdn-tip2025_amd/csrc/fft2d.hip
--- a/fdn-tip2025_amd/csrc/fft2d.hip
+++ b/fdn-tip2025_amd/csrc/fft2d.hip
@@ -406,9 +406,14 @@
     }
 }
 
+struct RowPad {
+    const float* w; const float* b;
+    int C, H, W;
+};
+
 template <bool BIG>
 __global__ __launch_bounds__(NT) void rfft_rows_kernel(const float* __restrict__ in, float2* __restrict__ out, int W, long R,
-                                                       int rpb, const Plan p, const Rader rd, int pitch) {
+                                                       int rpb, const Plan p, const Rader rd, int pitch, const RowPad pp) {
     extern __shared__ __attribute__((aligned(16))) unsigned char smem[];
     const int M = W / 2, Wf = M + 1;
     float2* A = reinterpret_cast<float2*>(smem);
@@ -424,7 +429,41 @@
         constexpr int U = 8;
         const float2* in2 = reinterpret_cast<const float2*>(in + row0 * W);
         const int tot = rpb * M, live = nrow * M;
-        if (M % 2 == 0 && (reinterpret_cast<uintptr_t>(in) & 15) == 0) {
+        if (pp.w) {
+            long* prow = reinterpret_cast<long*>(Bf);
+            float2* pwb = reinterpret_cast<float2*>(prow + rpb);
+            if ((int)threadIdx.x < rpb) {
+                const long row = row0 + min((int)threadIdx.x, nrow - 1);
+                const long plane = row / (pp.H + 2);
+                const int hr = (int)(row - plane * (pp.H + 2)), c = (int)(plane % pp.C);
+                prow[threadIdx.x] = (hr >= 1 && hr <= pp.H) ? (plane * pp.H + (hr - 1)) * pp.W : -1L;
+                pwb[threadIdx.x] = make_float2(pp.w[c], pp.b[c]);
+            }
+            __syncthreads();
+            const float r_M = 1.0f / (float)M;
+            for (int base = threadIdx.x; base < tot; base += NT * U) {
+                float xa[U], xb[U];
+#pragma unroll
+                for (int u = 0; u < U; ++u) {
+                    const int idx = min(base + NT * u, tot - 1);
+                    const int s_ = fdiv(idx, r_M), m = idx - s_ * M;
+                    const float* src = in + max(prow[s_], 0L);
+                    xa[u] = src[min(max(2 * m - 1, 0), pp.W - 1)];
+                    xb[u] = src[min(2 * m, pp.W - 1)];
+                }
+#pragma unroll
+                for (int u = 0; u < U; ++u) {
+                    const int idx = base + NT * u;
+                    if (idx >= tot) continue;
+                    const int s_ = fdiv(idx, r_M), m = idx - s_ * M;
+                    const bool rowin = prow[s_] >= 0;
+                    const float2 wb = pwb[s_];
+                    const float v0 = __fadd_rn((rowin && m >= 1) ? __fmul_rn(wb.x, xa[u]) : 0.f, wb.y);
+                    const float v1 = __fadd_rn((rowin && 2 * m + 1 <= pp.W) ? __fmul_rn(wb.x, xb[u]) : 0.f, wb.y);
+                    A[idx] = idx < live ? make_float2(v0, v1) : make_float2(0.f, 0.f);
+                }
+            }
+        } else if (M % 2 == 0 && (reinterpret_cast<uintptr_t>(in) & 15) == 0) {
             const float4* in4 = reinterpret_cast<const float4*>(in2);
             float4* A4 = reinterpret_cast<float4*>(A);
             const int tot4 = tot / 2, live4 = live / 2;
@@ -522,7 +561,7 @@
 __global__ __launch_bounds__(NT) void irfft_rows_kernel(const float2* __restrict__ in, long in_ws, long in_plane_rows,
                                                         long in_plane_stride, float* __restrict__ out, int W, int H, long R,
                                                         int rpb, float scale, const float* __restrict__ res, float alpha,
-                                                        const Plan p) {
+                                                        const float* __restrict__ ratio, long img_rows, const Plan p) {
     extern __shared__ __attribute__((aligned(16))) unsigned char smem[];
     const int M = W / 2;
     float2* A = reinterpret_cast<float2*>(smem);
@@ -593,6 +632,10 @@
                         v.x = fmaf(alpha, r[u].x, v.x); v.y = fmaf(alpha, r[u].y, v.y);
                         v.z = fmaf(alpha, r[u].z, v.z); v.w = fmaf(alpha, r[u].w, v.w);
                     }
+                    if (ratio) {
+                        const float q = ratio[(row0 + (2 * idx) / M) / img_rows];
+                        v.x *= q; v.y *= q; v.z *= q; v.w *= q;
+                    }
                     out4[idx] = v;
                 }
             }
@@ -613,6 +656,11 @@
                 if (res2) {
                     v.x = fmaf(alpha, r[u].x, v.x);
                     v.y = fmaf(alpha, r[u].y, v.y);
+                }
+                if (ratio) {
+                    const float q = ratio[(row0 + idx / M) / img_rows];
+                    v.x *= q;
+                    v.y *= q;
                 }
                 out2[idx] = v;
             }
@@ -1303,6 +1351,7 @@
 __global__ __launch_bounds__(256, 2) void irfft_rows_rp_kernel(const float2* __restrict__ in, long in_ws, long in_plane_stride,
                                                                float* __restrict__ out, int H, long R, float scale,
                                                                const float* __restrict__ res, float alpha,
+                                                               const float* __restrict__ ratio, long img_rows,
                                                                const float2* __restrict__ tab) {
     typedef RowPlan<R1, P> L;
     constexpr int M = L::M, W = L::W, RW = L::RW, CJ = L::CJ, PS = L::PS, RS = L::RS, NJ = L::NJ;
@@ -1394,10 +1443,12 @@
             const unsigned voff = (unsigned)(rw * W + 2 * n2) * 4u;
             f2 r[R1];
             if (res) sfor<0, R1>([&](auto n1) { r[decltype(n1)::value] = bload2(rr, voff, (unsigned)(decltype(n1)::value * P * 8)); });
+            const float q = ratio ? ratio[(row0 + rw) / img_rows] : 1.0f;
             sfor<0, R1>([&](auto n1) {
                 constexpr int N1 = decltype(n1)::value;
                 f2 x = u[N1] * scale;
                 if (res) x += alpha * r[N1];
+                if (ratio) x = x * q;
                 bstore2(x, ro, voff, (unsigned)(N1 * P * 8));
             });
         }
@@ -1458,14 +1509,14 @@
 
 template <int R1, int P>
 int launch_irfft_rp(const float* in_c, long in_row_bins, long in_plane_bins, float* out, long planes, int H, float scale,
-                    const float* res, float alpha, fdn_stream_t stream) {
+                    const float* res, float alpha, const float* ratio, long img_rows, fdn_stream_t stream) {
     typedef RowPlan<R1, P> L;
     const float2* tab = get_table_rows_rp(R1, P);
     if (!tab) return FDN_ERR_LAUNCH;
     if (int e = set_lds(irfft_rows_rp_kernel<R1, P>, L::lds)) return e;
     const long rows = planes * H;
     hipLaunchKernelGGL((irfft_rows_rp_kernel<R1, P>), dim3(cdiv(rows, L::RW)), dim3(256), L::lds, static_cast<hipStream_t>(stream),
-                       reinterpret_cast<const float2*>(in_c), in_row_bins, in_plane_bins, out, H, rows, scale, res, alpha, tab);
+                       reinterpret_cast<const float2*>(in_c), in_row_bins, in_plane_bins, out, H, rows, scale, res, alpha, ratio, img_rows, tab);
     return fdn_launch_status();
 }
 
@@ -1561,12 +1612,13 @@
     return fdn_launch_status();
 }
 
-extern "C" int fdn_rfft_rows(const float* in, float* out_c, long rows, int W, long out_row_bins, fdn_stream_t stream) {
+namespace {
+int rfft_rows_impl(const float* in, float* out_c, long rows, int W, long out_row_bins, const RowPad& pp, fdn_stream_t stream) {
     FDN_CHECK_ARG(in && out_c && rows > 0 && W >= 2 && W % 2 == 0 && (out_row_bins == 0 || (out_row_bins >= W / 2 + 1 && out_row_bins < (1L << 20))));
     const int pitch = out_row_bins ? (int)out_row_bins : W / 2 + 1;
     {
         int R1 = 0, P = 0;
-        if (rows_plan(W, &R1, &P) && (reinterpret_cast<uintptr_t>(in) & 7) == 0) {
+        if (!pp.w && rows_plan(W, &R1, &P) && (reinterpret_cast<uintptr_t>(in) & 7) == 0) {
 #define FDN_CALL(a, b) launch_rfft_rp<a, b>(in, out_c, rows, stream, pitch)
             FDN_ROWS_DISPATCH(FDN_CALL)
 #undef FDN_CALL
@@ -1581,16 +1633,30 @@
     if (r.kind == FDN_FFT_RADER && !get_rader(W / 2, &rd)) return FDN_ERR_LAUNCH;
     const int rpb = r.width;
     const size_t lds = r.lds;
+    if (pp.w && (rpb > NT || (size_t)rpb * 16 > (size_t)rpb * (W / 2) * sizeof(float2))) return FDN_ERR_UNSUPPORTED;
     if (r.big) {
         if (int e = set_lds(rfft_rows_kernel<true>, lds)) return e;
         hipLaunchKernelGGL(rfft_rows_kernel<true>, dim3(cdiv(rows, rpb)), dim3(NT), lds, static_cast<hipStream_t>(stream), in,
-                           reinterpret_cast<float2*>(out_c), W, rows, rpb, p, rd, pitch);
+                           reinterpret_cast<float2*>(out_c), W, rows, rpb, p, rd, pitch, pp);
     } else {
         if (int e = set_lds(rfft_rows_kernel<false>, lds)) return e;
         hipLaunchKernelGGL(rfft_rows_kernel<false>, dim3(cdiv(rows, rpb)), dim3(NT), lds, static_cast<hipStream_t>(stream), in,
-                           reinterpret_cast<float2*>(out_c), W, rows, rpb, p, rd, pitch);
+                           reinterpret_cast<float2*>(out_c), W, rows, rpb, p, rd, pitch, pp);
     }
     return fdn_launch_status();
+}
+}
+
+extern "C" int fdn_rfft_rows(const float* in, float* out_c, long rows, int W, long out_row_bins, fdn_stream_t stream) {
+    return rfft_rows_impl(in, out_c, rows, W, out_row_bins, RowPad{nullptr, nullptr, 0, 0, 0}, stream);
+}
+
+extern "C" int fdn_rfft_rows_pad1(const float* x, const float* w, const float* bias, float* out_c, int B, int C, int H, int W,
+                                  long out_row_bins, fdn_stream_t stream) {
+    FDN_CHECK_ARG(x && w && bias && out_c && B > 0 && C > 0 && H > 0 && W >= 2 && W % 2 == 0 && W < (1 << 20));
+    int R1 = 0, P = 0;
+    if (rows_plan(W + 2, &R1, &P)) return FDN_ERR_UNSUPPORTED;
+    return rfft_rows_impl(x, out_c, (long)B * C * (H + 2), W + 2, out_row_bins, RowPad{w, bias, C, H, W}, stream);
 }
 
 extern "C" int fdn_rfft_rows_ln(const float* x, const float* stats, const float* gamma, const float* beta, float* out_c, int B, int C,
@@ -1611,13 +1677,14 @@
     return FDN_ERR_UNSUPPORTED;
 }
 
-extern "C" int fdn_irfft_rows(const float* in_c, long in_row_bins, long in_plane_bins, float* out, long planes, int H, int W,
-                              float scale, const float* res, float alpha, fdn_stream_t stream) {
+namespace {
+int irfft_rows_impl(const float* in_c, long in_row_bins, long in_plane_bins, float* out, long planes, int H, int W,
+                    float scale, const float* res, float alpha, const float* ratio, long img_rows, fdn_stream_t stream) {
     FDN_CHECK_ARG(in_c && out && planes > 0 && H > 0 && W >= 2 && W % 2 == 0 && in_row_bins >= W / 2 + 1);
     {
         int R1 = 0, P = 0;
         if (rows_plan(W, &R1, &P) && ((reinterpret_cast<uintptr_t>(out) | reinterpret_cast<uintptr_t>(res)) & 7) == 0) {
-#define FDN_CALL(a, b) launch_irfft_rp<a, b>(in_c, in_row_bins, in_plane_bins, out, planes, H, scale, res, alpha, stream)
+#define FDN_CALL(a, b) launch_irfft_rp<a, b>(in_c, in_row_bins, in_plane_bins, out, planes, H, scale, res, alpha, ratio, img_rows, stream)
             FDN_ROWS_DISPATCH(FDN_CALL)
 #undef FDN_CALL
         }
@@ -1634,14 +1701,26 @@
         if (int e = set_lds(irfft_rows_kernel<true>, lds)) return e;
         hipLaunchKernelGGL(irfft_rows_kernel<true>, dim3(cdiv(rows, rpb)), dim3(NT), lds, static_cast<hipStream_t>(stream),
                            reinterpret_cast<const float2*>(in_c), in_row_bins, (long)H, in_plane_bins, out, W, H, rows, rpb,
-                           scale, res, alpha, p);
+                           scale, res, alpha, ratio, img_rows, p);
     } else {
         if (int e = set_lds(irfft_rows_kernel<false>, lds)) return e;
         hipLaunchKernelGGL(irfft_rows_kernel<false>, dim3(cdiv(rows, rpb)), dim3(NT), lds, static_cast<hipStream_t>(stream),
                            reinterpret_cast<const float2*>(in_c), in_row_bins, (long)H, in_plane_bins, out, W, H, rows, rpb,
-                           scale, res, alpha, p);
+                           scale, res, alpha, ratio, img_rows, p);
     }
     return fdn_launch_status();
+}
+}
+
+extern "C" int fdn_irfft_rows(const float* in_c, long in_row_bins, long in_plane_bins, float* out, long planes, int H, int W,
+                              float scale, const float* res, float alpha, fdn_stream_t stream) {
+    return irfft_rows_impl(in_c, in_row_bins, in_plane_bins, out, planes, H, W, scale, res, alpha, nullptr, 1, stream);
+}
+
+extern "C" int fdn_irfft_rows_ratio(const float* in_c, long in_row_bins, long in_plane_bins, float* out, long planes, int H, int W,
+                                    float scale, const float* res, float alpha, const float* ratio, int C, fdn_stream_t stream) {
+    FDN_CHECK_ARG(!ratio || (C > 0 && planes % C == 0));
+    return irfft_rows_impl(in_c, in_row_bins, in_plane_bins, out, planes, H, W, scale, res, alpha, ratio, (long)C * H, stream);
 }
 
 __global__ __launch_bounds__(256) void pack_guidance_kernel(const float* __restrict__ amp, const float* __restrict__ pha,
diff --git a/fdn-tip2025_amd/fdn_hip/__init__.py b/fdn-tip2025_amd/fdn_hip/__init__.py
--- a/fdn-tip2025_amd/fdn_hip/__init__.py
+++ b/fdn-tip2025_amd/fdn_hip/__init__.py
@@ -31,7 +31,7 @@
     pass
 
 
-ABI_VERSION = 20
+ABI_VERSION = 21
 
 
 def lib_path():
diff --git a/fdn-tip2025_amd/fdn_hip/_abi.py b/fdn-tip2025_amd/fdn_hip/_abi.py
--- a/fdn-tip2025_amd/fdn_hip/_abi.py
+++ b/fdn-tip2025_amd/fdn_hip/_abi.py
@@ -33,14 +33,17 @@
     "fdn_fft_prepare": ("I", ['I']),
     "fdn_sincos_f32": ("I", ['P', 'P', 'P', 'L', 'P']),
     "fdn_rfft_rows": ("I", ['P', 'P', 'L', 'I', 'L', 'P']),
+    "fdn_rfft_rows_pad1": ("I", ['P', 'P', 'P', 'P', 'I', 'I', 'I', 'I', 'L', 'P']),
     "fdn_rfft_rows_ln": ("I", ['P', 'P', 'P', 'P', 'P', 'I', 'I', 'I', 'I', 'L', 'P']),
     "fdn_irfft_rows": ("I", ['P', 'L', 'L', 'P', 'L', 'I', 'I', 'F', 'P', 'F', 'P']),
+    "fdn_irfft_rows_ratio": ("I", ['P', 'L', 'L', 'P', 'L', 'I', 'I', 'F', 'P', 'F', 'P', 'I', 'P']),
     "fdn_pack_guidance": ("I", ['P', 'P', 'P', 'I', 'I', 'I', 'L', 'P']),
     "fdn_fft_cols_fcaffn": ("I", ['P', 'P', 'P', 'P', 'I', 'I', 'I', 'I', 'P']),
     "fdn_fft_cols_fwd": ("I", ['P', 'P', 'P', 'L', 'I', 'I', 'I', 'I', 'P']),
     "fdn_fft_route": ("I", ['I', 'I', 'P', 'I']),
     "fdn_fft_cols_inv_polar": ("I", ['P', 'P', 'I', 'I', 'P', 'L', 'I', 'I', 'P']),
     "fdn_conv2d": ("I", ['P', 'P', 'P', 'P', 'P', 'I', 'I', 'I', 'I', 'I', 'I', 'I', 'I', 'I', 'I', 'I', 'F', 'P']),
+    "fdn_conv2d_ex": ("I", ['P', 'P', 'P', 'P', 'P', 'I', 'I', 'I', 'I', 'I', 'I', 'I', 'I', 'I', 'I', 'I', 'F', 'P', 'I', 'P']),
     "fdn_upconv_gather": ("I", ['P', 'P', 'I', 'I', 'I', 'I', 'P']),
     "fdn_conv_transpose4x4s2": ("I", ['P', 'P', 'P', 'P', 'I', 'I', 'I', 'I', 'I', 'I', 'P']),
     "fdn_resample": ("I", ['P', 'P', 'L', 'I', 'I', 'I', 'I', 'P']),
@@ -105,14 +108,17 @@
     "fdn_fft_prepare": ['n'],
     "fdn_sincos_f32": ['x', 'sn', 'cs', 'n', 'stream'],
     "fdn_rfft_rows": ['in', 'out_c', 'rows', 'W', 'out_row_bins', 'stream'],
+    "fdn_rfft_rows_pad1": ['x', 'w', 'bias', 'out_c', 'B', 'C', 'H', 'W', 'out_row_bins', 'stream'],
     "fdn_rfft_rows_ln": ['x', 'stats', 'gamma', 'beta', 'out_c', 'B', 'C', 'H', 'W', 'out_row_bins', 'stream'],
     "fdn_irfft_rows": ['in_c', 'in_row_bins', 'in_plane_bins', 'out', 'planes', 'H', 'W', 'scale', 'res', 'alpha', 'stream'],
+    "fdn_irfft_rows_ratio": ['in_c', 'in_row_bins', 'in_plane_bins', 'out', 'planes', 'H', 'W', 'scale', 'res', 'alpha', 'ratio', 'C', 'stream'],
     "fdn_pack_guidance": ['amp', 'pha', 'packed', 'B', 'H', 'Wf', 'row_bins', 'stream'],
     "fdn_fft_cols_fcaffn": ['z', 'guide', 'wxa', 'wxp', 'B', 'C', 'H', 'Wf', 'stream'],
     "fdn_fft_cols_fwd": ['z', 'out_abs', 'out_ang', 'planes', 'H', 'Wf', 'rd_before', 'fix_real', 'stream'],
     "fdn_fft_route": ['kind', 'n', 'desc', 'ndesc'],
     "fdn_fft_cols_inv_polar": ['mag', 'pha', 'Hin', 'Wfin', 'z_out', 'planes', 'H', 'Wf', 'stream'],
     "fdn_conv2d": ['x', 'w', 'bias', 'res', 'out', 'B', 'Cin', 'H', 'W', 'Cout', 'KH', 'KW', 'stride', 'pad', 'act', 'res_before_act', 'post_add', 'stream'],
+    "fdn_conv2d_ex": ['x', 'w', 'bias', 'res', 'out', 'B', 'Cin', 'H', 'W', 'Cout', 'KH', 'KW', 'stride', 'pad', 'act', 'res_before_act', 'post_add', 'stats_out', 'one_pixel', 'stream'],
     "fdn_upconv_gather": ['z', 'out', 'B', 'Cout', 'h', 'w', 'stream'],
     "fdn_conv_transpose4x4s2": ['x', 'w', 'bias', 'out', 'B', 'Cin', 'H', 'W', 'Cout', 'act', 'stream'],
     "fdn_resample": ['x', 'out', 'planes', 'H', 'W', 'mode', 'r', 'stream'],
diff --git a/fdn-tip2025_amd/fdn_hip/ops.py b/fdn-tip2025_amd/fdn_hip/ops.py
--- a/fdn-tip2025_amd/fdn_hip/ops.py
+++ b/fdn-tip2025_amd/fdn_hip/ops.py
@@ -441,6 +441,18 @@
     return out
 
 
+def rfft_rows_pad1(x, w, bias, pitch=None):
+    if "rfft_pad1" not in OUTSIDE_BLOCKS:
+        return None
+    B, C, H, W = x.shape
+    out = torch.empty((B, C, H + 2, pitch or (W + 2) // 2 + 1, 2), device=x.device, dtype=torch.float32)
+    rc = lib().fdn_rfft_rows_pad1(_flat(x, "x"), _flat(w, "w"), _flat(bias, "bias"), _flat(out, "out"), B, C, H, W, ctypes.c_long(pitch or 0), stream())
+    if rc == ERR_UNSUPPORTED:
+        return None
+    check(rc, "fdn_rfft_rows_pad1")
+    return out
+
+
 ROWS_PLANNED_W = tuple(2 * r * p for r in (20, 30) for p in (32, 16, 8)) + (608, 304) + (1120, 560, 280)
 
 
@@ -457,10 +469,21 @@
     return out
 
 
-def irfft_rows(z, H, W, scale, res=None, alpha=0.0, out=None):
+OUTSIDE_BLOCKS = frozenset(("irfft_ratio", "conv_stats", "conv_run", "rfft_pad1"))
+
+
+def irfft_rows(z, H, W, scale, res=None, alpha=0.0, out=None, ratio=None):
     B, C, Hin, Wfin, _ = z.shape
     if out is None:
         out = torch.empty((B, C, H, W), device=z.device, dtype=torch.float32)
+    if ratio is not None and "irfft_ratio" not in OUTSIDE_BLOCKS:
+        return scale_batch_(irfft_rows(z, H, W, scale, res=res, alpha=alpha, out=out), ratio)
+    if ratio is not None:
+        assert ratio.numel() == B, (ratio.shape, B)
+        check(lib().fdn_irfft_rows_ratio(_flat(z, "z"), ctypes.c_long(Wfin), ctypes.c_long(Hin * Wfin), _flat(out, "out"),
+                                         ctypes.c_long(B * C), H, W, ctypes.c_float(scale), _flat(res, "res"),
+                                         ctypes.c_float(alpha), _flat(ratio, "ratio"), C, stream()), "fdn_irfft_rows_ratio")
+        return out
     check(lib().fdn_irfft_rows(_flat(z, "z"), ctypes.c_long(Wfin), ctypes.c_long(Hin * Wfin), _flat(out, "out"),
                                ctypes.c_long(B * C), H, W, ctypes.c_float(scale), _flat(res, "res"),
                                ctypes.c_float(alpha), stream()), "fdn_irfft_rows")
@@ -511,14 +534,30 @@
     return z
 
 
-def conv2d(x, w, bias=None, stride=1, pad=0, act=ACT_NONE, res=None, res_before_act=False, post_add=0.0):
+def conv2d(x, w, bias=None, stride=1, pad=0, act=ACT_NONE, res=None, res_before_act=False, post_add=0.0, want_stats=False):
     B, Cin, H, W = x.shape
     Cout, _, KH, KW = w.shape
     OH, OW = (H + 2 * pad - KH) // stride + 1, (W + 2 * pad - KW) // stride + 1
     out = torch.empty((B, Cout, OH, OW), device=x.device, dtype=torch.float32)
-    check(lib().fdn_conv2d(_flat(x, "x"), _flat(w, "w"), _flat(bias, "bias"), _flat(res, "res"), _flat(out, "out"),
-                           B, Cin, H, W, Cout, KH, KW, stride, pad, act, int(res_before_act), ctypes.c_float(post_add),
-                           stream()), "fdn_conv2d")
+    if want_stats and "conv_stats" in OUTSIDE_BLOCKS and "conv_run" in OUTSIDE_BLOCKS:
+        st = torch.empty((B, 1, 2, OH * OW), device=x.device, dtype=torch.float32)
+        rc = lib().fdn_conv2d_ex(_flat(x, "x"), _flat(w, "w"), _flat(bias, "bias"), _flat(res, "res"), _flat(out, "out"),
+                                 B, Cin, H, W, Cout, KH, KW, stride, pad, act, int(res_before_act), ctypes.c_float(post_add),
+                                 _flat(st, "stats_out"), 0, stream())
+        if rc != ERR_UNSUPPORTED:
+            check(rc, "fdn_conv2d_ex")
+            out._fdn_stats = st
+            return out
+    if "conv_run" in OUTSIDE_BLOCKS:
+        check(lib().fdn_conv2d(_flat(x, "x"), _flat(w, "w"), _flat(bias, "bias"), _flat(res, "res"), _flat(out, "out"),
+                               B, Cin, H, W, Cout, KH, KW, stride, pad, act, int(res_before_act), ctypes.c_float(post_add),
+                               stream()), "fdn_conv2d")
+    else:
+        check(lib().fdn_conv2d_ex(_flat(x, "x"), _flat(w, "w"), _flat(bias, "bias"), _flat(res, "res"), _flat(out, "out"),
+                                  B, Cin, H, W, Cout, KH, KW, stride, pad, act, int(res_before_act), ctypes.c_float(post_add),
+                                  None, 1, stream()), "fdn_conv2d_ex")
+    if want_stats:
+        out._fdn_stats = chan_stats(out)
     return out
 
 
diff --git a/fdn-tip2025_amd/fdn_hip/pipeline.py b/fdn-tip2025_amd/fdn_hip/pipeline.py
--- a/fdn-tip2025_amd/fdn_hip/pipeline.py
+++ b/fdn-tip2025_amd/fdn_hip/pipeline.py
@@ -67,7 +67,7 @@
 def weights_signature(*modules):
     from . import _cu_budgets, matrix_pipe_mode, ops
     ps = [p for m in modules for p in list(m.parameters()) + list(m.buffers())]
-    return (storage_dtype(), matrix_pipe_mode(), tuple(sorted(_cu_budgets.items())), bool(ops.FDSA_FULL), int(ops.FDSA_FULL_MAX_C), bool(ops.FDSA_TAIL), bool(ops.FDSA_TAIL_PIN), int(ops.FDSA_TAIL_PIN_MAX_C), str(ops.FFN_TAIL_MODE), bool(ops.SPECTRAL_MLP_FUSED), bool(ops.GEMM_OWN_STATS), bool(ops.UPCONV_GATHER), bool(ops.AFF_MULTIRES),
+    return (storage_dtype(), matrix_pipe_mode(), tuple(sorted(_cu_budgets.items())), bool(ops.FDSA_FULL), int(ops.FDSA_FULL_MAX_C), bool(ops.FDSA_TAIL), bool(ops.FDSA_TAIL_PIN), int(ops.FDSA_TAIL_PIN_MAX_C), str(ops.FFN_TAIL_MODE), bool(ops.SPECTRAL_MLP_FUSED), bool(ops.GEMM_OWN_STATS), bool(ops.UPCONV_GATHER), bool(ops.AFF_MULTIRES), tuple(sorted(ops.OUTSIDE_BLOCKS)),
             len(ps), sum(p._version for p in ps), sum(p.data_ptr() & 0xFFFFFFFF for p in ps))
 
 
diff --git a/include/fdn_hip.h b/include/fdn_hip.h
--- a/include/fdn_hip.h
+++ b/include/fdn_hip.h
@@ -107,10 +107,14 @@
 int fdn_fft_prepare(int n);
 int fdn_sincos_f32(const float* x, float* sn, float* cs, long n, fdn_stream_t stream);
 int fdn_rfft_rows(const float* in, float* out_c, long rows, int W, long out_row_bins, fdn_stream_t stream);
+int fdn_rfft_rows_pad1(const float* x, const float* w, const float* bias, float* out_c, int B, int C, int H, int W,
+                       long out_row_bins, fdn_stream_t stream);
 int fdn_rfft_rows_ln(const float* x, const float* stats, const float* gamma, const float* beta, float* out_c, int B, int C, int H,
                      int W, long out_row_bins, fdn_stream_t stream);
 int fdn_irfft_rows(const float* in_c, long in_row_bins, long in_plane_bins, float* out, long planes, int H, int W,
                    float scale, const float* res, float alpha, fdn_stream_t stream);
+int fdn_irfft_rows_ratio(const float* in_c, long in_row_bins, long in_plane_bins, float* out, long planes, int H, int W,
+                         float scale, const float* res, float alpha, const float* ratio, int C, fdn_stream_t stream);
 int fdn_pack_guidance(const float* amp, const float* pha, float* packed, int B, int H, int Wf, long row_bins, fdn_stream_t stream);
 int fdn_fft_cols_fcaffn(float* z, const float* guide, const float* wxa, const float* wxp, int B, int C, int H, int Wf,
                         fdn_stream_t stream);
@@ -125,6 +129,9 @@
 int fdn_conv2d(const float* x, const float* w, const float* bias, const float* res, float* out, int B, int Cin, int H,
                int W, int Cout, int KH, int KW, int stride, int pad, int act, int res_before_act, float post_add,
                fdn_stream_t stream);
+int fdn_conv2d_ex(const float* x, const float* w, const float* bias, const float* res, float* out, int B, int Cin, int H,
+                  int W, int Cout, int KH, int KW, int stride, int pad, int act, int res_before_act, float post_add,
+                  float* stats_out, int one_pixel, fdn_stream_t stream);
 int fdn_upconv_gather(const float* z, float* out, int B, int Cout, int h, int w, fdn_stream_t stream);
 int fdn_conv_transpose4x4s2(const float* x, const float* w, const float* bias, float* out, int B, int Cin, int H, int W,
                             int Cout, int act, fdn_stream_t stream);
```

Result: no change. 28.03 images/s, median of 6 (+0.4%).
